# pananananas/MVD

Hardware: AMD Instinct MI355X
Metric: UNet forward-passes/sec @512x512 SD2.1+MV adapter (higher is better)
Workload: dtype bf16; 1 GPU; cfg4: configs[3]/[4]: 8 objects x 4 target views per GPU (32 pairs), camera FiLM + cross-view adapter; pairs_per_gpu=32, global_pairs=32, latent=64x64x4, image=512x512, forward=cold, hip_graph=False, q2_statistics=replica-local, parallelism=dp1 (pairs sharded by object), weights=synthetic seeded, SD2.1 shapes (865.9M UNet x2 + 99.2M adapter + 19.1M camera), encoder_weights=distinct

## Files before the change

### include/mvd_hip.h

```cpp
#ifndef MVD_HIP_H
#define MVD_HIP_H
#include <stddef.h>
#include <stdint.h>

#ifdef __cplusplus
extern "C" {
#endif

#define MVD_MAX_LEVELS 4

typedef struct {
  int in_channels;
  int out_channels;
  int num_levels;
  int block_out_channels[MVD_MAX_LEVELS];
  int num_heads[MVD_MAX_LEVELS];
  int layers_per_block;
  int cross_attention_dim;
  int norm_num_groups;
  float norm_eps;
  int cam_output_dim;
  int cam_hidden_dim;
  int simple_cam_encoder;
  float cam_modulation_strength;
} mvd_config_t;

typedef struct mvd_engine mvd_engine_t;

const char* mvd_last_error(void);

int mvd_engine_create(const mvd_config_t* cfg, mvd_engine_t** out);
int mvd_engine_destroy(mvd_engine_t* e);

int mvd_engine_set_weight(mvd_engine_t* e, int set, const char* slot, const void* ptr, int64_t numel, int dtype);
int mvd_engine_clear_weights(mvd_engine_t* e, int set);

int64_t mvd_engine_workspace_bytes(mvd_engine_t* e, int batch, int height, int width, int text_len, int ref_batch);
int64_t mvd_engine_refcache_bytes(mvd_engine_t* e, int ref_batch, int height, int width, int keep_features);
int mvd_engine_bind_workspace(mvd_engine_t* e, void* ws, int64_t ws_bytes, void* refcache, int64_t refcache_bytes);

enum {
  MVD_USE_CAMERA = 1,
  MVD_USE_IMAGE = 2,
  MVD_REUSE_REF = 4,
  MVD_KEEP_FEATURES = 8
};

typedef struct {
  int batch;
  int height, width;
  int text_len;
  const float* sample;
  const float* timesteps;
  const float* text;
  const float* source_camera;
  const float* target_camera;
  int cam_rows;
  int cam_batch;
  const float* fourier_proj;
  const float* source_latents;
  const float* encoder_text;
  int ref_batch;
  int flags;
  float* out;
} mvd_forward_args_t;

int mvd_unet_forward(mvd_engine_t* e, const mvd_forward_args_t* args, void* stream);

int64_t mvd_engine_reference_pixels(mvd_engine_t* e, int height, int width);
int mvd_engine_reference_encode(mvd_engine_t* e, const mvd_forward_args_t* args, float* local_stats, void* stream);
int mvd_engine_reference_finish(mvd_engine_t* e, const float* mean_k, void* stream);

int mvd_engine_set_graph(mvd_engine_t* e, int enable);

int mvd_engine_share_encoder_weights(mvd_engine_t* e, int enable);

int mvd_engine_set_profiling(mvd_engine_t* e, int enable);
int mvd_engine_profile_summary(mvd_engine_t* e, int cap, int* cls, int* launches, double* ms, double* flops, double* bytes);
int mvd_engine_profile_shapes(mvd_engine_t* e, char* buf_host, int cap);

int mvd_engine_num_features(mvd_engine_t* e);
int mvd_engine_feature_shape(mvd_engine_t* e, int idx, int* channels, int* height, int* width);
int mvd_engine_get_feature(mvd_engine_t* e, int idx, float* out_nchw, void* stream);
int mvd_engine_encode_cameras(mvd_engine_t* e, const float* source_camera, const float* target_camera, int cam_rows,
                              int batch, const float* fourier_proj, float* out_emb, void* stream);
int mvd_engine_apply_modulation(mvd_engine_t* e, const char* name, const float* emb, int batch, const float* x_nchw,
                                int channels, int hw, float* out_nchw, void* stream);
int mvd_engine_get_camera_embedding(mvd_engine_t* e, float* out, void* stream);

int mvd_op_linear(const void* a, const void* a2, int k1, int k2, const void* w, const float* bias, const float* rowvec,
                  int ld_rowvec, int rows_per_batch, const void* res, float alpha, int geglu, void* out, int out_f32,
                  int m, int n, int force_cfg, int splitk, float* splitk_ws ,
                  void* stream);
int mvd_op_ln_linear(const void* x, int k, const void* w_folded, const float* c1, const float* c2, float eps, int geglu,
                     void* out, int m, int n, void* stream);
int mvd_op_linear_xs(const void* x, int ldx, const void* w_packed, int m, int k, int units, int geglu, int ln, float ln_eps,
                     const void* res, int ldres, void* out, int ldo, int csplit, void* stream);
int mvd_op_conv3x3_ws(const void* x, int batch, int h, int w, int c, const void* w_packed, const float* bias, const float* rowvec,
                      int ld_rowvec, const void* res, const void* sc, const void* sc2, int sc_c1, int sc_c2, void* out, int n,
                      int variant, void* stream);
int mvd_op_conv3x3(const void* x, int batch, int in_h, int in_w, int cin, int stride, int upsample, int asym_pad, const void* w,
                   const float* bias, const float* rowvec, int ld_rowvec, const void* res, const void* sc, const void* sc2,
                   int sc_c1, int sc_c2, void* out, int cout, int force_cfg, int splitk, float* splitk_ws, void* stream);
int mvd_op_conv3x3_up4(const void* x, int batch, int in_h, int in_w, int cin, const void* w4, const float* bias, void* out, int cout,
                       int force_cfg, void* stream);
int mvd_op_attention(const void* q, const void* k, const void* v, void* o, int batch, int heads, int nq, int nk, int ldq,
                     int ldk, int ldv, int ldo, float scale, void* stream);
int64_t mvd_op_attention_split_ws_bytes(int batch, int heads, int nq, int nsplit);
int mvd_op_attention_split(const void* q, const void* k, const void* v, void* o, int batch, int heads, int nq, int nk, int ldq,
                           int ldk, int ldv, int ldo, int nsplit, void* ws, void* stream);
int mvd_op_groupnorm(const void* x0, const void* x1, int c0, int c1, int batch, int hw, int groups, float eps,
                     const float* gamma, const float* beta, int silu, void* y, float* ws, void* stream);
int mvd_op_layernorm(const void* x, int rows, int c, float eps, const float* gamma, const float* beta, void* y,
                     void* stream);
int mvd_op_refnorm(const void* x, int batch, int hw, int c, void* y, void* stream);
int mvd_op_film(const void* x, int batch, int hw, int c, const float* scale, const float* shift, void* y, void* stream);
int mvd_op_conv_in(const void* x, int batch, int h, int w, int cin, const float* wt, const float* bias, int cout, void* y,
                   void* stream);
int mvd_op_conv_out(const void* x, int batch, int h, int w, int c, const void* wt, const float* bias, int cout, float* y,
                    void* stream);
int mvd_op_nchw_to_nhwc(const float* x, int batch, int c, int hw, const float* scale, const float* shift, void* y,
                        void* stream);
int mvd_op_nhwc_to_nchw(const void* x, int batch, int hw, int c, float* y, void* stream);
int mvd_op_f32_to_bf16(const float* x, int64_t n, void* y, void* stream);
int mvd_op_skinny_linear(const float* x, int ldx, int batch, int k, const void* w, int wbf16, const float* bias, int n, int act_in,
                         float* y, int ldy, void* stream);
int mvd_gemm_num_configs(void);
int mvd_debug_last_gemm_plan(int* out);
int mvd_debug_last_attention_plan(int* out);
int mvd_debug_last_groupnorm_plan(int* out);
long mvd_debug_up4_launches(void);
int mvd_debug_last_gemm_nowait(void);
int mvd_debug_pick_splitk(int m, int n, int k, int geglu);
int mvd_debug_pick_splitk_conv(int m, int n, int k);
int mvd_gemm_sm_num_tiles(void);
int mvd_debug_set_attention_nw(int nw_log2);
typedef enum {
  MVD_DBG_NO_SM_LN_FOLD = 1,
  MVD_DBG_SM_NO_SPLITK = 2,
  MVD_DBG_NO_SM = 4,
  MVD_DBG_NO_SPLIT_KV = 8,
  MVD_DBG_ONE_STREAM = 16,
  MVD_DBG_SINGLE_STREAM_POLICY = 32,
  MVD_DBG_SIDE_DEFAULT_PRIORITY = 64,
  MVD_DBG_NO_XS = 128,
  MVD_DBG_NO_WS = 256,
  MVD_DBG_WS_SMALL_MAPS = 512,
  MVD_DBG_WS_BLOCK64 = 1024,
  MVD_DBG_WS_NO_SHORTCUT = 2048,
  MVD_DBG_WS_NOT_IN_ENCODER = 4096,
  MVD_DBG_WS_ONLY_IN_ENCODER = 8192,
  MVD_DBG_WS_THEN_TILED = 16384,
  MVD_DBG_WS_CHECK = 32768,
  MVD_DBG_GRAPH_ONE_STREAM = 65536,
  MVD_DBG_PP_ROW_MAJOR = 131072,
  MVD_DBG_NO_DEEP_CONV_SPLIT = 262144,
  MVD_DBG_LATE_FROM_UP1 = 524288,
  MVD_DBG_NO_UP4 = 1048576,
  MVD_DBG_GN_ONE_PASS = 2097152,
  MVD_DBG_FORK_LATE = 4194304,
  MVD_DBG_SKINNY_VECTOR = 8388608
} mvd_debug_flag_t;
int mvd_debug_set_flags(int flags);

int mvd_op_ddpm_step(const float* model_out, const float* sample, const float* noise, float c0, float c1, float c2,
                     float c3, float sigma, float* out, int64_t n, void* stream);
int mvd_op_cfg_combine(const float* uncond_cond, float guidance_scale, float* out, int64_t n_half, void* stream);
int mvd_op_sampler_step(const float* model_out, int guided, float guidance_scale, const float* sample, const float* x0_prev,
                        const float* noise, float a0, float a1, float p, float q, float r, float sigma, float* out,
                        float* x0_out, int64_t n, void* stream);

int mvd_op_add_noise(const float* x0, const float* noise, const int32_t* timesteps, const float* sqrt_ac, const float* sqrt_1mac,
                     int num_train_timesteps, float* noisy, float* velocity, int batch, int64_t per_sample, void* stream);
int64_t mvd_op_noise_loss_ws_bytes(int batch, int64_t per_sample);
int mvd_op_noise_loss(const float* pred, const float* noise, const float* x0, const float* noisy, const int32_t* timesteps,
                      const float* sqrt_ac, const float* sqrt_1mac, const float* snr, int num_train_timesteps, int prediction_type,
                      float snr_gamma, float* denoised, float* result, int batch, int64_t per_sample, void* ws, int64_t ws_bytes,
                      void* stream);
int64_t mvd_op_image_metrics_ws_bytes(int n, int c, int h, int w, int want_ssim);
int mvd_op_image_metrics(const float* x, const float* y, int n, int c, int h, int w, float data_range, int want_ssim, float* result,
                         float* per_image, void* ws, int64_t ws_bytes, void* stream);

typedef struct {
  int in_channels;
  int latent_channels;
  int num_levels;
  int block_out_channels[MVD_MAX_LEVELS];
  int layers_per_block;
  int norm_num_groups;
  float norm_eps;
} mvd_vae_config_t;
typedef struct mvd_vae mvd_vae_t;
int mvd_vae_create(const mvd_vae_config_t* cfg, mvd_vae_t** out);
int mvd_vae_destroy(mvd_vae_t* v);
int mvd_vae_set_weight(mvd_vae_t* v, const char* slot, const void* ptr, int64_t numel, int dtype);
int64_t mvd_vae_workspace_bytes(mvd_vae_t* v, int batch, int height, int width, int decode);
int mvd_vae_bind_workspace(mvd_vae_t* v, void* ws, int64_t ws_bytes);
int mvd_vae_encode(mvd_vae_t* v, const float* image_nchw, int batch, int height, int width, float* moments, void* stream);
int mvd_vae_decode(mvd_vae_t* v, const float* latents_nchw, int batch, int height, int width, float* image, void* stream);
int64_t mvd_vae_mid_attention_workspace_bytes(mvd_vae_t* v, int decoder, int batch, int height, int width);
int mvd_vae_mid_attention(mvd_vae_t* v, int decoder, const void* x_nhwc_bf16, int batch, int height, int width, void* out_nhwc_bf16,
                          void* stream);
int mvd_op_softmax_rows(const float* s, int rows, int n, void* p_bf16, void* stream);
int mvd_op_gaussian_sample(const float* moments, const float* noise, int batch, int channels, int hw, float scale, float* out,
                           void* stream);

typedef struct {
  int vocab_size;
  int hidden_size;
  int intermediate_size;
  int num_layers;
  int num_heads;
  int max_positions;
  float layer_norm_eps;
  int act;
} mvd_text_config_t;
typedef struct mvd_text mvd_text_t;
int mvd_text_create(const mvd_text_config_t* cfg, mvd_text_t** out);
int mvd_text_destroy(mvd_text_t* t);
int mvd_text_set_weight(mvd_text_t* t, const char* slot, const void* ptr, int64_t numel, int dtype);
int64_t mvd_text_workspace_bytes(mvd_text_t* t, int batch, int seq_len);
int mvd_text_bind_workspace(mvd_text_t* t, void* ws, int64_t bytes);
int mvd_text_encode(mvd_text_t* t, const int32_t* ids, int batch, int seq_len, float* out, void* stream);
int mvd_op_attention_causal(const void* q, const void* k, const void* v, void* o, int batch, int heads, int n, int ldq, int ldk,
                            int ldv, int ldo, float scale, void* stream);

typedef struct {
  int image_size;
  int patch_size;
  int hidden_size;
  int intermediate_size;
  int num_layers;
  int num_heads;
  int projection_dim;
  float layer_norm_eps;
  int act;
} mvd_vision_config_t;
typedef struct mvd_vision mvd_vision_t;
int mvd_vision_create(const mvd_vision_config_t* cfg, mvd_vision_t** out);
int mvd_vision_destroy(mvd_vision_t* v);
int mvd_vision_set_weight(mvd_vision_t* v, const char* slot, const void* ptr, int64_t numel, int dtype);
int64_t mvd_vision_workspace_bytes(mvd_vision_t* v, int batch, int h, int w, int resize_to);
int mvd_vision_bind_workspace(mvd_vision_t* v, void* ws, int64_t bytes);
int mvd_vision_preprocess(mvd_vision_t* v, const float* images_nchw, int batch, int h, int w, int quantize, int resize_to, int crop,
                          const float* mean, const float* std_, int want_patches, float* pixel_values, void* stream);
// ... 71 lines not shown
```

### mvd_amd/_lib.py

```python
from __future__ import annotations

import ctypes as C
import enum
import os

HERE = os.path.dirname(os.path.abspath(__file__))
LIB_PATH = os.environ.get("MVD_HIP_LIB") or os.path.join(HERE, "libmvd_hip.so")

MVD_MAX_LEVELS = 4
MVD_USE_CAMERA, MVD_USE_IMAGE, MVD_REUSE_REF, MVD_KEEP_FEATURES = 1, 2, 4, 8


class MvdError(RuntimeError):
    pass


class DebugFlag(enum.IntFlag):
    NO_SM_LN_FOLD = 1
    SM_NO_SPLITK = 2
    NO_SM = 4
    NO_SPLIT_KV = 8
    ONE_STREAM = 16
    SINGLE_STREAM_POLICY = 32
    SIDE_DEFAULT_PRIORITY = 64
# ... 24 lines not shown
        ("norm_eps", C.c_float), ("cam_output_dim", C.c_int), ("cam_hidden_dim", C.c_int),
        ("simple_cam_encoder", C.c_int), ("cam_modulation_strength", C.c_float),
    ]


class mvd_vae_config_t(C.Structure):
    _fields_ = [
        ("in_channels", C.c_int), ("latent_channels", C.c_int), ("num_levels", C.c_int),
        ("block_out_channels", C.c_int * MVD_MAX_LEVELS), ("layers_per_block", C.c_int), ("norm_num_groups", C.c_int),
        ("norm_eps", C.c_float),
    ]


class mvd_text_config_t(C.Structure):
    _fields_ = [
        ("vocab_size", C.c_int), ("hidden_size", C.c_int), ("intermediate_size", C.c_int), ("num_layers", C.c_int),
        ("num_heads", C.c_int), ("max_positions", C.c_int), ("layer_norm_eps", C.c_float), ("act", C.c_int),
    ]


class mvd_vision_config_t(C.Structure):
    _fields_ = [
        ("image_size", C.c_int), ("patch_size", C.c_int), ("hidden_size", C.c_int), ("intermediate_size", C.c_int),
        ("num_layers", C.c_int), ("num_heads", C.c_int), ("projection_dim", C.c_int), ("layer_norm_eps", C.c_float), ("act", C.c_int),
    ]


class mvd_forward_args_t(C.Structure):
    _fields_ = [
        ("batch", C.c_int), ("height", C.c_int), ("width", C.c_int), ("text_len", C.c_int),
        ("sample", C.c_void_p), ("timesteps", C.c_void_p), ("text", C.c_void_p),
        ("source_camera", C.c_void_p), ("target_camera", C.c_void_p), ("cam_rows", C.c_int), ("cam_batch", C.c_int),
        ("fourier_proj", C.c_void_p), ("source_latents", C.c_void_p), ("encoder_text", C.c_void_p),
        ("ref_batch", C.c_int), ("flags", C.c_int), ("out", C.c_void_p),
    ]


_SIGS = {
    "mvd_last_error": (C.c_char_p, []),
    "mvd_engine_create": (C.c_int, [C.POINTER(mvd_config_t), C.POINTER(C.c_void_p)]),
    "mvd_engine_destroy": (C.c_int, [C.c_void_p]),
    "mvd_engine_set_weight": (C.c_int, [C.c_void_p, C.c_int, C.c_char_p, C.c_void_p, C.c_int64, C.c_int]),
    "mvd_engine_clear_weights": (C.c_int, [C.c_void_p, C.c_int]),
    "mvd_engine_workspace_bytes": (C.c_int64, [C.c_void_p, C.c_int, C.c_int, C.c_int, C.c_int, C.c_int]),
    "mvd_engine_refcache_bytes": (C.c_int64, [C.c_void_p, C.c_int, C.c_int, C.c_int, C.c_int]),
    "mvd_engine_bind_workspace": (C.c_int, [C.c_void_p, C.c_void_p, C.c_int64, C.c_void_p, C.c_int64]),
    "mvd_unet_forward": (C.c_int, [C.c_void_p, C.POINTER(mvd_forward_args_t), C.c_void_p]),
    "mvd_engine_set_profiling": (C.c_int, [C.c_void_p, C.c_int]),
    "mvd_engine_profile_summary": (C.c_int, [C.c_void_p, C.c_int, C.POINTER(C.c_int), C.POINTER(C.c_int),
                                             C.POINTER(C.c_double), C.POINTER(C.c_double), C.POINTER(C.c_double)]),
    "mvd_engine_profile_shapes": (C.c_int, [C.c_void_p, C.c_char_p, C.c_int]),
    "mvd_engine_set_graph": (C.c_int, [C.c_void_p, C.c_int]),
    "mvd_engine_reference_pixels": (C.c_int64, [C.c_void_p, C.c_int, C.c_int]),
    "mvd_engine_reference_encode": (C.c_int, [C.c_void_p, C.POINTER(mvd_forward_args_t), C.c_void_p, C.c_void_p]),
    "mvd_engine_reference_finish": (C.c_int, [C.c_void_p, C.c_void_p, C.c_void_p]),
    "mvd_engine_share_encoder_weights": (C.c_int, [C.c_void_p, C.c_int]),
    "mvd_engine_num_features": (C.c_int, [C.c_void_p]),
    "mvd_engine_feature_shape": (C.c_int, [C.c_void_p, C.c_int, C.POINTER(C.c_int), C.POINTER(C.c_int), C.POINTER(C.c_int)]),
    "mvd_engine_get_feature": (C.c_int, [C.c_void_p, C.c_int, C.c_void_p, C.c_void_p]),
    "mvd_engine_encode_cameras": (C.c_int, [C.c_void_p, C.c_void_p, C.c_void_p, C.c_int, C.c_int, C.c_void_p, C.c_void_p, C.c_void_p]),
    "mvd_engine_apply_modulation": (C.c_int, [C.c_void_p, C.c_char_p, C.c_void_p, C.c_int, C.c_void_p, C.c_int, C.c_int, C.c_void_p, C.c_void_p]),
    "mvd_engine_get_camera_embedding": (C.c_int, [C.c_void_p, C.c_void_p, C.c_void_p]),
    "mvd_op_linear": (C.c_int, [C.c_void_p, C.c_void_p, C.c_int, C.c_int, C.c_void_p, C.c_void_p, C.c_void_p, C.c_int,
                                C.c_int, C.c_void_p, C.c_float, C.c_int, C.c_void_p, C.c_int, C.c_int, C.c_int, C.c_int,
                                C.c_int, C.c_void_p, C.c_void_p]),
    "mvd_op_ln_linear": (C.c_int, [C.c_void_p, C.c_int, C.c_void_p, C.c_void_p, C.c_void_p, C.c_float, C.c_int, C.c_void_p,
                                   C.c_int, C.c_int, C.c_void_p]),
    "mvd_op_linear_xs": (C.c_int, [C.c_void_p, C.c_int, C.c_void_p, C.c_int, C.c_int, C.c_int, C.c_int, C.c_int, C.c_float,
                                   C.c_void_p, C.c_int, C.c_void_p, C.c_int, C.c_int, C.c_void_p]),
    "mvd_op_conv3x3_ws": (C.c_int, [C.c_void_p, C.c_int, C.c_int, C.c_int, C.c_int, C.c_void_p, C.c_void_p, C.c_void_p, C.c_int,
                                    C.c_void_p, C.c_void_p, C.c_void_p, C.c_int, C.c_int, C.c_void_p, C.c_int, C.c_int, C.c_void_p]),
    "mvd_op_conv3x3": (C.c_int, [C.c_void_p, C.c_int, C.c_int, C.c_int, C.c_int, C.c_int, C.c_int, C.c_int, C.c_void_p, C.c_void_p,
                                 C.c_void_p, C.c_int, C.c_void_p, C.c_void_p, C.c_void_p, C.c_int, C.c_int, C.c_void_p,
                                 C.c_int, C.c_int, C.c_int, C.c_void_p, C.c_void_p]),
    "mvd_op_attention": (C.c_int, [C.c_void_p, C.c_void_p, C.c_void_p, C.c_void_p, C.c_int, C.c_int, C.c_int, C.c_int,
                                   C.c_int, C.c_int, C.c_int, C.c_int, C.c_float, C.c_void_p]),
    "mvd_op_attention_split_ws_bytes": (C.c_int64, [C.c_int, C.c_int, C.c_int, C.c_int]),
    "mvd_op_attention_split": (C.c_int, [C.c_void_p, C.c_void_p, C.c_void_p, C.c_void_p, C.c_int, C.c_int, C.c_int, C.c_int, C.c_int,
                                         C.c_int, C.c_int, C.c_int, C.c_int, C.c_void_p, C.c_void_p]),
    "mvd_op_groupnorm": (C.c_int, [C.c_void_p, C.c_void_p, C.c_int, C.c_int, C.c_int, C.c_int, C.c_int, C.c_float,
                                   C.c_void_p, C.c_void_p, C.c_int, C.c_void_p, C.c_void_p, C.c_void_p]),
    "mvd_op_layernorm": (C.c_int, [C.c_void_p, C.c_int, C.c_int, C.c_float, C.c_void_p, C.c_void_p, C.c_void_p, C.c_void_p]),
    "mvd_op_refnorm": (C.c_int, [C.c_void_p, C.c_int, C.c_int, C.c_int, C.c_void_p, C.c_void_p]),
    "mvd_op_film": (C.c_int, [C.c_void_p, C.c_int, C.c_int, C.c_int, C.c_void_p, C.c_void_p, C.c_void_p, C.c_void_p]),
    "mvd_op_conv_in": (C.c_int, [C.c_void_p, C.c_int, C.c_int, C.c_int, C.c_int, C.c_void_p, C.c_void_p, C.c_int, C.c_void_p, C.c_void_p]),
    "mvd_op_conv_out": (C.c_int, [C.c_void_p, C.c_int, C.c_int, C.c_int, C.c_int, C.c_void_p, C.c_void_p, C.c_int, C.c_void_p, C.c_void_p]),
    "mvd_op_nchw_to_nhwc": (C.c_int, [C.c_void_p, C.c_int, C.c_int, C.c_int, C.c_void_p, C.c_void_p, C.c_void_p, C.c_void_p]),
    "mvd_op_nhwc_to_nchw": (C.c_int, [C.c_void_p, C.c_int, C.c_int, C.c_int, C.c_void_p, C.c_void_p]),
    "mvd_op_f32_to_bf16": (C.c_int, [C.c_void_p, C.c_int64, C.c_void_p, C.c_void_p]),
    "mvd_op_skinny_linear": (C.c_int, [C.c_void_p, C.c_int, C.c_int, C.c_int, C.c_void_p, C.c_int, C.c_void_p, C.c_int, C.c_int,
                                        C.c_void_p, C.c_int, C.c_void_p]),
    "mvd_gemm_num_configs": (C.c_int, []),
    "mvd_debug_last_gemm_plan": (C.c_int, [C.POINTER(C.c_int)]),
    "mvd_debug_up4_launches": (C.c_long, []),
    "mvd_op_conv3x3_up4": (C.c_int, [C.c_void_p, C.c_int, C.c_int, C.c_int, C.c_int, C.c_void_p, C.c_void_p, C.c_void_p, C.c_int, C.c_int,
                                     C.c_void_p]),
    "mvd_debug_last_gemm_nowait": (C.c_int, []),
    "mvd_debug_last_attention_plan": (C.c_int, [C.POINTER(C.c_int)]),
    "mvd_debug_last_groupnorm_plan": (C.c_int, [C.POINTER(C.c_int)]),
    "mvd_debug_pick_splitk": (C.c_int, [C.c_int, C.c_int, C.c_int, C.c_int]),
    "mvd_debug_pick_splitk_conv": (C.c_int, [C.c_int, C.c_int, C.c_int]),
    "mvd_gemm_sm_num_tiles": (C.c_int, []),
    "mvd_debug_set_attention_nw": (C.c_int, [C.c_int]),
    "mvd_debug_set_flags": (C.c_int, [C.c_int]),
    "mvd_op_ddpm_step": (C.c_int, [C.c_void_p, C.c_void_p, C.c_void_p, C.c_float, C.c_float, C.c_float, C.c_float,
                                   C.c_float, C.c_void_p, C.c_int64, C.c_void_p]),
    "mvd_op_cfg_combine": (C.c_int, [C.c_void_p, C.c_float, C.c_void_p, C.c_int64, C.c_void_p]),
    "mvd_op_sampler_step": (C.c_int, [C.c_void_p, C.c_int, C.c_float, C.c_void_p, C.c_void_p, C.c_void_p, C.c_float, C.c_float,
                                      C.c_float, C.c_float, C.c_float, C.c_float, C.c_void_p, C.c_void_p, C.c_int64, C.c_void_p]),
    "mvd_op_add_noise": (C.c_int, [C.c_void_p, C.c_void_p, C.c_void_p, C.c_void_p, C.c_void_p, C.c_int, C.c_void_p, C.c_void_p, C.c_int,
                                   C.c_int64, C.c_void_p]),
    "mvd_op_noise_loss_ws_bytes": (C.c_int64, [C.c_int, C.c_int64]),
    "mvd_op_noise_loss": (C.c_int, [C.c_void_p, C.c_void_p, C.c_void_p, C.c_void_p, C.c_void_p, C.c_void_p, C.c_void_p, C.c_void_p,
                                    C.c_int, C.c_int, C.c_float, C.c_void_p, C.c_void_p, C.c_int, C.c_int64, C.c_void_p, C.c_int64,
                                    C.c_void_p]),
    "mvd_op_image_metrics_ws_bytes": (C.c_int64, [C.c_int, C.c_int, C.c_int, C.c_int, C.c_int]),
    "mvd_op_image_metrics": (C.c_int, [C.c_void_p, C.c_void_p, C.c_int, C.c_int, C.c_int, C.c_int, C.c_float, C.c_int, C.c_void_p,
                                       C.c_void_p, C.c_void_p, C.c_int64, C.c_void_p]),
    "mvd_vae_create": (C.c_int, [C.POINTER(mvd_vae_config_t), C.POINTER(C.c_void_p)]),
    "mvd_vae_destroy": (C.c_int, [C.c_void_p]),
    "mvd_vae_set_weight": (C.c_int, [C.c_void_p, C.c_char_p, C.c_void_p, C.c_int64, C.c_int]),
    "mvd_vae_workspace_bytes": (C.c_int64, [C.c_void_p, C.c_int, C.c_int, C.c_int, C.c_int]),
    "mvd_vae_bind_workspace": (C.c_int, [C.c_void_p, C.c_void_p, C.c_int64]),
    "mvd_vae_encode": (C.c_int, [C.c_void_p, C.c_void_p, C.c_int, C.c_int, C.c_int, C.c_void_p, C.c_void_p]),
    "mvd_vae_decode": (C.c_int, [C.c_void_p, C.c_void_p, C.c_int, C.c_int, C.c_int, C.c_void_p, C.c_void_p]),
    "mvd_vae_mid_attention_workspace_bytes": (C.c_int64, [C.c_void_p, C.c_int, C.c_int, C.c_int, C.c_int]),
    "mvd_vae_mid_attention": (C.c_int, [C.c_void_p, C.c_int, C.c_void_p, C.c_int, C.c_int, C.c_int, C.c_void_p, C.c_void_p]),
    "mvd_op_softmax_rows": (C.c_int, [C.c_void_p, C.c_int, C.c_int, C.c_void_p, C.c_void_p]),
    "mvd_op_gaussian_sample": (C.c_int, [C.c_void_p, C.c_void_p, C.c_int, C.c_int, C.c_int, C.c_float, C.c_void_p, C.c_void_p]),
    "mvd_text_create": (C.c_int, [C.POINTER(mvd_text_config_t), C.POINTER(C.c_void_p)]),
    "mvd_text_destroy": (C.c_int, [C.c_void_p]),
    "mvd_text_set_weight": (C.c_int, [C.c_void_p, C.c_char_p, C.c_void_p, C.c_int64, C.c_int]),
    "mvd_text_workspace_bytes": (C.c_int64, [C.c_void_p, C.c_int, C.c_int]),
    "mvd_text_bind_workspace": (C.c_int, [C.c_void_p, C.c_void_p, C.c_int64]),
    "mvd_text_encode": (C.c_int, [C.c_void_p, C.c_void_p, C.c_int, C.c_int, C.c_void_p, C.c_void_p]),
    "mvd_op_attention_causal": (C.c_int, [C.c_void_p, C.c_void_p, C.c_void_p, C.c_void_p, C.c_int, C.c_int, C.c_int, C.c_int,
                                          C.c_int, C.c_int, C.c_int, C.c_float, C.c_void_p]),
    "mvd_vision_create": (C.c_int, [C.POINTER(mvd_vision_config_t), C.POINTER(C.c_void_p)]),
    "mvd_vision_destroy": (C.c_int, [C.c_void_p]),
    "mvd_vision_set_weight": (C.c_int, [C.c_void_p, C.c_char_p, C.c_void_p, C.c_int64, C.c_int]),
    "mvd_vision_workspace_bytes": (C.c_int64, [C.c_void_p, C.c_int, C.c_int, C.c_int, C.c_int]),
    "mvd_vision_bind_workspace": (C.c_int, [C.c_void_p, C.c_void_p, C.c_int64]),
    "mvd_vision_preprocess": (C.c_int, [C.c_void_p, C.c_void_p, C.c_int, C.c_int, C.c_int, C.c_int, C.c_int, C.c_int,
                                        C.POINTER(C.c_float), C.POINTER(C.c_float), C.c_int, C.c_void_p, C.c_void_p]),
    "mvd_vision_patch_rows_offset": (C.c_int64, [C.c_void_p]),
    "mvd_vision_encode": (C.c_int, [C.c_void_p, C.c_void_p, C.c_int, C.c_void_p, C.c_void_p, C.c_void_p, C.c_void_p]),
    "mvd_op_clip_pool_project": (C.c_int, [C.c_void_p, C.c_void_p, C.c_void_p, C.c_int, C.c_int, C.c_int, C.c_int, C.c_void_p,
                                           C.c_void_p, C.c_float, C.c_void_p, C.c_int, C.c_void_p, C.c_void_p, C.c_void_p]),
    "mvd_op_clip_cosine": (C.c_int, [C.c_void_p, C.c_void_p, C.c_int, C.c_int, C.c_void_p, C.c_void_p, C.c_void_p]),
    "mvd_vgg_create": (C.c_int, [C.POINTER(C.c_void_p)]),
    "mvd_vgg_destroy": (C.c_int, [C.c_void_p]),
    "mvd_vgg_set_weight": (C.c_int, [C.c_void_p, C.c_char_p, C.c_void_p, C.c_int64, C.c_int]),
    "mvd_vgg_workspace_bytes": (C.c_int64, [C.c_void_p, C.c_int, C.c_int, C.c_int]),
    "mvd_vgg_bind_workspace": (C.c_int, [C.c_void_p, C.c_void_p, C.c_int64]),
    "mvd_vgg_features": (C.c_int, [C.c_void_p, C.c_void_p, C.c_int, C.c_int, C.c_int, C.c_void_p, C.POINTER(C.c_void_p), C.c_void_p]),
    "mvd_vgg_perceptual": (C.c_int, [C.c_void_p, C.c_void_p, C.c_void_p, C.c_int, C.c_int, C.c_int, C.c_void_p, C.c_void_p, C.c_void_p]),
    "mvd_op_conv3x3_relu": (C.c_int, [C.c_void_p, C.c_int, C.c_int, C.c_int, C.c_int, C.c_void_p, C.c_void_p, C.c_void_p, C.c_int, C.c_int,
                                      C.c_int, C.c_int, C.c_int, C.c_void_p, C.c_void_p]),
    "mvd_op_linear_relu": (C.c_int, [C.c_void_p, C.c_int, C.c_void_p, C.c_void_p, C.c_void_p, C.c_int, C.c_int, C.c_int, C.c_int, C.c_int,
                                     C.c_int, C.c_void_p, C.c_void_p]),
    "mvd_op_maxpool2x2": (C.c_int, [C.c_void_p, C.c_int, C.c_int, C.c_int, C.c_int, C.c_void_p, C.c_void_p]),
    "mvd_op_sqdiff_mean_ws_bytes": (C.c_int64, [C.c_int, C.c_int64]),
    "mvd_op_sqdiff_mean": (C.c_int, [C.c_void_p, C.c_void_p, C.c_int, C.c_int64, C.c_void_p, C.c_void_p, C.c_void_p, C.c_int64, C.c_void_p]),
    "mvd_lpips_create": (C.c_int, [C.POINTER(C.c_void_p)]),
    "mvd_lpips_destroy": (C.c_int, [C.c_void_p]),
    "mvd_lpips_set_weight": (C.c_int, [C.c_void_p, C.c_char_p, C.c_void_p, C.c_int64, C.c_int]),
    "mvd_lpips_workspace_bytes": (C.c_int64, [C.c_void_p, C.c_int, C.c_int, C.c_int]),
    "mvd_lpips_bind_workspace": (C.c_int, [C.c_void_p, C.c_void_p, C.c_int64]),
    "mvd_lpips_features": (C.c_int, [C.c_void_p, C.c_void_p, C.c_int, C.c_int, C.c_int, C.POINTER(C.c_void_p), C.c_void_p]),
    "mvd_lpips_distance": (C.c_int, [C.c_void_p, C.c_void_p, C.c_void_p, C.c_int, C.c_int, C.c_int, C.c_int, C.c_void_p, C.c_void_p,
                                     C.c_void_p, C.c_void_p]),
    "mvd_op_im2col_patch": (C.c_int, [C.c_void_p, C.c_int, C.c_int, C.c_int, C.c_int, C.POINTER(C.c_float), C.POINTER(C.c_float), C.c_void_p,
                                      C.c_void_p]),
    "mvd_op_maxpool3x3s2": (C.c_int, [C.c_void_p, C.c_int, C.c_int, C.c_int, C.c_int, C.c_void_p, C.c_void_p]),
    "mvd_op_lpips_head_ws_bytes": (C.c_int64, [C.c_int, C.POINTER(C.c_int), C.c_int]),
    "mvd_op_lpips_head": (C.c_int, [C.c_int, C.POINTER(C.c_void_p), C.POINTER(C.c_void_p), C.POINTER(C.c_int), C.POINTER(C.c_int),
                                    C.POINTER(C.c_int), C.POINTER(C.c_int), C.POINTER(C.c_void_p), C.c_int, C.c_void_p, C.c_void_p, C.c_void_p,
                                    C.c_void_p, C.c_int64, C.c_void_p]),
    "mvd_fid_create": (C.c_int, [C.POINTER(C.c_int), C.c_int, C.POINTER(C.c_int), C.c_int, C.POINTER(C.c_char_p), C.c_int, C.c_int, C.c_int,
                                 C.POINTER(C.c_void_p)]),
# ... 61 lines not shown
```

### mvd_amd/csrc/engine.hip

```cpp
#include <math.h>
#include <stdio.h>
#include <stdlib.h>
#include <string.h>

#include <string>
#include <unordered_map>
#include <vector>

#include "host_util.h"

int mvd_launch_silu_to_bf16(const float* x, int64_t n, bf16_t* y, hipStream_t s);

static int g_debug_flags = 0;
extern "C" int mvd_debug_set_flags(int flags) { g_debug_flags = flags; return 0; }
int mvd_debug_flags() { return g_debug_flags; }

namespace {

struct FeatureInfo { std::string name; int level; int C; int heads; std::string key;  };
constexpr int MVD_REF_ONLY_INTERNAL = 1 << 30;

}

struct mvd_engine {
  mvd_config_t cfg;
  WeightTable w[2];
  Arena tmp, act, persist;
  void* ws_ptr = nullptr; int64_t ws_bytes = 0;
  void* rc_ptr = nullptr; int64_t rc_bytes = 0;
  std::vector<FeatureInfo> feats;
  std::vector<bf16_t*> refkv;
  std::vector<bf16_t*> feat_keep;
  int rc_batch = 0, rc_h = 0, rc_w = 0; bool rc_valid = false; bool rc_keep = false;
  float* ref_stats_out = nullptr;
  bool rc_pending = false;
  int64_t ref_pixels(int h, int w) const { int64_t n = 0; for (auto& f : feats) n += (int64_t)(h >> f.level) * (w >> f.level); return n; }
  int64_t feat_pixel_off(int idx) const { int64_t n = 0; for (int i = 0; i < idx; ++i) n += (int64_t)(rc_h >> feats[i].level) * (rc_w >> feats[i].level); return n; }
  float* cam_emb = nullptr; int cam_batch = 0;
  unsigned int* cnt_base = nullptr; int cnt_used = 0, cnt_cap = 0;
  hipStream_t side = nullptr;
  std::vector<hipEvent_t> feat_ev;
  hipEvent_t fork_ev = nullptr, join_ev = nullptr;
  bool dual_now = false;
  int ensure_side_stream() {
    if (side) return 0;
    {
      int lo = 0, hi = 0;
      (void)hipDeviceGetStreamPriorityRange(&lo, &hi);
      const int pr = (g_debug_flags & MVD_DBG_SIDE_DEFAULT_PRIORITY) ? 0 : hi;
      if (hipStreamCreateWithPriority(&side, hipStreamNonBlocking, pr) != hipSuccess) { mvd_set_error("engine: hipStreamCreate failed"); return -3; }
    }
    feat_ev.resize(feats.size());
    for (auto& ev : feat_ev) if (hipEventCreateWithFlags(&ev, hipEventDisableTiming) != hipSuccess) { mvd_set_error("engine: hipEventCreate failed"); return -3; }
    if (hipEventCreateWithFlags(&fork_ev, hipEventDisableTiming) != hipSuccess || hipEventCreateWithFlags(&join_ev, hipEventDisableTiming) != hipSuccess) { mvd_set_error("engine: hipEventCreate failed"); return -3; }
    return 0;
  }
  bool share_encoder = false;
  struct HostState {
    std::vector<bf16_t*> refkv, feat_keep;
    int rc_batch, rc_h, rc_w; bool rc_valid, rc_keep;
    float* cam_emb; int cam_batch;
  };
  HostState host_state() const { return {refkv, feat_keep, rc_batch, rc_h, rc_w, rc_valid, rc_keep, cam_emb, cam_batch}; }
  void set_host_state(const HostState& h) {
    refkv = h.refkv; feat_keep = h.feat_keep; rc_batch = h.rc_batch; rc_h = h.rc_h; rc_w = h.rc_w; rc_valid = h.rc_valid;
    rc_keep = h.rc_keep; cam_emb = h.cam_emb; cam_batch = h.cam_batch;
  }
  struct GraphEntry { std::string key; hipGraph_t g; hipGraphExec_t x; HostState after; };
  bool dual_late = false;
  bool graph_on = false;
  std::vector<GraphEntry> graphs;
  std::vector<std::string> graph_seen;
  void drop_graphs() {
    for (auto& ge : graphs) { (void)hipGraphExecDestroy(ge.x); (void)hipGraphDestroy(ge.g); }
    graphs.clear(); graph_seen.clear();
  }
  ~mvd_engine() {
    drop_graphs();
    for (hipEvent_t ev : ev_pool) (void)hipEventDestroy(ev);
    for (hipEvent_t ev : feat_ev) if (ev) (void)hipEventDestroy(ev);
    if (fork_ev) (void)hipEventDestroy(fork_ev);
    if (join_ev) (void)hipEventDestroy(join_ev);
    if (side) (void)hipStreamDestroy(side);
  }
  std::vector<int> temb_off;
  int temb_total = 0;
  std::vector<int> tkv_off;
  int tkv_total = 0;
  bool prof = false;
  bool prof_overlap = false;
  struct ProfRec { int cls; double flops; double bytes; hipEvent_t e0, e1; int M, N, K, tag; };
  int prof_M = 0, prof_N = 0, prof_K = 0, prof_tag = 0;
  std::vector<ProfRec> prof_recs;
  std::vector<hipEvent_t> ev_pool; size_t ev_used = 0;
  hipEvent_t get_event() {
    if (ev_used == ev_pool.size()) { hipEvent_t ev = nullptr; (void)hipEventCreate(&ev); ev_pool.push_back(ev); }
    return ev_pool[ev_used++];
  }
// ... 69 lines not shown

struct Ctx {
  mvd_engine* e;
  hipStream_t s;
  int set;
  bool dry;
  int err = 0;
  bool nowait = false;

  const void* W(const std::string& name, int dtype, int64_t numel, int set_override = -1) {
    if (dry) return nullptr;
    const int st = set_override >= 0 ? set_override : set;
    return e->w[st].find(name, dtype, numel, &err, "", st);
  }
  const bf16_t* WB(const std::string& n, int64_t numel, int so = -1) { return (const bf16_t*)W(n, 1, numel, so); }
  const float* WF(const std::string& n, int64_t numel, int so = -1) { return (const float*)W(n, 0, numel, so); }
  bool has(const std::string& n, int so = -1) { return e->w[so >= 0 ? so : set].has(n); }

  template <class T> T* talloc(size_t n) { return e->tmp.alloc_n<T>(n); }
  template <class T> T* aalloc(size_t n) { return e->act.alloc_n<T>(n); }
  Act new_act(int B, int H, int W_, int C, bool longlived) { return arena_act(longlived ? e->act : e->tmp, B, H, W_, C); }

  template <class F> int profiled(int cls, double flops, double bytes, F&& launch) {
    if (!e->prof) return launch();
    hipEvent_t e0 = e->get_event(), e1 = e->get_event();
    (void)hipEventRecord(e0, s);
    const int r = launch();
    (void)hipEventRecord(e1, s);
    e->prof_recs.push_back({cls, flops, bytes, e0, e1, e->prof_M, e->prof_N, e->prof_K, e->prof_tag});
    return r;
  }
  static bool sm_enabled() {
    static const bool use_sm = MVD_ENV_INT("MVD_GEMM_SM", 1) != 0;
    return use_sm && !(g_debug_flags & MVD_DBG_NO_SM);
  }
  void tiled_plan(const MvdGemmArgs& g, int& S, int& fc) {
    S = mvd_gemm_pick_splitk(g);
    fc = -1;
    if (e->dual_now && !e->dual_late && !(g_debug_flags & MVD_DBG_SINGLE_STREAM_POLICY) && !g.geglu && !g.ln_c1 && !g.out_f32 && g.N % 320 == 0 && mvd_gemm_pp_applicable(g)) {
      const int cfg = mvd_gemm_pick_config(g);
      const long t7 = (long)((g.M + 255) / 256) * (g.N / 320);
      if (t7 >= 100) { S = 1; if (cfg != 7) fc = 7; }
    }
  }
  int gemm(MvdGemmArgs& g) {
    if (err) return err;
    int sm_tile = 0, sm_ns = 0, sm_S = 1;
    if (sm_enabled() && mvd_gemm_sm_plan(g, &sm_tile, &sm_ns, &sm_S)) {
      if (g_debug_flags & MVD_DBG_SM_NO_SPLITK) sm_S = 1;
      const size_t mark = e->tmp.off;
      if (sm_S > 1) {
        g.splitk = sm_S; g.splitk_nowait = nowait ? 1 : 0; g.part = talloc<float>((size_t)sm_S * g.M * g.N);
        const int tiles = ((g.M + 63) / 64) * (g.N / 64);
        g.tile_cnt = e->cnt_base + e->cnt_used;
        e->cnt_used += tiles;
        if (!dry && e->cnt_used > e->cnt_cap) { mvd_set_error("forward: split-K tile counters exhausted (%d > %d)", e->cnt_used, e->cnt_cap); return err = -15; }
      }
      int r = 0;
      if (!dry) {
        const double fl = 2.0 * g.M * (double)g.N * g.Ktot;
        e->prof_M = g.M; e->prof_N = g.N; e->prof_K = g.Ktot; e->prof_tag = g.seg[0].mode * 100 + g.geglu * 10 + (sm_S > 1 ? sm_S : 0);
        r = profiled(MVD_PC_SM_64X64 + sm_tile, fl, 0.0, [&] { return mvd_launch_gemm_sm(g, s, sm_tile, sm_ns); });
      }
      e->tmp.off = mark;
      return r;
    }
    int S = 1, fc = -1;
    tiled_plan(g, S, fc);
    const size_t mark = e->tmp.off;
    if (S > 1) { g.splitk = S; g.part = talloc<float>((size_t)S * g.M * g.N); } else g.splitk = 1;
    static const bool trace = MVD_ENV_INT("MVD_TRACE_GEMM", 0) != 0;
    if (trace && !dry) fprintf(stderr, "gemm M=%d N=%d K=%d mode=%d nseg=%d geglu=%d cfg=%d splitk=%d\n", g.M, g.N, g.Ktot, g.seg[0].mode, g.nseg, g.geglu, mvd_gemm_pick_config(g), S);
    int r = 0;
    if (!dry) {
      const double fl = 2.0 * g.M * (double)g.N * g.Ktot;
      e->prof_M = g.M; e->prof_N = g.N; e->prof_K = g.Ktot; e->prof_tag = g.seg[0].mode * 100 + g.geglu * 10 + (S > 1 ? S : 0);
      r = launch_tiled(g, s, fc, [&](auto&& launch) { return profiled(e->prof ? gemm_class(g, mvd_gemm_pick_config(g), S) : 0, fl, 0.0, launch); });
    }
    e->tmp.off = mark;
    return r;
  }

  int try_xs(const bf16_t* x, int K, int M, const std::string& slot, int64_t n_full, int N, bool geglu, bool ln,
             const bf16_t* res, int ldres, void* out, int ldo, int set_override = -1) {
    if (err) return err;
    if (dry || (g_debug_flags & MVD_DBG_NO_XS) || K != 320 || slot.empty() || !has(slot, set_override)) return 0;
    MvdXsArgs a; memset(&a, 0, sizeof(a));
    a.x = x; a.ldx = K; a.M = M; a.K = K; a.units = N / 32; a.geglu = geglu; a.ln = ln; a.ln_eps = 1e-5f;
    a.res = res; a.ldres = ldres; a.out = (bf16_t*)out; a.ldo = ldo;
    if (N % 64 || !mvd_gemm_xs_applicable(a)) return 0;
    if ((long)((M + 255) / 256) * mvd_gemm_xs_pick_csplit(a) < 448) return 0;
    a.w = WB(slot, (n_full / 32) * 21 * 512, set_override);
    if (!a.w) return err;
    e->prof_M = M; e->prof_N = N; e->prof_K = K; e->prof_tag = geglu * 10 + (ln ? 1 : 0);
    const int r = profiled(geglu ? MVD_PC_XS_GEGLU : (res ? MVD_PC_XS_RESIDUAL : (ln ? MVD_PC_XS_LN_DENSE : MVD_PC_XS_DENSE)), 2.0 * M * (double)N * K, 0.0, [&] { return mvd_launch_gemm_xs(a, s); });
    return r ? r : 1;
  }

  int linear(const bf16_t* a, const bf16_t* a2, int k1, int k2, int M, const bf16_t* w, const float* bias, int N,
             const bf16_t* res, int ldres, void* out, int ldo, bool geglu = false, bool out_f32 = false, int ldw = 0,
             const std::string& xs = std::string(), int xs_set = -1) {
    if (!xs.empty() && !a2 && !k2 && !geglu && !out_f32) {
      const int r = try_xs(a, k1, M, xs, N, N, false, false, res, ldres, out, ldo, xs_set);
      if (r) return r < 0 ? r : 0;
    }
    MvdGemmArgs g = gemm_dense(a, a2, k1, k2, M, w, ldw, bias, N, out, ldo);
    g.res = res; g.ldres = ldres; g.geglu = geglu; g.out_f32 = out_f32;
    return gemm(g);
  }

  int ln_linear(const bf16_t* x, int M, int C, const std::string& ln_key, const std::string& slot, int64_t n_full, int N,
                const float* bias, bf16_t* ln_tmp, void* out, int ldo, bool geglu) {
    MvdGemmArgs g = gemm_dense(x, nullptr, C, 0, M, nullptr, 0, nullptr, N, out, ldo);
    g.geglu = geglu;
    {
      const int r = try_xs(x, C, M, slot + ".wx", n_full, N, geglu, true, nullptr, 0, out, ldo);
      if (r) return r < 0 ? r : 0;
    }
    static const bool use_fold = MVD_ENV_INT("MVD_LN_FOLD", 1) != 0;
    auto sm_fold_ok = [&]() {
      MvdGemmArgs t = g;
      static const float dummy = 0.f;
      t.ln_c1 = &dummy; t.bias = &dummy; t.W = reinterpret_cast<const bf16_t*>(&dummy);
      int a_, b_, c_;
      return sm_enabled() && !(g_debug_flags & MVD_DBG_NO_SM_LN_FOLD) && mvd_gemm_sm_plan(t, &a_, &b_, &c_);
    };
    if (use_fold && !dry && has(slot + ".wf") && has(slot + ".cf") && (mvd_gemm_ln_fold_ok(g) || sm_fold_ok())) {
      const float* cf = WF(slot + ".cf", 2 * n_full);
      g.W = WB(slot + ".wf", n_full * C);
      g.ln_c1 = cf; g.bias = cf ? cf + n_full : nullptr; g.ln_eps = 1e-5f;
      return gemm(g);
    }
    CHECK(layernorm(x, M, C, WF(ln_key + ".g", C), WF(ln_key + ".b", C), ln_tmp));
    g.seg[0].p0 = ln_tmp; g.W = WB(slot + ".w", n_full * C); g.bias = bias;
    return gemm(g);
  }

  int try_ws(const Act& x, int ups, const std::string& slot, const float* bias, const float* rowvec, int ld_rowvec, const bf16_t* res,
             const bf16_t* sc0, const bf16_t* sc1, int scc0, int scc1, Act& out) {
    if (err) return err;
    if (dry || (g_debug_flags & MVD_DBG_NO_WS) || slot.empty() || !has(slot)) return 0;
    MvdWsArgs a; memset(&a, 0, sizeof(a));
    a.x = x.p; a.B = x.B; a.H = x.H; a.W = x.W; a.C = x.C; a.ups = ups; a.sc0 = sc0; a.sc1 = sc1; a.scc0 = scc0; a.scc1 = scc1;
    a.bias = bias; a.rowvec = rowvec; a.ld_rowvec = ld_rowvec; a.res = res; a.ldres = out.C; a.out = out.p; a.ldo = out.C;
    a.M = out.rows(); a.N = out.C;
    if ((g_debug_flags & MVD_DBG_WS_SMALL_MAPS) && a.M > 256) return 0;
    if (g_debug_flags & MVD_DBG_WS_BLOCK64) a.variant = 1;
    if ((g_debug_flags & MVD_DBG_WS_NO_SHORTCUT) && scc0) return 0;
    if ((g_debug_flags & MVD_DBG_WS_NOT_IN_ENCODER) && nowait) return 0;
    if ((g_debug_flags & MVD_DBG_WS_ONLY_IN_ENCODER) && !nowait) return 0;
    if (out.H != (ups ? 2 : 1) * x.H || out.W != (ups ? 2 : 1) * x.W || out.B != x.B || a.M > 1024) return 0;
    if ((long)(a.M / 64) * (a.N / 16) > 1000) return 0;
    a.w = reinterpret_cast<const bf16_t*>(&a);
    if (!mvd_conv_ws_applicable(a)) return 0;
    a.w = WB(slot, (int64_t)mvd_conv_ws_packed_elems(x.C, scc0 + scc1, out.C));
    if (!a.w) return err;
    e->prof_M = a.M; e->prof_N = a.N; e->prof_K = 9 * x.C + scc0 + scc1; e->prof_tag = 100 + (scc0 ? 1 : 0);
    const int r = profiled(MVD_PC_CONV_WS, 2.0 * a.M * (double)a.N * (9.0 * x.C + scc0 + scc1), 0.0, [&] { return mvd_launch_conv_ws(a, s); });
    if (!r && (g_debug_flags & MVD_DBG_WS_THEN_TILED)) return 0;
#ifdef MVD_PROBE
    if (!r && (g_debug_flags & MVD_DBG_WS_CHECK)) {
      const size_t mark = e->tmp.off;
      Act chk = new_act(out.B, out.H, out.W, out.C, false);
      const bf16_t* wold = WB(slot.substr(0, slot.size() - 1), (int64_t)out.C * (9 * x.C + scc0 + scc1));
      if (wold) {
        const int saved = g_debug_flags; g_debug_flags |= MVD_DBG_NO_WS;
        conv3(x, 1, ups, wold, bias, rowvec, ld_rowvec, res, sc0, sc1, scc0, scc1, chk);
        g_debug_flags = saved;
        g_ws_ptrs[0] = (const char*)x.p; g_ws_lens[0] = (size_t)x.rows() * x.C * 2;
        g_ws_ptrs[1] = (const char*)sc0; g_ws_lens[1] = (size_t)out.rows() * scc0 * 2;
        g_ws_ptrs[2] = (const char*)sc1; g_ws_lens[2] = (size_t)out.rows() * scc1 * 2;
        g_ws_ptrs[3] = (const char*)out.p; g_ws_lens[3] = (size_t)out.rows() * out.C * 2;
        ws_check_launch(slot, set, nowait, out.p, chk.p, (long)out.rows() * out.C, s);
      }
      e->tmp.off = mark;
    }
// ... 129 lines not shown
  int feat_idx = 0;

  int resnet(const std::string& key, const Act& x0, const Act* x1, int cout, Act& out) {
    const int cin0 = x0.C, cin1 = x1 ? x1->C : 0, cin = cin0 + cin1;
    const int B_ = x0.B, hw = x0.hw();
    const size_t mark = c.e->tmp.off;
    Act t1 = c.new_act(B_, x0.H, x0.W, cin, false);
    CHECK(c.groupnorm(x0.p, x1 ? x1->p : nullptr, cin0, cin1, B_, hw, cfg.norm_eps, c.WF(key + ".norm1.g", cin), c.WF(key + ".norm1.b", cin), 1, t1.p));
    Act h1 = c.new_act(B_, x0.H, x0.W, cout, false);
    const int toff = c.e->temb_off[resnet_idx++];
    CHECK(c.conv3(t1, 1, 0, c.WB(key + ".conv1.w", (int64_t)cout * 9 * cin), c.WF(key + ".conv1.b", cout), tproj + toff, c.e->temb_total,
                  nullptr, nullptr, nullptr, 0, 0, h1, key + ".conv1.ws"));
    Act t2 = c.new_act(B_, x0.H, x0.W, cout, false);
    CHECK(c.groupnorm(h1.p, nullptr, cout, 0, B_, hw, cfg.norm_eps, c.WF(key + ".norm2.g", cout), c.WF(key + ".norm2.b", cout), 1, t2.p));
    if (cin != cout) {
      CHECK(c.conv3(t2, 1, 0, c.WB(key + ".conv2.w", (int64_t)cout * (9 * cout + cin)), c.WF(key + ".conv2.b", cout), nullptr, 0, nullptr,
                    x0.p, x1 ? x1->p : nullptr, cin0, cin1, out, key + ".conv2.ws"));
    } else {
      CHECK(c.conv3(t2, 1, 0, c.WB(key + ".conv2.w", (int64_t)cout * 9 * cout), c.WF(key + ".conv2.b", cout), nullptr, 0, x0.p, nullptr,
                    nullptr, 0, 0, out, key + ".conv2.ws"));
    }
    c.e->tmp.off = mark;
    return c.err;
  }

  int transformer(const std::string& key, const Act& x, int heads, Act& out) {
    const int C = x.C, M = x.rows(), hw = x.hw(), B_ = x.B;
    const bool ad = o.adapter;
    const bool packed = c.set == 0 && (c.dry || c.has(key + ".ref_kv.w", 0));
    if (ad && !packed) { mvd_set_error("adapter requested but no adapter weights registered for %s", key.c_str()); return -14; }
    const int ld_out = packed ? 2 * C : C;
    const char* bias_slot = (packed && !ad) ? ".out.b0" : ".out.b";
    const size_t mark = c.e->tmp.off;
    bf16_t* n0 = c.talloc<bf16_t>((size_t)M * C);
    CHECK(c.groupnorm(x.p, nullptr, C, 0, B_, hw, 1e-6f, c.WF(key + ".norm.g", C), c.WF(key + ".norm.b", C), 0, n0));
    bf16_t* h = c.talloc<bf16_t>((size_t)M * C);
    CHECK(c.linear(n0, nullptr, C, 0, M, c.WB(key + ".proj_in.w", (int64_t)C * C), c.WF(key + ".proj_in.b", C), C, nullptr, 0, h, C, false, false, 0, key + ".proj_in.wx"));
    bf16_t* ln = n0;
    const float scale = 0.125f;
    bf16_t* o_self = c.talloc<bf16_t>((size_t)M * C);
    bf16_t* o_ref = ad ? c.talloc<bf16_t>((size_t)M * C) : nullptr;
    const bf16_t* rkv = ad ? c.e->refkv[feat_idx] : nullptr;
    const int ref_nk = ad ? (int)((int64_t)o.ref_batch * hw / B_) : 0;
    if (ad && (int64_t)ref_nk * B_ != (int64_t)o.ref_batch * hw) { mvd_set_error("adapter: ref tokens %d x %d not divisible by batch %d", o.ref_batch, hw, B_); return -12; }

    if (ad && c.e->dual_now && !c.dry && !c.err && hipStreamWaitEvent(c.s, c.e->feat_ev[feat_idx], 0) != hipSuccess) { mvd_set_error("forward: hipStreamWaitEvent failed"); return -3; }
    {
      const int nq = ad ? 4 * C : 3 * C;
      bf16_t* qkv = c.talloc<bf16_t>((size_t)M * nq);
      CHECK(c.ln_linear(h, M, C, key + ".ln1", key + ".attn1.qkv", (int64_t)(packed ? 4 : 3) * C, nq, nullptr, ln, qkv, nq, false));
      MvdAttnArgs a; memset(&a, 0, sizeof(a));
      a.batch = B_; a.heads = heads; a.scale = scale; a.prescaled = 1; a.nprob = ad ? 2 : 1;
      a.p[0] = {qkv, qkv + C, qkv + 2 * C, o_self, nq, nq, nq, C, (int64_t)hw * nq, (int64_t)hw * nq, (int64_t)hw * nq, (int64_t)hw * C, hw, hw};
      if (ad) a.p[1] = {qkv + 3 * C, rkv, rkv + C, o_ref, nq, 4 * C, 4 * C, C, (int64_t)hw * nq, (int64_t)ref_nk * 4 * C, (int64_t)ref_nk * 4 * C, (int64_t)hw * C, hw, ref_nk};
      CHECK(c.attention(a));
      CHECK(c.linear(o_self, o_ref, C, ad ? C : 0, M, c.WB(key + ".attn1.out.w", (int64_t)C * ld_out), c.WF(key + ".attn1" + bias_slot, C), C, h, C, h, C, false, false, ld_out,
                     ad ? std::string() : key + ".attn1.out.wx"));
    }
    {
      const int nq = ad ? 2 * C : C;
      bf16_t* q2 = c.talloc<bf16_t>((size_t)M * nq);
      const bf16_t* kv2 = tkv + c.e->tkv_off[feat_idx];
      const int ldkv = c.e->tkv_total;
      CHECK(c.ln_linear(h, M, C, key + ".ln2", key + ".attn2.q", (int64_t)(packed ? 2 : 1) * C, nq, nullptr, ln, q2, nq, false));
      MvdAttnArgs a; memset(&a, 0, sizeof(a));
      a.batch = B_; a.heads = heads; a.scale = scale; a.prescaled = 1; a.nprob = ad ? 2 : 1;
      a.p[0] = {q2, kv2, kv2 + C, o_self, nq, ldkv, ldkv, C, (int64_t)hw * nq, (int64_t)L * ldkv, (int64_t)L * ldkv, (int64_t)hw * C, hw, L};
      if (ad) a.p[1] = {q2 + C, rkv + 2 * C, rkv + 3 * C, o_ref, nq, 4 * C, 4 * C, C, (int64_t)hw * nq, (int64_t)ref_nk * 4 * C, (int64_t)ref_nk * 4 * C, (int64_t)hw * C, hw, ref_nk};
      CHECK(c.attention(a));
      CHECK(c.linear(o_self, o_ref, C, ad ? C : 0, M, c.WB(key + ".attn2.out.w", (int64_t)C * ld_out), c.WF(key + ".attn2" + bias_slot, C), C, h, C, h, C, false, false, ld_out,
                     ad ? std::string() : key + ".attn2.out.wx"));
    }
    {
      bf16_t* ff = c.talloc<bf16_t>((size_t)M * 4 * C);
      CHECK(c.ln_linear(h, M, C, key + ".ln3", key + ".ff1", (int64_t)8 * C, 8 * C, c.WF(key + ".ff1.b", 8 * C), ln, ff, 4 * C, true));
      CHECK(c.linear(ff, nullptr, 4 * C, 0, M, c.WB(key + ".ff2.w", (int64_t)C * 4 * C), c.WF(key + ".ff2.b", C), C, h, C, h, C));
    }
    CHECK(c.linear(h, nullptr, C, 0, M, c.WB(key + ".proj_out.w", (int64_t)C * C), c.WF(key + ".proj_out.b", C), C, x.p, C, out.p, C, false, false, 0, key + ".proj_out.wx"));
    c.e->tmp.off = mark;

    if (o.capture) {
      const size_t mk = c.e->tmp.off;
      bf16_t* rn = c.talloc<bf16_t>((size_t)M * C);
      if (o.defer_norm) {
        if (!c.dry && !c.err) CHECK(mvd_launch_refstats(out.p, B_, hw, C, o.stats + 2 * c.e->feat_pixel_off(feat_idx), c.s));
      } else {
        if (!c.dry && !c.err) CHECK(mvd_launch_refnorm(out.p, B_, hw, C, rn, c.s));
        CHECK(c.linear(rn, nullptr, C, 0, M, c.WB(key + ".ref_kv.w", (int64_t)4 * C * C, 0), nullptr, 4 * C, nullptr, 0, c.e->refkv[feat_idx], 4 * C, false, false, 0,
                       key + ".ref_kv.wx", 0));
        if (c.e->dual_now && !c.dry && !c.err && hipEventRecord(c.e->feat_ev[feat_idx], c.s) != hipSuccess) { mvd_set_error("forward: hipEventRecord failed"); return -3; }
      }
      if (c.e->rc_keep && !c.dry && !c.err)
        CHECK((int)hipMemcpyAsync(c.e->feat_keep[feat_idx], out.p, (size_t)M * C * sizeof(bf16_t), hipMemcpyDeviceToDevice, c.s));
      c.e->tmp.off = mk;
    }
    ++feat_idx;
    return c.err;
  }

  int film(const std::string& name, const Act& x, Act& out) {
    auto it = o.film_ss->find(name);
    if (it == o.film_ss->end()) { out = x; return 0; }
    if (c.dry || c.err) return c.err;
    return mvd_launch_film(x.p, x.B, x.hw(), x.C, it->second.first, it->second.second, x.C, out.p, c.s);
  }

  int run(const Act& x_in, float* out_nchw) {
    const int n = cfg.num_levels, Lb = cfg.layers_per_block;
    const int C0 = cfg.block_out_channels[0];
    std::vector<Act> skips;
    tkv = c.aalloc<bf16_t>((size_t)B * L * c.e->tkv_total);
    CHECK(c.linear(text, nullptr, cfg.cross_attention_dim, 0, B * L, c.WB("text_kv.w", (int64_t)c.e->tkv_total * cfg.cross_attention_dim), nullptr,
                   c.e->tkv_total, nullptr, 0, tkv, c.e->tkv_total));
    Act h = c.new_act(B, H0, W0, C0, true);
    CHECK(c.linear(x_in.p, nullptr, 64, 0, B * H0 * W0, c.WB("conv_in.w", (int64_t)C0 * 64), c.WF("conv_in.b", C0), C0, nullptr, 0, h.p, C0));
    skips.push_back(h);
    for (int i = 0; i < n; ++i) {
      const int co = cfg.block_out_channels[i];
      const std::string bk = "down_blocks." + std::to_string(i);
      for (int j = 0; j < Lb; ++j) {
        Act r = c.new_act(B, h.H, h.W, co, true);
        CHECK(resnet(bk + ".resnets." + std::to_string(j), h, nullptr, co, r));
        h = r;
        if (i + 1 < n) {
          Act t = c.new_act(B, h.H, h.W, co, true);
          CHECK(transformer(bk + ".attentions." + std::to_string(j), h, cfg.num_heads[i], t));
          h = t;
        }
        skips.push_back(h);
      }
      if (i + 1 < n) {
        Act d = c.new_act(B, (h.H + 1) / 2, (h.W + 1) / 2, co, true);
        CHECK(c.conv3(h, 2, 0, c.WB(bk + ".down.w", (int64_t)co * 9 * co), c.WF(bk + ".down.b", co), nullptr, 0, nullptr, nullptr, nullptr, 0, 0, d));
        h = d;
        skips.push_back(h);
      }
      if (o.film) {
        Act m = c.new_act(B, h.H, h.W, h.C, true);
        Act res = m;
        CHECK(film("down_" + std::to_string(i), h, res));
        h = res;
      }
    }
    {
      const int cm = cfg.block_out_channels[n - 1];
      Act r = c.new_act(B, h.H, h.W, cm, true);
      CHECK(resnet("mid_block.resnets.0", h, nullptr, cm, r));
      Act t = c.new_act(B, h.H, h.W, cm, true);
      CHECK(transformer("mid_block.attentions.0", r, cfg.num_heads[n - 1], t));
      Act r2 = c.new_act(B, h.H, h.W, cm, true);
      CHECK(resnet("mid_block.resnets.1", t, nullptr, cm, r2));
      h = r2;
      if (o.film) { Act res = h; CHECK(film("mid_0", h, res)); h = res; }
    }
    for (int i = 0; i < n; ++i) {
      const int co = cfg.block_out_channels[n - 1 - i];
      const std::string bk = "up_blocks." + std::to_string(i);
      if (!o.capture && i >= o.late_from) c.e->dual_late = true;
      for (int j = 0; j <= Lb; ++j) {
        Act skip = skips.back(); skips.pop_back();
        if (skip.H != h.H || skip.W != h.W) { mvd_set_error("up block %d: skip %dx%d vs hidden %dx%d (odd latent size unsupported)", i, skip.H, skip.W, h.H, h.W); return -13; }
        Act r = c.new_act(B, h.H, h.W, co, true);
        CHECK(resnet(bk + ".resnets." + std::to_string(j), h, &skip, co, r));
        h = r;
        if (i > 0) {
          Act t = c.new_act(B, h.H, h.W, co, true);
          CHECK(transformer(bk + ".attentions." + std::to_string(j), h, cfg.num_heads[n - 1 - i], t));
          h = t;
        }
      }
      if (i + 1 < n) {
        Act u = c.new_act(B, h.H * 2, h.W * 2, co, true);
// ... 652 lines not shown
  if (rows_per_batch > 0) g.rows_per_batch = g.outW = rows_per_batch;
  g.rowvec = rowvec; g.ld_rowvec = ld_rowvec; g.res = (const bf16_t*)res; g.ldres = on; g.alpha = alpha; g.geglu = geglu; g.out_f32 = out_f32;
  return op_launch(g, force_cfg, splitk, splitk_ws, (hipStream_t)stream);
}

int mvd_op_ln_linear(const void* x, int k, const void* w_folded, const float* c1, const float* c2, float eps, int geglu,
                     void* out, int m, int n, void* stream) {
  MvdGemmArgs g = gemm_dense((const bf16_t*)x, nullptr, k, 0, m, (const bf16_t*)w_folded, 0, c2, n, out, geglu ? n / 2 : n);
  g.ln_c1 = c1; g.ln_eps = eps; g.geglu = geglu; g.ldres = g.ldo;
  if (!c1 || !c2) { mvd_set_error("mvd_op_ln_linear: c1 and c2 are required"); return -1; }
  if (!mvd_gemm_ln_fold_ok(g)) {
    int tile = 0, ns = 0, S = 1;
    if (mvd_gemm_sm_plan(g, &tile, &ns, &S) && S == 1) {
      g_mvd_last_gemm.cfg = 100 + 10 * tile + ns; g_mvd_last_gemm.splitk = 1;
      return mvd_launch_gemm_sm(g, (hipStream_t)stream, tile, ns);
    }
    mvd_set_error("mvd_op_ln_linear: M=%d N=%d K=%d geglu=%d is not a shape of the fused LayerNorm GEMMs", m, n, k, geglu);
    return -1;
  }
  return mvd_launch_gemm(g, (hipStream_t)stream);
}

int mvd_op_conv3x3(const void* x, int batch, int in_h, int in_w, int cin, int stride, int upsample, int asym_pad, const void* w,
                   const float* bias, const float* rowvec, int ld_rowvec, const void* res, const void* sc, const void* sc2,
                   int sc_c1, int sc_c2, void* out, int cout, int force_cfg, int splitk, float* splitk_ws, void* stream) {
  const int oh = upsample ? in_h * 2 : (stride == 2 ? (in_h + 1) / 2 : in_h);
  const int ow = upsample ? in_w * 2 : (stride == 2 ? (in_w + 1) / 2 : in_w);
  MvdGemmArgs g = gemm_conv3((const bf16_t*)x, in_h, in_w, cin, stride, upsample, asym_pad, (const bf16_t*)sc, (const bf16_t*)sc2, sc_c1, sc_c2,
                             (const bf16_t*)w, bias, batch, oh, ow, cout, out);
  g.rowvec = rowvec; g.ld_rowvec = ld_rowvec; g.res = (const bf16_t*)res;
  return op_launch(g, force_cfg, splitk, splitk_ws, (hipStream_t)stream);
}

int mvd_op_conv3x3_up4(const void* x, int batch, int in_h, int in_w, int cin, const void* w4, const float* bias, void* out, int cout,
                       int force_cfg, void* stream) {
  if (!x || !w4 || !out || batch <= 0 || in_h <= 0 || in_w <= 0 || cin <= 0 || cout <= 0) { mvd_set_error("mvd_op_conv3x3_up4: bad argument"); return -1; }
  MvdGemmArgs g = gemm_conv3((const bf16_t*)x, in_h, in_w, cin, 1, 1, 0, nullptr, nullptr, 0, 0, (const bf16_t*)w4, bias, batch, 2 * in_h, 2 * in_w,
                             cout, out);
  gemm_conv3_to_up4(g);
  g.splitk = 1;
  return mvd_launch_gemm(g, (hipStream_t)stream, force_cfg);
}

int mvd_op_attention(const void* q, const void* k, const void* v, void* o, int batch, int heads, int nq, int nk, int ldq,
                     int ldk, int ldv, int ldo, float scale, void* stream) {
  MvdAttnArgs a; memset(&a, 0, sizeof(a));
  a.nprob = 1; a.batch = batch; a.heads = heads; a.scale = scale;
  a.prescaled = scale == 0.f;
  a.p[0] = {(const bf16_t*)q, (const bf16_t*)k, (const bf16_t*)v, (bf16_t*)o, ldq, ldk, ldv, ldo,
            (int64_t)nq * ldq, (int64_t)nk * ldk, (int64_t)nk * ldv, (int64_t)nq * ldo, nq, nk};
  return mvd_launch_attention(a, (hipStream_t)stream);
}

int64_t mvd_op_attention_split_ws_bytes(int batch, int heads, int nq, int nsplit) {
  MvdAttnArgs a; memset(&a, 0, sizeof(a));
  a.nprob = 1; a.batch = batch; a.heads = heads; a.p[0].nq = nq;
  return (int64_t)mvd_attention_split_ws_bytes(a, nsplit) + (int64_t)mvd_attention_split_counters(a) * 4 + 256;
}
int mvd_op_attention_split(const void* q, const void* k, const void* v, void* o, int batch, int heads, int nq, int nk, int ldq,
                           int ldk, int ldv, int ldo, int nsplit, void* ws, void* stream) {
  MvdAttnArgs a; memset(&a, 0, sizeof(a));
  a.nprob = 1; a.batch = batch; a.heads = heads; a.scale = 0.f; a.prescaled = 1;
  a.p[0] = {(const bf16_t*)q, (const bf16_t*)k, (const bf16_t*)v, (bf16_t*)o, ldq, ldk, ldv, ldo,
            (int64_t)nq * ldq, (int64_t)nk * ldk, (int64_t)nk * ldv, (int64_t)nq * ldo, nq, nk};
  if (nsplit > 1) {
    if (!ws) { mvd_set_error("op_attention_split: null workspace"); return -1; }
    const size_t pb = (mvd_attention_split_ws_bytes(a, nsplit) + 255) & ~size_t(255);
    a.nsplit = nsplit; a.split_ws = ws; a.split_cnt = reinterpret_cast<unsigned int*>(reinterpret_cast<char*>(ws) + pb);
    if (hipMemsetAsync(a.split_cnt, 0, (size_t)mvd_attention_split_counters(a) * 4, (hipStream_t)stream) != hipSuccess) { mvd_set_error("op_attention_split: hipMemsetAsync failed"); return -3; }
  }
  return mvd_launch_attention(a, (hipStream_t)stream);
}

int mvd_op_groupnorm(const void* x0, const void* x1, int c0, int c1, int batch, int hw, int groups, float eps,
                     const float* gamma, const float* beta, int silu, void* y, float* ws, void* stream) {
  return mvd_launch_groupnorm((const bf16_t*)x0, (const bf16_t*)x1, c0, c1, batch, hw, groups, eps, gamma, beta, silu, (bf16_t*)y, ws, (hipStream_t)stream);
}
int mvd_op_layernorm(const void* x, int rows, int c, float eps, const float* gamma, const float* beta, void* y, void* stream) {
  return mvd_launch_layernorm((const bf16_t*)x, rows, c, eps, gamma, beta, (bf16_t*)y, (hipStream_t)stream);
}
int mvd_op_refnorm(const void* x, int batch, int hw, int c, void* y, void* stream) {
  return mvd_launch_refnorm((const bf16_t*)x, batch, hw, c, (bf16_t*)y, (hipStream_t)stream);
}
int mvd_op_film(const void* x, int batch, int hw, int c, const float* scale, const float* shift, void* y, void* stream) {
  return mvd_launch_film((const bf16_t*)x, batch, hw, c, scale, shift, c, (bf16_t*)y, (hipStream_t)stream);
}
int mvd_op_conv_in(const void* x, int batch, int h, int w, int cin, const float* wt, const float* bias, int cout, void* y, void* stream) {
  return mvd_launch_conv_in((const bf16_t*)x, batch, h, w, cin, wt, bias, cout, (bf16_t*)y, (hipStream_t)stream);
}
int mvd_op_conv_out(const void* x, int batch, int h, int w, int c, const void* wt, const float* bias, int cout, float* y, void* stream) {
  return mvd_launch_conv_out((const bf16_t*)x, batch, h, w, c, (const bf16_t*)wt, bias, cout, y, (hipStream_t)stream);
}
int mvd_op_nchw_to_nhwc(const float* x, int batch, int c, int hw, const float* scale, const float* shift, void* y, void* stream) {
  return mvd_launch_nchw_to_nhwc(x, batch, c, hw, scale, shift, c, (bf16_t*)y, (hipStream_t)stream);
}
int mvd_op_nhwc_to_nchw(const void* x, int batch, int hw, int c, float* y, void* stream) {
  return mvd_launch_nhwc_to_nchw_f32((const bf16_t*)x, batch, hw, c, y, (hipStream_t)stream);
}
int mvd_op_f32_to_bf16(const float* x, int64_t n, void* y, void* stream) {
  return mvd_launch_f32_to_bf16(x, n, (bf16_t*)y, (hipStream_t)stream);
}
int mvd_op_skinny_linear(const float* x, int ldx, int batch, int k, const void* w, int wbf16, const float* bias, int n, int act_in,
                         float* y, int ldy, void* stream) {
  return mvd_launch_skinny_linear(x, ldx, batch, k, w, wbf16, bias, n, act_in, y, ldy, (hipStream_t)stream);
}

}
```

### mvd_amd/csrc/gemm.hip

```cpp
#include <stdlib.h>
#include <string.h>
#include "kernels.h"
#include "gemm_tile.h"

thread_local MvdLaunchPlan g_mvd_last_gemm = {-1, 1, 0, 0, 0, 0};

namespace {

__global__ __launch_bounds__(256) void splitk_reduce_kernel(const MvdGemmArgs a) {
  const long nvec = (long)a.M * (a.N >> 2);
  const int nv = a.N >> 2;
  for (long e = (long)blockIdx.x * blockDim.x + threadIdx.x; e < nvec; e += (long)gridDim.x * blockDim.x) {
    const int m = (int)(e / nv), n = (int)(e - (long)m * nv) * 4;
    f32x4 v = *reinterpret_cast<const f32x4*>(a.part + (size_t)m * a.N + n);
    for (int s = 1; s < a.splitk; ++s) v += *reinterpret_cast<const f32x4*>(a.part + ((size_t)s * a.M + m) * a.N + n);
    if (a.bias) v += *reinterpret_cast<const f32x4*>(a.bias + n);
    if (a.rowvec) v += *reinterpret_cast<const f32x4*>(a.rowvec + (size_t)(m / a.rows_per_batch) * a.ld_rowvec + n);
    v *= a.alpha;
    if (a.res) {
      const u32x2 r = *reinterpret_cast<const u32x2*>(a.res + (size_t)m * a.ldres + n);
      v[0] += bflo(r[0]); v[1] += bfhi(r[0]); v[2] += bflo(r[1]); v[3] += bfhi(r[1]);
    }
    if (a.out_f32) {
      *reinterpret_cast<f32x4*>(reinterpret_cast<float*>(a.out) + (size_t)m * a.ldo + n) = v;
    } else {
      u32x2 o = {pack2bf(v[0], v[1]), pack2bf(v[2], v[3])};
      *reinterpret_cast<u32x2*>(reinterpret_cast<bf16_t*>(a.out) + (size_t)m * a.ldo + n) = o;
    }
  }
}

struct CfgInfo { int bm, bn, tn_even; };

template <class C, int AMODE, bool GLDS>
int launch_mode(const MvdGemmArgs& a, hipStream_t s) {
  if constexpr (GLDS) { if (a.splitk > 1) return launch_mode2<C, AMODE, true, true>(a, s); }
  return launch_mode2<C, AMODE, GLDS, false>(a, s);
}

template <class C, bool DMA_ONLY = false>
int launch_cfg(const MvdGemmArgs& a, hipStream_t s, bool glds) {
  if (a.splitk > 1) glds = true;
  if (glds || DMA_ONLY) {
    if (a.seg[0].mode == MVD_A_DENSE) return launch_mode<C, 0, true>(a, s);
    return a.nseg == 1 ? launch_mode<C, 1, true>(a, s) : launch_mode<C, 2, true>(a, s);
  }
  if constexpr (!DMA_ONLY) {
    if (a.seg[0].mode == MVD_A_DENSE) return launch_mode<C, 0, false>(a, s);
    return a.nseg == 1 ? launch_mode<C, 1, false>(a, s) : launch_mode<C, 2, false>(a, s);
  }
  return -1;
}

using C0 = Cfg<256, 160, 4, 2>;
using C1 = Cfg<256, 128, 4, 2>;
using C2 = Cfg<128, 160, 2, 2>;
using C3 = Cfg<128, 128, 2, 2>;
using C4 = Cfg<128, 64, 2, 2>;
using C5 = Cfg<64, 64, 2, 2>;
using C7 = Cfg<256, 320, 2, 4>;
using C6 = Cfg<256, 320, 4, 2>;
using C8 = Cfg<128, 320, 2, 4>;
const CfgInfo kCfgs[] = {{256, 160, 0}, {256, 128, 1}, {128, 160, 0}, {128, 128, 1}, {128, 64, 1}, {64, 64, 1}, {256, 320, 1}, {256, 320, 0},
                         {128, 320, 0}};
constexpr int kNumCfgs = 9;

}

extern "C" int mvd_gemm_num_configs(void) { return kNumCfgs; }

extern "C" int mvd_debug_last_gemm_plan(int* out) {
  if (!out) { mvd_set_error("last_gemm_plan: null argument"); return -1; }
  out[0] = g_mvd_last_gemm.cfg; out[1] = g_mvd_last_gemm.splitk; out[2] = g_mvd_last_gemm.tiles;
  out[3] = g_mvd_last_gemm.grid; out[4] = g_mvd_last_gemm.per_cu;
  return 0;
}

std::atomic<long> g_mvd_up4_launches{0};
extern "C" long mvd_debug_up4_launches(void) { return g_mvd_up4_launches.load(); }

extern "C" int mvd_debug_last_gemm_nowait(void) { return g_mvd_last_gemm.nowait; }

static int deep_conv_split(const MvdGemmArgs& a, long t7) {
  static const int on = MVD_ENV_INT("MVD_GEMM_DEEP_CONV_SPLIT", 1);
  if (!on || (mvd_debug_flags() & MVD_DBG_NO_DEEP_CONV_SPLIT) || a.seg[0].mode == MVD_A_DENSE || a.geglu || a.out_f32 || t7 < 24 || t7 > 64 || a.Ktot < 8192 || (a.splitk > 0 && a.splitk < 4)) return 1;
  int s = (int)(256 / t7);
  while (s > 1 && a.Ktot / 64 / s < 16) --s;
  return s > 16 ? 16 : s;
}

int mvd_gemm_pick_config(const MvdGemmArgs& a) {
  static const int use7 = MVD_ENV_INT("MVD_GEMM_BIG", 1);
  static const int split_min_slabs = MVD_ENV_INT("MVD_GEMM_SPLIT_MINK", 4096) / 64;
  static const int use8 = MVD_ENV_INT("MVD_GEMM_C8", 0);
  if (use7 && !a.relu && a.N % 320 == 0 && a.M >= 1024) {
    const long t7 = (long)((a.M + 255) / 256) * (a.N / 320);
    if (a.geglu) { if (t7 >= 200) return 6; }
    else if (t7 >= 200) return 7;
    else if (use8 && t7 * 2 >= 200) return 8;
    else if (a.Ktot / 64 >= split_min_slabs && t7 * 2 >= 200) return 7;
    else if (deep_conv_split(a, t7) > 1) return 7;
  }
  static const int order[] = {2, 3, 4, 5};
  int cfg = -1, first_valid = -1;
  long best_blocks = -1;
  for (int c : order) {
    if (a.N % kCfgs[c].bn) continue;
    if (a.geglu && !kCfgs[c].tn_even) continue;
    if (a.relu && c == 2) continue;
    const long blocks = (long)((a.M + kCfgs[c].bm - 1) / kCfgs[c].bm) * (a.N / kCfgs[c].bn);
    if (first_valid < 0) {
      first_valid = c;
      if (blocks < 300 && !a.geglu && a.Ktot / 64 >= 16 && c <= 3 && a.M >= 512) return c;
    }
    if (blocks >= 300) return c;
    if (blocks > best_blocks) { best_blocks = blocks; cfg = c; }
  }
  return cfg;
}

int mvd_launch_gemm(const MvdGemmArgs& a, hipStream_t s, int force_cfg) {
  if (a.M <= 0 || a.N <= 0 || a.Ktot <= 0 || a.nseg < 1 || a.nseg > 2) { mvd_set_error("gemm: bad dims M=%d N=%d K=%d nseg=%d", a.M, a.N, a.Ktot, a.nseg); return -1; }
  int ksum = 0;
  for (int i = 0; i < a.nseg; ++i) {
    const MvdASeg& g = a.seg[i];
    if (g.mode == MVD_A_DENSE) {
      if (g.c0 % 64 || g.c1 % 64 || g.ksize != g.c0 + g.c1 || !g.p0 || (g.c1 && !g.p1)) { mvd_set_error("gemm: bad dense segment %d (c0=%d c1=%d ksize=%d)", i, g.c0, g.c1, g.ksize); return -1; }
    } else if (g.mode == MVD_A_CONV3) {
      if (g.ups != 0 && g.ups != 1 && g.ups != 2) { mvd_set_error("gemm: bad conv segment %d (ups=%d)", i, g.ups); return -1; }
      if (g.c0 % 64 || g.c1 != 0 || g.ksize != (g.ups == 2 ? 4 : 9) * g.c0 || !g.p0 || (g.stride != 1 && g.stride != 2) || (g.ups && g.stride != 1)) { mvd_set_error("gemm: bad conv segment %d", i); return -1; }
      if (g.asym && (g.asym != 1 || g.stride != 2 || (g.inH & 1) || (g.inW & 1))) { mvd_set_error("gemm: bottom/right-only padding needs stride 2 and an even input size"); return -1; }
      const int eh = g.ups ? 2 * g.inH : (g.stride == 2 ? (g.inH + 1) / 2 : g.inH);
      const int ew = g.ups ? 2 * g.inW : (g.stride == 2 ? (g.inW + 1) / 2 : g.inW);
      if (eh != a.outH || ew != a.outW || a.rows_per_batch != a.outH * a.outW || a.M % a.rows_per_batch) { mvd_set_error("gemm: conv geometry mismatch (in %dx%d out %dx%d rpb %d M %d)", g.inH, g.inW, a.outH, a.outW, a.rows_per_batch, a.M); return -1; }
    } else { mvd_set_error("gemm: bad mode"); return -1; }
    ksum += g.ksize;
  }
  if (a.nseg == 2 && !(a.seg[0].mode == MVD_A_CONV3 && a.seg[1].mode == MVD_A_DENSE)) { mvd_set_error("gemm: a second segment must be a dense segment after a conv segment"); return -1; }
  if (ksum != a.Ktot) { mvd_set_error("gemm: segment K sum %d != Ktot %d", ksum, a.Ktot); return -1; }
  if (a.ldw < a.Ktot || (a.ldw % 8) || !a.W) { mvd_set_error("gemm: bad weight stride ldw=%d (K=%d)", a.ldw, a.Ktot); return -1; }
  if (a.rows_per_batch <= 0) { mvd_set_error("gemm: rows_per_batch must be > 0"); return -1; }
  if (a.N % 64) { mvd_set_error("gemm: N=%d must be a multiple of 64", a.N); return -1; }
  if (a.splitk > 1 && (!a.part || a.geglu || a.splitk > (force_cfg >= 100 ? 64 : 16) || a.splitk > a.Ktot / 64)) { mvd_set_error("gemm: bad split-K request (splitk=%d)", a.splitk); return -1; }
  if (a.geglu && (a.out_f32 || a.res || a.rowvec)) { mvd_set_error("gemm: unsupported GEGLU epilogue combination"); return -1; }
  if (a.relu && (a.relu != 1 || a.geglu || a.ln_c1 || a.nseg != 1 || a.w_blocked || (a.seg[0].mode == MVD_A_CONV3 && a.seg[0].ups == 2))) {
    mvd_set_error("gemm: the ReLU epilogue takes one dense or one 3x3 segment (no GEGLU, LayerNorm fold, fused shortcut, sub-pixel upsampler, blocked weights)");
    return -1;
  }
  const int on = a.geglu ? a.N / 2 : a.N;
  if (a.ldo < on || (a.ldo % 4) || (a.res && (a.ldres % 4))) { mvd_set_error("gemm: bad leading dims"); return -1; }

  static const int default_glds = MVD_ENV_INT("MVD_GEMM_GLDS", 1);
  bool glds = default_glds != 0;
#ifdef MVD_PROBE
  static const int dbg = MVD_ENV_INT("MVD_GEMM_DEBUG", 0);
  if (dbg) const_cast<MvdGemmArgs&>(a).dbg = dbg;
#endif
  if (a.seg[0].mode == MVD_A_CONV3 && a.seg[0].ups == 2) {
    if ((force_cfg >= 0 && force_cfg != 7) || (a.dbg & ~32) || !mvd_gemm_pp_up4_applicable(a)) {
      mvd_set_error("gemm: the 2x2 sub-pixel upsampling convolution does not take this problem (in %dx%d C=%d N=%d cfg=%d): source width a multiple of 16 or 8 (even height), N %% 320 == 0, bias only, unsplit",
                    a.seg[0].inH, a.seg[0].inW, a.seg[0].c0, a.N, force_cfg);
      return -1;
    }
    g_mvd_last_gemm.cfg = 7; g_mvd_last_gemm.splitk = 1;
    return mvd_launch_gemm_pp(a, s);
  }
  int cfg = force_cfg;
  if (cfg >= 1000) { const_cast<MvdGemmArgs&>(a).w_blocked = 1; cfg -= 1000; }
  if (a.w_blocked && cfg < 100) { mvd_set_error("gemm: the blocked weight layout is read by the small-M kernels only"); return -1; }
  if (cfg >= 100) {
    const int tile = (cfg - 100) / 10, ns = (cfg - 100) % 10;
    if (a.splitk > 1 && !a.tile_cnt) { mvd_set_error("gemm: the small-M kernels combine split-K in the kernel and need tile counters"); return -1; }
    g_mvd_last_gemm.cfg = cfg; g_mvd_last_gemm.splitk = a.splitk > 1 ? a.splitk : 1;
    return mvd_launch_gemm_sm(a, s, tile, ns ? ns : 4);
  }
#ifdef MVD_PROBE
  static const int use_ring = MVD_ENV_INT("MVD_GEMM_RING", 0);
  if (cfg == 15) {
    if (a.N % 320 || a.geglu || a.out_f32) { mvd_set_error("gemm: the ring kernel needs N %% 320 == 0, bf16 output, no GEGLU"); return -1; }
    return mvd_launch_gemm_ring(a, s);
  }
#endif
  bool legacy = MVD_ENV_INT("MVD_GEMM_LEGACY", 0) != 0;
  if (cfg == 16 || cfg == 17) { legacy = true; cfg -= 10; }
  if (cfg == 14) { glds = true; cfg = 8; }
  else if (cfg >= 8 && cfg < 14) { glds = true; cfg -= 8; } else if (cfg >= 0 && cfg < 6) { glds = false; }
  if (cfg < 0) cfg = mvd_gemm_pick_config(a);
  if (a.ln_c1) {
    if ((cfg != 6 && cfg != 7) || legacy || a.dbg || !mvd_gemm_ln_fold_ok(a)) { mvd_set_error("gemm: LayerNorm fold not available for M=%d N=%d K=%d cfg=%d", a.M, a.N, a.Ktot, cfg); return -1; }
  }
  if (cfg < 0 || cfg >= kNumCfgs || a.N % kCfgs[cfg].bn || (a.geglu && !kCfgs[cfg].tn_even)) { mvd_set_error("gemm: no tile config for N=%d geglu=%d cfg=%d", a.N, a.geglu, cfg); return -1; }
  g_mvd_last_gemm.cfg = cfg; g_mvd_last_gemm.splitk = a.splitk > 1 ? a.splitk : 1;
#ifndef MVD_PROBE
  if (cfg == 0 || cfg == 1 || cfg == 8 || force_cfg == 16 || force_cfg == 17) { mvd_set_error("gemm: tile config %d exists in probe builds only", force_cfg >= 0 ? force_cfg : cfg); return -1; }
#endif
  if (a.relu) {
    if (cfg < 3 || cfg > 5) { mvd_set_error("gemm: the ReLU epilogue exists for tile configs 3, 4, 5 (128x128, 128x64, 64x64), not %d", force_cfg >= 0 ? force_cfg : cfg); return -1; }
    if (a.splitk <= 1) return mvd_launch_gemm_relu(a, s, cfg, glds);
  }
  switch (cfg) {
#ifdef MVD_PROBE
    case 0: return launch_cfg<C0>(a, s, glds);
    case 1: return launch_cfg<C1>(a, s, glds);
    case 8: return launch_cfg<C8>(a, s, true);
#endif
    case 2: return launch_cfg<C2>(a, s, glds);
    case 3: return launch_cfg<C3>(a, s, glds);
    case 4: return launch_cfg<C4>(a, s, glds);
    case 6:
      if (!a.geglu || a.seg[0].mode != MVD_A_DENSE || a.splitk > 1) { mvd_set_error("gemm: tile config 6 is GEGLU-only"); return -1; }
      if (!legacy && !(a.dbg & ~32) && mvd_gemm_pp_applicable(a)) return mvd_launch_gemm_pp(a, s);
      return launch_mode2<C6, 0, true, false>(a, s);
    case 7:
      if (!legacy && !(a.dbg & ~32) && !a.geglu && mvd_gemm_pp_applicable(a)) return mvd_launch_gemm_pp(a, s);
#ifdef MVD_PROBE
      if (use_ring && !a.out_f32 && !a.dbg) return mvd_launch_gemm_ring(a, s);
#endif
      return launch_cfg<C7, true>(a, s, true);
    default: return launch_cfg<C5>(a, s, glds);
  }
}

int mvd_gemm_pick_splitk(const MvdGemmArgs& a) {
  if (a.geglu) return 1;
  const int cfg = mvd_gemm_pick_config(a);
  if (cfg < 0) return 1;
  const long tiles = (long)((a.M + kCfgs[cfg].bm - 1) / kCfgs[cfg].bm) * (a.N / kCfgs[cfg].bn);
  const int nkt = a.Ktot / 64;
  if (cfg == 7 && deep_conv_split(a, tiles) > 1) return deep_conv_split(a, tiles);
  if (cfg == 7 || cfg == 8) return (tiles >= 200 || nkt < 16) ? 1 : 2;
  if (tiles >= 256 || nkt < 16) return 1;
  long s = 512 / tiles;
  if (s > nkt / 8) s = nkt / 8;
  long cap = (long)a.Ktot / (4L * a.M);
  cap = cap < 4 ? 4 : (cap > 16 ? 16 : cap);
  if (s > cap) s = cap;
  return s < 2 ? 1 : (int)s;
}

extern "C" int mvd_debug_pick_splitk(int m, int n, int k, int geglu) {
  MvdGemmArgs a; memset(&a, 0, sizeof(a));
  a.M = m; a.N = n; a.Ktot = k; a.geglu = geglu;
  return mvd_gemm_pick_splitk(a);
}
extern "C" int mvd_debug_pick_splitk_conv(int m, int n, int k) {
  MvdGemmArgs a; memset(&a, 0, sizeof(a));
  a.M = m; a.N = n; a.Ktot = k; a.seg[0].mode = MVD_A_CONV3;
  return mvd_gemm_pick_splitk(a);
}

int mvd_launch_splitk_reduce(const MvdGemmArgs& a, hipStream_t s) {
  if (a.splitk < 2 || !a.part || (a.N & 3)) { mvd_set_error("splitk_reduce: bad arguments"); return -1; }
  const long nvec = (long)a.M * (a.N >> 2);
  int grid = (int)((nvec + 255) / 256);
  if (grid > 2048) grid = 2048;
  if (a.relu) return mvd_launch_splitk_reduce_relu(a, s, grid);
  hipLaunchKernelGGL(splitk_reduce_kernel, dim3(grid), dim3(256), 0, s, a);
  hipError_t e = hipGetLastError();
  if (e != hipSuccess) { mvd_set_error("splitk_reduce launch: %s", hipGetErrorString(e)); return -3; }
  return 0;
}
```

### mvd_amd/csrc/gemm_pp.hip

```cpp
#include <stdlib.h>
#include <string.h>
#include "kernels.h"
#include "bufaddr.h"

namespace {

constexpr int BN = 320, NT = 512;
constexpr int B_BYTES = BN * 128, B_IT = BN * 8 / NT;

MVD_DEVINL int fresh_lane() {
  int l = (int)__builtin_amdgcn_mbcnt_hi(~0u, __builtin_amdgcn_mbcnt_lo(~0u, 0u));
  asm volatile("" : "+v"(l));
  return l;
}

MVD_DEVINL int swz_off(int row, int chunk) { return row * 128 + ((chunk ^ ((row >> 1) & 7)) << 4); }

constexpr int XCH_C1 = 0, XCH_C2 = 2048, XCH_STATS = 4096, XCH_BYTES = 6144;

template <int BM, int WM, int WN, int AMODE, bool SPLITK, bool LNF = false>
__global__ __launch_bounds__(NT, 2) void gemm_pp_kernel(const MvdGemmArgs a) {
  static_assert(!LNF || (AMODE == 0 && !SPLITK), "the LayerNorm fold is a dense, unsplit form");
  constexpr int A_BYTES = BM * 128, STAGE_BYTES = A_BYTES + B_BYTES;
  constexpr int A_IT = BM * 8 / NT;
// ... 469 lines not shown
  issue_consts(ld_n0);
  init_acc();
  asm volatile("s_waitcnt vmcnt(0)" ::: "memory");
  phase_end();
  if (grp == 1) phase_end();

  int cur = 0;
  bool pend = false;
  int pm0 = 0, pn0 = 0, pks = 0;
  for (;;) {
    const int tl = S == 1 ? tile : tile / S;
    const int ks = S == 1 ? 0 : tile - tl * S;
    int m0, n0;
    tile_mn(tl, m0, n0);
    const int next_tile = tile + tile_step;
    const bool have_next = next_tile < tile_end;
    int nkt0 = 0, nkt1 = 0;
    if (have_next) slab_range(next_tile, nkt0, nkt1);
    for (int kt = kt0; kt < kt1; ++kt) {
      const bool last_k = kt + 1 == kt1;
      const bool more = !last_k || have_next;
      const int nlk = last_k ? nkt0 : kt + 1;
      if (pend) {
        if (grp == 0) phase_end();
        if constexpr (LNF) { stats_publish(); phase_end(); }
        epilogue(pm0, pn0, pks);
        init_acc();
        phase_end();
        if (grp == 1) phase_end();
        pend = false;
      }
      if (LNF && kt == kt0 && tile != tile_first) issue_consts(n0);
      read_frags(cur, 0);
      if (more) {
        if (last_k) setup_loader(next_tile);
        if (grp == 0) { issue_a(cur ^ 1, nlk, 0, A_IT); issue_w(cur ^ 1, nlk, 0, W_Q_R0); }
        else issue_a(cur ^ 1, nlk, 0, A_IT / 2);
      }
      asm volatile("s_waitcnt lgkmcnt(0)" ::: "memory");
      phase_end();
      mfma_half();
      phase_end();
      read_frags(cur, 1);
      if (grp == 0) {
        if (more) issue_w(cur ^ 1, nlk, W_Q_R0, W_Q);
        asm volatile("s_waitcnt lgkmcnt(0)" ::: "memory");
      } else {
        if (more) issue_a(cur ^ 1, nlk, A_IT / 2, A_IT);
        asm volatile("s_waitcnt lgkmcnt(0)" ::: "memory");
      }
      phase_end();
      mfma_half();
      asm volatile("s_waitcnt vmcnt(0)" ::: "memory");
      phase_end();
      if (last_k) { pend = true; pm0 = m0; pn0 = n0; pks = ks; }
      cur ^= 1;
    }
    if (!have_next) break;
    tile = next_tile; kt0 = nkt0; kt1 = nkt1;
  }
  if constexpr (LNF) { stats_publish(); phase_end(); }
  epilogue(pm0, pn0, pks);
  if (grp == 0) phase_end();
}

template <int BM, int WM, int WN, int AMODE, bool SPLITK, bool LNF = false>
int launch_pp(const MvdGemmArgs& a, hipStream_t s) {
  constexpr int LDS_BYTES = 2 * (BM * 128 + B_BYTES) + (LNF ? XCH_BYTES : 0);
  static bool init[16] = {};
  int dev = 0;
  (void)hipGetDevice(&dev);
  if (!init[dev & 15]) {
    hipError_t e = hipFuncSetAttribute(reinterpret_cast<const void*>(&gemm_pp_kernel<BM, WM, WN, AMODE, SPLITK, LNF>),
                                       hipFuncAttributeMaxDynamicSharedMemorySize, LDS_BYTES);
    if (e != hipSuccess) { mvd_set_error("gemm_pp: hipFuncSetAttribute: %s", hipGetErrorString(e)); return -2; }
    init[dev & 15] = true;
  }
  const int ntm = ((AMODE == 4 ? a.M / 4 : a.M) + BM - 1) / BM, ntn = a.N / BN;
  MvdGemmArgs b = a;
  b.walk_cg = SPLITK ? 0 : mvd_gemm_pp_walk(a);
  int grid = 256;
  const int ntiles = ntm * ntn * (a.splitk > 1 ? a.splitk : 1) * (AMODE == 4 ? 4 : 1);
  if (ntiles < grid) grid = ((ntiles + 7) / 8) * 8;
  g_mvd_last_gemm.tiles = ntiles; g_mvd_last_gemm.grid = grid; g_mvd_last_gemm.per_cu = 1;
  hipLaunchKernelGGL((gemm_pp_kernel<BM, WM, WN, AMODE, SPLITK, LNF>), dim3(grid), dim3(NT), LDS_BYTES, s, b);
  hipError_t e = hipGetLastError();
  if (e != hipSuccess) { mvd_set_error("gemm_pp launch: %s", hipGetErrorString(e)); return -3; }
  return 0;
}

template <int BM, int WM, int WN>
int launch_pp_mode(const MvdGemmArgs& a, hipStream_t s) {
  const bool sk = a.splitk > 1;
  if (a.seg[0].mode == MVD_A_DENSE) return sk ? launch_pp<BM, WM, WN, 0, true>(a, s) : launch_pp<BM, WM, WN, 0, false>(a, s);
  if (a.seg[0].ups == 2) {
    if (!mvd_gemm_pp_up4_applicable(a)) { mvd_set_error("gemm_pp: not a problem of the 2x2 sub-pixel upsampling convolution"); return -1; }
    g_mvd_up4_launches.fetch_add(1);
    return launch_pp<BM, WM, WN, 4, false>(a, s);
  }
  if (a.seg[0].ups) {
    if (a.nseg != 1) { mvd_set_error("gemm_pp: an upsampling convolution takes no shortcut segment"); return -1; }
    return sk ? launch_pp<BM, WM, WN, 3, true>(a, s) : launch_pp<BM, WM, WN, 3, false>(a, s);
  }
  if (a.nseg == 1) return sk ? launch_pp<BM, WM, WN, 1, true>(a, s) : launch_pp<BM, WM, WN, 1, false>(a, s);
  return sk ? launch_pp<BM, WM, WN, 2, true>(a, s) : launch_pp<BM, WM, WN, 2, false>(a, s);
}

}

int mvd_gemm_pp_walk(const MvdGemmArgs& a) {
  static const int on = MVD_ENV_INT("MVD_GEMM_PP_WALK", 1);
  if (!on || (mvd_debug_flags() & MVD_DBG_PP_ROW_MAJOR) || a.walk_cg < 0) return 0;
  if (a.walk_cg > 0) return a.walk_cg;
  if (a.seg[0].mode != MVD_A_DENSE || a.nseg != 1 || a.splitk > 1) return 0;
  const int ntm = (a.M + 255) / 256, ntn = a.N / BN;
  if (ntm % 8 || ntm < 64 || ntn < 8) return 0;
  const size_t panel = (size_t)BN * a.Ktot * 2;
  if (panel * ntn <= (size_t)(5 << 19)) return 0;
  int c = (int)(((size_t)7 << 18) / panel);
  if (c < 2) return 0;
  while (c > 1 && (ntn % c || 32 % c)) --c;
  return c >= 2 ? c : 0;
}

bool mvd_gemm_pp_applicable(const MvdGemmArgs& a) {
  constexpr int BM = 256;
  const size_t lim = (size_t)1 << 31;
  if (a.N % BN || a.Ktot % 64 || a.out_f32) return false;
  if (a.relu) return false;
  if ((size_t)a.N * a.ldw * 2 >= lim) return false;
  if ((size_t)(a.M + BM) * a.ldo * 2 >= lim || (a.res && (size_t)(a.M + BM) * a.ldres * 2 >= lim)) return false;
  if (a.splitk > 1 && (size_t)(a.M + BM) * a.N * 4 >= lim) return false;
  for (int i = 0; i < a.nseg; ++i) {
    const MvdASeg& g = a.seg[i];
    if (g.mode == MVD_A_DENSE) {
      if ((size_t)(a.M + BM) * (g.c0 > g.c1 ? g.c0 : g.c1) * 2 >= lim) return false;
    } else {
      const size_t bytes = (size_t)(a.M / a.rows_per_batch) * g.inH * g.inW * g.c0 * 2 + (size_t)(g.inW + 1) * g.c0 * 2;
      if (bytes + (size_t)3 * g.inW * g.c0 * 2 >= lim) return false;
      if (2 * g.inH >= 32768 || 2 * g.inW >= 32768) return false;
    }
  }
  return true;
}

bool mvd_gemm_pp_up4_applicable(const MvdGemmArgs& a) {
  const MvdASeg& g = a.seg[0];
  if (a.nseg != 1 || g.mode != MVD_A_CONV3 || g.ups != 2 || g.stride != 1 || g.asym || g.c1) return false;
  if (a.res || a.rowvec || a.splitk > 1 || a.geglu || a.ln_c1 || a.out_f32) return false;
  if (g.c0 <= 0 || g.c0 % 64 || g.ksize != 4 * g.c0 || a.Ktot != 4 * g.c0 || a.ldw != a.Ktot) return false;
  if (g.inH <= 0 || g.inW <= 0 || a.outH != 2 * g.inH || a.outW != 2 * g.inW || a.rows_per_batch != a.outH * a.outW || a.M % a.rows_per_batch) return false;
  if (!(g.inW % 16 == 0 || (g.inW == 8 && g.inH % 2 == 0))) return false;
  const size_t lim = (size_t)1 << 31;
  if ((size_t)4 * a.N * a.ldw * 2 >= lim) return false;
  if ((size_t)(a.M + 2 * a.outW + 16 + 256) * a.ldo * 2 >= lim) return false;
  return mvd_gemm_pp_applicable(a);
}

int mvd_launch_gemm_pp(const MvdGemmArgs& a, hipStream_t s) {
  if (a.ln_c1) {
    const MvdASeg& g = a.seg[0];
    if (a.nseg != 1 || g.mode != MVD_A_DENSE || g.c1 || a.splitk > 1 || a.res || a.rowvec || !a.bias) {
      mvd_set_error("gemm_pp: the LayerNorm fold takes one dense source, a bias, no residual / row vector / split-K"); return -1;
    }
    return a.geglu ? launch_pp<256, 4, 2, 0, false, true>(a, s) : launch_pp<256, 2, 4, 0, false, true>(a, s);
  }
  if (a.geglu) {
    if (a.seg[0].mode != MVD_A_DENSE || a.splitk > 1) { mvd_set_error("gemm_pp: GEGLU needs a dense, unsplit problem"); return -1; }
    return launch_pp<256, 4, 2, 0, false>(a, s);
  }
  return launch_pp_mode<256, 2, 4>(a, s);
}

bool mvd_gemm_ln_fold_ok(const MvdGemmArgs& a) {
  const MvdASeg& g = a.seg[0];
  if (a.nseg != 1 || g.mode != MVD_A_DENSE || g.c1 || a.splitk > 1 || a.res || a.rowvec || a.out_f32) return false;
  if (a.Ktot != g.c0 || a.Ktot > 640) return false;
  if (a.geglu && a.Ktot > 320) return false;
  const int cfg = mvd_gemm_pick_config(a);
  return (a.geglu ? cfg == 6 : cfg == 7) && mvd_gemm_pp_applicable(a);
}
```

### mvd_amd/csrc/gemm_xs.hip

```cpp
#include <stdio.h>
#include <stdlib.h>
#include <string.h>
#include "../../include/mvd_hip.h"
#include "kernels.h"
#include "bufaddr.h"

namespace {

#define XS_WAIT_VM(n) asm volatile("s_waitcnt vmcnt(" #n ")" ::: "memory")

template <int KS, bool GEGLU, bool RES, bool LN>
__global__ __launch_bounds__(256, 2) void gemm_xs_kernel(const MvdXsArgs a) {
  constexpr int NW = 4, RT = 2, NS = GEGLU ? 2 : 3;
  constexpr int STG = GEGLU ? 8192 : 4096;
  constexpr int UNIT = (KS + 1) * 1024;
  constexpr int P = KS / NW;
  static_assert(KS % NW == 0 && !(GEGLU && RES) && !(RES && LN), "shape of the instantiations");
  constexpr int E = 2 * RT + (RES ? 2 * RT : 0);
  extern __shared__ __attribute__((aligned(16))) unsigned char smem[];
  const int lane = threadIdx.x & 63;
  const int wave = __builtin_amdgcn_readfirstlane(threadIdx.x >> 6);
  const int r = lane & 31, h = lane >> 5;
#ifdef XS_DBG
  constexpr int dbg = XS_DBG;
#else
  constexpr int dbg = 0;
#endif

  int rb, cp;
  if (a.csplit == 1) { rb = blockIdx.x; cp = 0; }
  else {
    const int per = 8 * a.csplit, g = blockIdx.x / per, rem = blockIdx.x - g * per;
    rb = g * 8 + (rem & 7); cp = rem >> 3;
  }
  if (rb * 256 >= a.M) return;
  const int upp = a.units / a.csplit;
  const int u0 = cp * upp, nit = upp;
  const int row_w = rb * 256 + wave * (RT * 32);

  const __amdgpu_buffer_rsrc_t rs_w = buf_rsrc(a.w, a.units * UNIT);
  auto issue_unit = [&](int it, int stage) {
    unsigned char* dst = smem + stage * UNIT;
    const unsigned so = (unsigned)(u0 + it) * (unsigned)UNIT;
    if (dbg & 4) return;
#pragma unroll
    for (int i = 0; i < P; ++i) dma16(rs_w, dst + (wave * P + i) * 1024, (unsigned)lane * 16u, so + (unsigned)((wave * P + i) * 1024));
    dma4(rs_w, dst + KS * 1024 + wave * 256, (unsigned)lane * 4u, so + (unsigned)(KS * 1024 + wave * 256));
  };
  issue_unit(0, 0);
  if (NS == 3 && nit > 1) issue_unit(1, 1);

  const __amdgpu_buffer_rsrc_t rs_x = buf_rsrc(a.x, (int)((size_t)a.M * a.ldx * 2));
  u32x4 x[RT][KS];
#pragma unroll
  for (int t = 0; t < RT; ++t) {
    const int vo = (row_w + t * 32 + r) * a.ldx * 2 + h * 16;
#pragma unroll
    for (int s = 0; s < KS; ++s) x[t][s] = (dbg & 8) ? u32x4{0x3f803f80u, 0x3f803f80u, 0x3f803f80u, 0x3f803f80u} : __builtin_amdgcn_raw_buffer_load_b128(rs_x, vo + s * 32, 0, 0);
  }
  if constexpr (LN) {
    const float invk = 1.f / (float)(KS * 16);
    const bf16x2 ones2 = __builtin_bit_cast(bf16x2, 0x3f803f80u);
#pragma unroll
    for (int t = 0; t < RT; ++t) {
      float sm = 0.f, sq = 0.f;
#pragma unroll
      for (int s = 0; s < KS; ++s) {
        const unsigned d[4] = {x[t][s].x, x[t][s].y, x[t][s].z, x[t][s].w};
#pragma unroll
        for (int e = 0; e < 4; ++e) {
          const bf16x2 v = __builtin_bit_cast(bf16x2, d[e]);
          sq = __builtin_amdgcn_fdot2_f32_bf16(v, v, sq, false);
          sm = __builtin_amdgcn_fdot2_f32_bf16(v, ones2, sm, false);
        }
      }
      sm += __shfl_xor(sm, 32); sq += __shfl_xor(sq, 32);
      const float mean = sm * invk;
      const float rstd = rsqrtf(fmaxf(sq * invk - mean * mean, 0.f) + a.ln_eps);
      const float nb = -mean * rstd;
#pragma unroll
      for (int s = 0; s < KS; ++s) {
        const unsigned d[4] = {x[t][s].x, x[t][s].y, x[t][s].z, x[t][s].w};
        x[t][s] = u32x4{pack2bf(fmaf(bflo(d[0]), rstd, nb), fmaf(bfhi(d[0]), rstd, nb)), pack2bf(fmaf(bflo(d[1]), rstd, nb), fmaf(bfhi(d[1]), rstd, nb)),
                        pack2bf(fmaf(bflo(d[2]), rstd, nb), fmaf(bfhi(d[2]), rstd, nb)), pack2bf(fmaf(bflo(d[3]), rstd, nb), fmaf(bfhi(d[3]), rstd, nb))};
      }
    }
  }
  const u32x4 one_frag = {h == 0 ? 0x3f803f80u : 0u, 0u, 0u, 0u};

  const __amdgpu_buffer_rsrc_t rs_o = buf_rsrc(a.out, (int)((size_t)a.M * a.ldo * 2));
  __amdgpu_buffer_rsrc_t rs_r = rs_o;
  if (RES) rs_r = buf_rsrc(a.res, (int)((size_t)a.M * a.ldres * 2));
  int vo_r[RT];
#pragma unroll
  for (int t = 0; t < RT; ++t) {
    vo_r[t] = RES ? (row_w + t * 32 + r) * a.ldres * 2 + h * 32 : 0;
  }

#ifdef XS_STAMPS
  long long st_acc[6] = {0, 0, 0, 0, 0, 0};
  const long long st_begin = (long long)__builtin_amdgcn_s_memtime();
  const long long st_rbegin = (long long)__builtin_amdgcn_s_memrealtime();
  long long st_t = st_begin;
#define XS_STAMP(i) do { const long long n_ = (long long)__builtin_amdgcn_s_memtime(); st_acc[i] += n_ - st_t; st_t = n_; } while (0)
#else
#define XS_STAMP(i) do {} while (0)
#endif
  float gs[16 * RT];

  auto top = [&](int it, int stage) {
    XS_STAMP(4);
    if (it == 0) XS_WAIT_VM(0);
    else if constexpr (GEGLU) { if ((it & 3) == 0) XS_WAIT_VM(8); else XS_WAIT_VM(0); }
    else if (it == nit - 1) { if (RES) XS_WAIT_VM(16); else XS_WAIT_VM(8); }
    else { if (RES) XS_WAIT_VM(22); else XS_WAIT_VM(14); }
    static_assert(P + 1 == 6 && 2 * E == (RES ? 16 : 8), "the counted waits above are written for these instantiations");
    __builtin_amdgcn_sched_barrier(0);
    XS_STAMP(0);
    __builtin_amdgcn_s_barrier();
    __builtin_amdgcn_sched_barrier(0);
    XS_STAMP(1);
    if (it + NS - 1 < nit) issue_unit(it + NS - 1, NS == 2 ? (stage ^ 1) : (stage >= 1 ? stage - 1 : 2));
    __builtin_amdgcn_sched_barrier(0);
    XS_STAMP(2);
  };
  auto multiply = [&](int stage, f32x16 (&acc)[RT], float (&side)[16 * RT], bool with_side) {
    const unsigned char* sp = smem + stage * UNIT + lane * 16;
    if (!with_side) {
      {
        const bf16x8 wb = *reinterpret_cast<const bf16x8*>(sp + KS * 1024);
#pragma unroll
        for (int t = 0; t < RT; ++t) {
          f32x16 z;
#pragma unroll
          for (int q = 0; q < 16; ++q) z[q] = 0.f;
          acc[t] = __builtin_amdgcn_mfma_f32_32x32x16_bf16(wb, __builtin_bit_cast(bf16x8, one_frag), z, 0, 0, 0);
        }
      }
#pragma unroll
      for (int s = 0; s < KS; ++s) {
        const bf16x8 wf = *reinterpret_cast<const bf16x8*>(sp + s * 1024);
#pragma unroll
        for (int t = 0; t < RT; ++t)
          if (!(dbg & 2)) acc[t] = __builtin_amdgcn_mfma_f32_32x32x16_bf16(wf, __builtin_bit_cast(bf16x8, x[t][s]), acc[t], 0, 0, 0);
          else acc[t][s & 15] += __builtin_bit_cast(float, __builtin_bit_cast(u32x4, wf).x);
      }
    } else {
#pragma unroll
      for (int st = 0; st <= KS; ++st) {
        const bf16x8 wc = *reinterpret_cast<const bf16x8*>(sp + (st == 0 ? KS : st - 1) * 1024);
#ifndef XS_GELU_GROUP
#define XS_GELU_GROUP 2
#endif
        if (st % (XS_GELU_GROUP / 2) == 0 && !(dbg & 16)) {
#pragma unroll
          for (int e = 0; e < XS_GELU_GROUP; ++e) {
            const int v = (st / (XS_GELU_GROUP / 2)) * XS_GELU_GROUP + e;
            if (v < 16 * RT) side[v] = gelu_erf_f(side[v]);
          }
#pragma unroll
          for (int e = 0; e < XS_GELU_GROUP; ++e) {
            const int v = (st / (XS_GELU_GROUP / 2)) * XS_GELU_GROUP + e;
            if (v < 16 * RT) asm volatile("" : "+v"(side[v]));
          }
        }
#pragma unroll
        for (int t = 0; t < RT; ++t) {
// ... 43 lines not shown
  auto add_res = [&](f32x16& o, int t, int so) {
    const u32x4 r0 = __builtin_amdgcn_raw_buffer_load_b128(rs_r, vo_r[t], so, 0);
    const u32x4 r1 = __builtin_amdgcn_raw_buffer_load_b128(rs_r, vo_r[t] + 16, so, 0);
#pragma unroll
    for (int e = 0; e < 4; ++e) {
      o[2 * e] += bflo(r0[e]); o[2 * e + 1] += bfhi(r0[e]);
      o[8 + 2 * e] += bflo(r1[e]); o[8 + 2 * e + 1] += bfhi(r1[e]);
    }
  };
  auto store_pair = [&](int g, f32x16 (&v0)[RT], f32x16 (&v1)[RT]) {
#pragma unroll
    for (int t = 0; t < RT; ++t) {
      if (RES) { add_res(v0[t], t, g * 128); add_res(v1[t], t, g * 128 + 64); }
      stage_chunk(0, 2 * h, pack8(v0[t], 0)); stage_chunk(0, 2 * h + 1, pack8(v0[t], 1));
      stage_chunk(0, 4 + 2 * h, pack8(v1[t], 0)); stage_chunk(0, 4 + 2 * h + 1, pack8(v1[t], 1));
      flush_rows(t, 0, g * 128);
    }
    __builtin_amdgcn_sched_barrier(0);
  };
  auto stage_tile = [&](int half, const f32x16 (&v)[RT]) {
#pragma unroll
    for (int t = 0; t < RT; ++t) { stage_chunk(t, 4 * half + 2 * h, pack8(v[t], 0)); stage_chunk(t, 4 * half + 2 * h + 1, pack8(v[t], 1)); }
    __builtin_amdgcn_sched_barrier(0);
  };
  auto flush_group = [&](int g) {
#pragma unroll
    for (int t = 0; t < RT; ++t) flush_rows(t, t, g * 128);
    __builtin_amdgcn_sched_barrier(0);
  };

#ifdef XS_STAMPS
  const long long st_prolog = (long long)__builtin_amdgcn_s_memtime() - st_begin;
  st_t = (long long)__builtin_amdgcn_s_memtime();
#endif
  int stage = 0;
  if constexpr (!GEGLU) {
    for (int it = 0; it < nit; it += 2) {
      f32x16 acc0[RT], acc1[RT];
      top(it, stage);
      multiply(stage, acc0, gs, false);
      stage = stage == NS - 1 ? 0 : stage + 1;
      top(it + 1, stage);
      multiply(stage, acc1, gs, false);
      stage = stage == NS - 1 ? 0 : stage + 1;
      store_pair((u0 + it) >> 1, acc0, acc1);
    }
  } else {
    for (int it = 0; it < nit; it += 2) {
      {
        top(it, stage);
        f32x16 gg[RT];
        multiply(stage, gg, gs, false);
#pragma unroll
        for (int t = 0; t < RT; ++t)
#pragma unroll
          for (int q = 0; q < 16; ++q) gs[t * 16 + q] = gg[t][q];
        stage = stage == NS - 1 ? 0 : stage + 1;
      }
      {
        top(it + 1, stage);
        f32x16 acc[RT];
        multiply(stage, acc, gs, true);
#pragma unroll
        for (int t = 0; t < RT; ++t)
#pragma unroll
          for (int q = 0; q < 16; ++q) acc[t][q] *= gs[t * 16 + q];
        stage_tile((it >> 1) & 1, acc);
        if (it & 2) flush_group((u0 + it) >> 2);
        stage = stage == NS - 1 ? 0 : stage + 1;
      }
    }
  }
#ifdef XS_STAMPS
  XS_STAMP(4);
  if (wave == 0 && lane == 0) {
    asm volatile("s_waitcnt vmcnt(0)" ::: "memory");
    long long* dst = reinterpret_cast<long long*>(a.out + (size_t)a.M * a.ldo) + (size_t)blockIdx.x * 8;
    for (int i = 0; i < 5; ++i) dst[i] = st_acc[i];
    dst[5] = (long long)__builtin_amdgcn_s_memrealtime() - st_rbegin; dst[6] = (long long)__builtin_amdgcn_s_memtime() - st_begin; dst[7] = st_rbegin; (void)st_prolog;
  }
#endif
}

template <int KS, bool GEGLU, bool RES, bool LN>
int launch_xs(const MvdXsArgs& a, hipStream_t s) {
  constexpr int LDS_BYTES = (GEGLU ? 2 : 3) * (KS + 1) * 1024 + 4 * (GEGLU ? 8192 : 4096);
  static bool init[16] = {};
  int dev = 0;
  (void)hipGetDevice(&dev);
  if (!init[dev & 15]) {
    hipError_t e = hipFuncSetAttribute(reinterpret_cast<const void*>(&gemm_xs_kernel<KS, GEGLU, RES, LN>), hipFuncAttributeMaxDynamicSharedMemorySize, LDS_BYTES);
    if (e != hipSuccess) { mvd_set_error("gemm_xs: hipFuncSetAttribute: %s", hipGetErrorString(e)); return -2; }
    init[dev & 15] = true;
    if (MVD_ENV_INT("MVD_XS_TRACE", 0)) {
      int occ = -1;
      (void)hipOccupancyMaxActiveBlocksPerMultiprocessor(&occ, reinterpret_cast<const void*>(&gemm_xs_kernel<KS, GEGLU, RES, LN>), 256, LDS_BYTES);
      fprintf(stderr, "gemm_xs<%d,%d,%d,%d>: %d workgroups per CU by the occupancy query (LDS %d B)\n", KS, (int)GEGLU, (int)RES, (int)LN, occ, LDS_BYTES);
    }
  }
  const int nrb = (a.M + 255) / 256;
  const int grid = a.csplit == 1 ? nrb : ((nrb + 7) / 8) * 8 * a.csplit;
  g_mvd_last_gemm.cfg = 9; g_mvd_last_gemm.splitk = 1; g_mvd_last_gemm.tiles = nrb * a.csplit; g_mvd_last_gemm.grid = grid; g_mvd_last_gemm.per_cu = 2;
  hipLaunchKernelGGL((gemm_xs_kernel<KS, GEGLU, RES, LN>), dim3(grid), dim3(256), LDS_BYTES, s, a);
  hipError_t e = hipGetLastError();
  if (e != hipSuccess) { mvd_set_error("gemm_xs launch: %s", hipGetErrorString(e)); return -3; }
  return 0;
}

}

bool mvd_gemm_xs_applicable(const MvdXsArgs& a) {
  const size_t lim = (size_t)1 << 31;
  if (a.K != 320 || a.units <= 0 || a.M <= 0 || a.relu) return false;
  if (a.units % (a.geglu ? 4 : 2)) return false;
  if ((a.geglu || a.ln) && a.res) return false;
  if ((size_t)(a.M + 256) * a.ldx * 2 >= lim || (size_t)(a.M + 256) * a.ldo * 2 >= lim) return false;
  if (a.res && (size_t)(a.M + 256) * a.ldres * 2 >= lim) return false;
  if ((size_t)a.units * 21 * 1024 >= lim) return false;
  if ((a.ldx & 7) || (a.ldo & 7) || (a.res && (a.ldres & 7))) return false;
  return true;
}

int mvd_gemm_xs_pick_csplit(const MvdXsArgs& a) {
  const int nrb = (a.M + 255) / 256;
  const int groups = a.units / (a.geglu ? 4 : 2);
  int cs = 1;
  while (nrb * cs < 1024 && groups % (cs * 2) == 0 && groups / (cs * 2) >= 3) cs *= 2;
  return cs;
}

int mvd_launch_gemm_xs(const MvdXsArgs& a_in, hipStream_t s) {
  MvdXsArgs a = a_in;
  if (a.csplit <= 0) a.csplit = mvd_gemm_xs_pick_csplit(a);
  const int groups = a.units / (a.geglu ? 4 : 2);
  if (!mvd_gemm_xs_applicable(a) || groups % a.csplit) {
    mvd_set_error("gemm_xs: M=%d K=%d units=%d geglu=%d csplit=%d is not a shape of the X-stationary kernels", a.M, a.K, a.units, a.geglu, a.csplit);
    return -1;
  }
  if (a.geglu) return a.ln ? launch_xs<20, true, false, true>(a, s) : launch_xs<20, true, false, false>(a, s);
  if (a.res) return launch_xs<20, false, true, false>(a, s);
  return a.ln ? launch_xs<20, false, false, true>(a, s) : launch_xs<20, false, false, false>(a, s);
}

extern "C" int mvd_op_linear_xs(const void* x, int ldx, const void* w_packed, int m, int k, int units, int geglu, int ln, float ln_eps,
                                const void* res, int ldres, void* out, int ldo, int csplit, void* stream) {
  MvdXsArgs a; memset(&a, 0, sizeof(a));
  a.x = (const bf16_t*)x; a.ldx = ldx; a.w = (const bf16_t*)w_packed; a.M = m; a.K = k; a.units = units; a.geglu = geglu;
  a.ln = ln; a.ln_eps = ln_eps; a.res = (const bf16_t*)res; a.ldres = ldres; a.out = (bf16_t*)out; a.ldo = ldo; a.csplit = csplit;
  if (!x || !w_packed || !out) { mvd_set_error("mvd_op_linear_xs: null operand"); return -1; }
  return mvd_launch_gemm_xs(a, (hipStream_t)stream);
}
```

### mvd_amd/csrc/kernels.h

```cpp
#pragma once
#include <hip/hip_runtime.h>
#include <stdint.h>
#include <atomic>
#include "common.h"
#include "../../include/mvd_hip.h"

enum { MVD_A_DENSE = 0, MVD_A_CONV3 = 1 };

struct MvdASeg {
  const bf16_t* p0;
  const bf16_t* p1;
  int c0, c1;
  int mode;
  int ksize;
  int inH, inW;
  int stride;
  int ups;
  int asym;
};

struct MvdGemmArgs {
  MvdASeg seg[2];
  int nseg;
  const bf16_t* W;
  int ldw;
  int M, N, Ktot;
  int rows_per_batch;
  int outH, outW;
  const float* bias;
  const float* rowvec;
  int ld_rowvec;
  const bf16_t* res;
  int ldres;
  float alpha;
  int geglu;
  void* out;
  int ldo;
  int out_f32;
  int splitk;
  float* part;
  int w_blocked;
  int splitk_nowait;
  unsigned int* tile_cnt;
  int dbg;
  int relu;
  const float* ln_c1;
  float ln_eps;
  int walk_cg;
};
static_assert(sizeof(MvdGemmArgs) == 280, "MvdGemmArgs is a kernel argument: a size change moves the hidden arguments of every GEMM kernel");

int mvd_launch_gemm(const MvdGemmArgs& a, hipStream_t s, int force_cfg = -1);
int mvd_gemm_pick_config(const MvdGemmArgs& a);
int mvd_launch_gemm_relu(const MvdGemmArgs& a, hipStream_t s, int cfg, bool glds);
int mvd_launch_splitk_reduce_relu(const MvdGemmArgs& a, hipStream_t s, int grid);
struct MvdLaunchPlan { int cfg, splitk, tiles, grid, per_cu, nowait; };
extern thread_local MvdLaunchPlan g_mvd_last_gemm;
extern std::atomic<long> g_mvd_up4_launches;
bool mvd_gemm_pp_applicable(const MvdGemmArgs& a);
bool mvd_gemm_pp_up4_applicable(const MvdGemmArgs& a);
int mvd_gemm_pp_walk(const MvdGemmArgs& a);
int mvd_debug_flags();
bool mvd_gemm_ln_fold_ok(const MvdGemmArgs& a);
int mvd_launch_gemm_pp(const MvdGemmArgs& a, hipStream_t s);
int mvd_launch_gemm_ring(const MvdGemmArgs& a, hipStream_t s);
bool mvd_gemm_sm_applicable(const MvdGemmArgs& a, int tile);
int mvd_launch_gemm_sm(const MvdGemmArgs& a, hipStream_t s, int tile, int nstage);
bool mvd_gemm_sm_plan(const MvdGemmArgs& a, int* tile, int* nstage, int* splitk);
struct MvdXsArgs {
  const bf16_t* x; int ldx;
  const bf16_t* w;
  int M, K, units;
  int geglu;
  int ln; float ln_eps;
  const bf16_t* res; int ldres;
  bf16_t* out; int ldo;
  int csplit;
  int relu;
};
bool mvd_gemm_xs_applicable(const MvdXsArgs& a);
int mvd_gemm_xs_pick_csplit(const MvdXsArgs& a);
int mvd_launch_gemm_xs(const MvdXsArgs& a, hipStream_t s);
struct MvdWsArgs {
  const bf16_t* x; int B, H, W, C;
  int ups;
  const bf16_t* sc0; const bf16_t* sc1; int scc0, scc1;
  const bf16_t* w;
  const float* bias;
  const float* rowvec; int ld_rowvec;
  const bf16_t* res; int ldres;
  bf16_t* out; int ldo;
  int M, N;
  int variant;
  int relu;
};
bool mvd_conv_ws_applicable(const MvdWsArgs& a);
size_t mvd_conv_ws_packed_elems(int C, int sc, int N);
int mvd_launch_conv_ws(const MvdWsArgs& a, hipStream_t s);
#define MVD_OP_SPLITK_COUNTERS 4096
int mvd_launch_splitk_reduce(const MvdGemmArgs& a, hipStream_t s);
int mvd_gemm_pick_splitk(const MvdGemmArgs& a);

struct MvdAttnProblem {
  const bf16_t* q; const bf16_t* k; const bf16_t* v; bf16_t* o;
  int ldq, ldk, ldv, ldo;
  int64_t bsq, bsk, bsv, bso;
  int nq, nk;
};
struct MvdAttnArgs {
  MvdAttnProblem p[2];
  int nprob;
  int batch, heads;
  float scale;
  int prescaled;
  int dbg;
  int nsplit;
  void* split_ws;
  unsigned int* split_cnt;
};
int mvd_attention_pick_split(const MvdAttnArgs& a);
size_t mvd_attention_split_ws_bytes(const MvdAttnArgs& a, int nsplit);
int mvd_attention_split_counters(const MvdAttnArgs& a);
int mvd_launch_attention(const MvdAttnArgs& a, hipStream_t s);

#define MVD_GN_MAXCHUNK 256
int mvd_launch_groupnorm(const bf16_t* x0, const bf16_t* x1, int c0, int c1, int batch, int hw, int groups,
                         float eps, const float* gamma, const float* beta, int silu, bf16_t* y, float* ws,
                         hipStream_t s);
int mvd_launch_layernorm(const bf16_t* x, int rows, int c, float eps, const float* gamma, const float* beta,
                         bf16_t* y, hipStream_t s);
int mvd_launch_refnorm(const bf16_t* x, int batch, int hw, int c, bf16_t* y, hipStream_t s);
int mvd_launch_refstats(const bf16_t* x, int batch, int hw, int c, float* stats , hipStream_t s);
int mvd_launch_refapply(const bf16_t* x, int batch, int hw, int c, const float* mean_k , bf16_t* y, hipStream_t s);

int mvd_launch_nchw_to_nhwc(const float* x, int batch, int c, int hw, const float* scale, const float* shift,
                            int ld_ss, bf16_t* y, hipStream_t s);
int mvd_launch_film(const bf16_t* x, int batch, int hw, int c, const float* scale, const float* shift, int ld_ss,
                    bf16_t* y, hipStream_t s);
int mvd_launch_conv_in(const bf16_t* x, int batch, int h, int w, int cin, const float* wt, const float* bias,
                       int cout, bf16_t* y, hipStream_t s);
int mvd_launch_conv_out(const bf16_t* x, int batch, int h, int w, int c, const bf16_t* wt, const float* bias,
                        int cout, float* y, hipStream_t s);
int mvd_launch_im2col_in(const float* x, int batch, int c, int h, int w, const float* scale, const float* shift, int ld_ss,
                         bf16_t* y, hipStream_t s);
int mvd_launch_f32_to_bf16(const float* x, int64_t n, bf16_t* y, hipStream_t s);
int mvd_launch_nhwc_to_nchw_f32(const bf16_t* x, int batch, int hw, int c, float* y, hipStream_t s);
int mvd_launch_maxpool2x2(const bf16_t* x, int batch, int h, int w, int c, bf16_t* y, hipStream_t s);

int mvd_launch_skinny_linear(const float* x, int ldx, int batch, int k, const void* w, int wbf16, const float* bias,
                             int n, int act_in, float* y, int ldy, hipStream_t s);
struct MvdSegTable { int n; int end[16]; };
int mvd_launch_skinny_linear_grouped(const float* x, int ldx, int xseg, int batch, int k, const float* w, const float* bias, int n,
                                     const MvdSegTable& seg, float* y, int ldy, hipStream_t s);
int mvd_launch_film_params_grouped(const float* raw, int batch, const MvdSegTable& seg, float strength, float* out, int out_rows,
                                   hipStream_t s);
int mvd_launch_layernorm_f32(const float* x, int rows, int c, float eps, const float* gamma, const float* beta,
                             int silu, float* y, hipStream_t s, int nseg = 1);
int mvd_launch_timestep_embedding(const float* t, int batch, int dim, float* y, hipStream_t s);
int mvd_launch_camera_features(const float* src, const float* tgt, int batch, int cam_rows, int nfreq,
                               float max_freq, float* rflat, float* enc, hipStream_t s);
int mvd_launch_film_params(const float* raw, int batch, int dim, float strength, float* scale, float* shift, int out_rows,
                           hipStream_t s);

int mvd_launch_film_nchw_f32(const float* x, int batch, int c, int hw, const float* scale, const float* shift, float* y,
                             hipStream_t s);

void mvd_set_error(const char* fmt, ...);

enum MvdProfClass {
  MVD_PC_GEMM_256X160 = 0, MVD_PC_GEMM_256X128 = 1, MVD_PC_GEMM_128X160 = 2, MVD_PC_GEMM_128X128 = 3, MVD_PC_GEMM_128X64 = 4,
  MVD_PC_GEMM_64X64 = 5,
  MVD_PC_PP_GEGLU = 6, MVD_PC_PP_DENSE = 7,
  MVD_PC_ATTN_1WAVE = 8, MVD_PC_ATTN_2WAVE = 9, MVD_PC_ATTN_4WAVE = 10, MVD_PC_ATTN_8WAVE = 11,
  MVD_PC_GEMM_128X320 = 12,
  MVD_PC_PP_CONV3 = 13, MVD_PC_PP_SPLITK = 14, MVD_PC_PP_LN_DENSE = 15,
  MVD_PC_GROUPNORM = 16, MVD_PC_LAYERNORM = 17,
  MVD_PC_SM_64X64 = 20, MVD_PC_SM_128X64 = 21, MVD_PC_SM_64X128 = 22, MVD_PC_SM_128X128 = 23, MVD_PC_SM_64X160 = 24,
  MVD_PC_SM_128X160 = 25, MVD_PC_SM_64X320 = 26,
  MVD_PC_XS_DENSE = 30, MVD_PC_XS_RESIDUAL = 31, MVD_PC_XS_LN_DENSE = 32, MVD_PC_XS_GEGLU = 33,
  MVD_PC_CONV_WS = 34
};
```

### mvd_amd/csrc/norm.hip

```cpp
#include <stdlib.h>
#include "kernels.h"
#include "bufaddr.h"

namespace {

MVD_DEVINL void unpack8(const u32x4 v, float* f) {
  f[0] = bflo(v[0]); f[1] = bfhi(v[0]); f[2] = bflo(v[1]); f[3] = bfhi(v[1]);
  f[4] = bflo(v[2]); f[5] = bfhi(v[2]); f[6] = bflo(v[3]); f[7] = bfhi(v[3]);
}
MVD_DEVINL u32x4 pack8(const float* f) {
  return u32x4{pack2bf(f[0], f[1]), pack2bf(f[2], f[3]), pack2bf(f[4], f[5]), pack2bf(f[6], f[7])};
}

__global__ void gn_stats_kernel(const bf16_t* __restrict__ x0, const bf16_t* __restrict__ x1, int c0, int c1, int hw,
                                int groups, int rows_per_chunk, int R, float* __restrict__ ws) {
  extern __shared__ __attribute__((aligned(16))) float sh[];
  const int C = c0 + c1, vec = C >> 3;
  const int b = blockIdx.y, chunk = blockIdx.x, nchunk = gridDim.x;
  const int v = threadIdx.x % vec, r = threadIdx.x / vec;
  const int row0 = chunk * rows_per_chunk;
  const int row1 = min(hw, row0 + rows_per_chunk);
  const int ch = v * 8;
  const bool first = ch < c0;
  const bf16_t* src = first ? x0 + (size_t)b * hw * c0 + ch : x1 + (size_t)b * hw * c1 + (ch - c0);
// ... 207 lines not shown
#pragma unroll
  for (int k = 0; k < 4; ++k) { if (2 * k < kb) q0 += pq[k]; else q1 += pq[k]; }
  reduce_groups(q0, q1, s_rstd, true);
  if (!active) return;
  float ga[8], gb[8];
  {
    const f32x4 g0 = *reinterpret_cast<const f32x4*>(gamma + ch), g1 = *reinterpret_cast<const f32x4*>(gamma + ch + 4);
    const f32x4 b0 = *reinterpret_cast<const f32x4*>(beta + ch), b1 = *reinterpret_cast<const f32x4*>(beta + ch + 4);
    const float r0 = s_rstd[glo], r1 = s_rstd[glo + 1 < gpw ? glo + 1 : glo];
#pragma unroll
    for (int j = 0; j < 8; ++j) {
      const float gm = j < 4 ? g0[j] : g1[j - 4], bt = j < 4 ? b0[j] : b1[j - 4];
      ga[j] = gm * (j < kb ? r0 : r1);
      gb[j] = bt - (j < kb ? m0 : m1) * ga[j];
    }
  }
  __amdgpu_buffer_rsrc_t rs_y = buf_rsrc(y + (size_t)b * hw * C, hw * C * 2);
  const unsigned voy = (unsigned)(pl * C + ch) * 2u;
  const int sty = npl * C * 2;
#pragma unroll
  for (int i = 0; i < NV; ++i) {
    if (i < nval) {
      const unsigned w[4] = {d[i].x, d[i].y, d[i].z, d[i].w};
      u32x4 o;
#pragma unroll
      for (int k = 0; k < 4; ++k) {
        float lo = fmaf(bflo(w[k]), ga[2 * k], gb[2 * k]), hi = fmaf(bfhi(w[k]), ga[2 * k + 1], gb[2 * k + 1]);
        if (silu) { lo = silu_f(lo); hi = silu_f(hi); }
        o[k] = pack2bf(lo, hi);
      }
      store16(o, rs_y, voy, i * sty);
    }
    __builtin_amdgcn_sched_barrier(0);
  }
}

template <int MAXV>
__global__ __launch_bounds__(256) void ln_kernel(const bf16_t* __restrict__ x, int rows, int c, float eps,
                                                  const float* __restrict__ gamma, const float* __restrict__ beta,
                                                  bf16_t* __restrict__ y) {
  const int lane = threadIdx.x & 63;
  const int row = blockIdx.x * 4 + (threadIdx.x >> 6);
  if (row >= rows) return;
  const int vec = c >> 3;
  float f[MAXV][8];
  float s = 0.f;
#pragma unroll
  for (int i = 0; i < MAXV; ++i) {
    const int v = lane + i * 64;
    if (v < vec) {
      unpack8(*reinterpret_cast<const u32x4*>(x + (size_t)row * c + v * 8), f[i]);
#pragma unroll
      for (int j = 0; j < 8; ++j) s += f[i][j];
    }
  }
  const float mean = wave_sum(s) / (float)c;
  float q = 0.f;
#pragma unroll
  for (int i = 0; i < MAXV; ++i) {
    const int v = lane + i * 64;
    if (v < vec) {
#pragma unroll
      for (int j = 0; j < 8; ++j) { const float d = f[i][j] - mean; q = fmaf(d, d, q); }
    }
  }
  const float rstd = rsqrtf(wave_sum(q) / (float)c + eps);
#pragma unroll
  for (int i = 0; i < MAXV; ++i) {
    const int v = lane + i * 64;
    if (v < vec) {
      float o[8];
      const f32x4 g0 = *reinterpret_cast<const f32x4*>(gamma + v * 8), g1 = *reinterpret_cast<const f32x4*>(gamma + v * 8 + 4);
      const f32x4 b0 = *reinterpret_cast<const f32x4*>(beta + v * 8), b1 = *reinterpret_cast<const f32x4*>(beta + v * 8 + 4);
#pragma unroll
      for (int j = 0; j < 4; ++j) {
        o[j] = (f[i][j] - mean) * rstd * g0[j] + b0[j];
        o[j + 4] = (f[i][j + 4] - mean) * rstd * g1[j] + b1[j];
      }
      *reinterpret_cast<u32x4*>(y + (size_t)row * c + v * 8) = pack8(o);
    }
  }
}

__global__ __launch_bounds__(256) void refnorm_kernel(const bf16_t* __restrict__ x, int batch, int hw, int c,
                                                      bf16_t* __restrict__ y) {
  __shared__ float red[8];
  const int p = blockIdx.x;
  const int vec = c >> 3;
  const int total = batch * vec;
  const int lane = threadIdx.x & 63, wave = threadIdx.x >> 6;
  auto block_sum = [&](float v) -> float {
    v = wave_sum(v);
    __syncthreads();
    if (lane == 0) red[wave] = v;
    __syncthreads();
    return red[0] + red[1] + red[2] + red[3];
  };
  float s = 0.f;
  for (int e = threadIdx.x; e < total; e += 256) {
    const int b = e / vec, v = e % vec;
    float f[8];
    unpack8(*reinterpret_cast<const u32x4*>(x + ((size_t)b * hw + p) * c + v * 8), f);
#pragma unroll
    for (int j = 0; j < 8; ++j) s += f[j];
  }
  const float n = (float)batch * (float)c;
  const float mean = block_sum(s) / n;
  float q = 0.f;
  for (int e = threadIdx.x; e < total; e += 256) {
    const int b = e / vec, v = e % vec;
    float f[8];
    unpack8(*reinterpret_cast<const u32x4*>(x + ((size_t)b * hw + p) * c + v * 8), f);
#pragma unroll
    for (int j = 0; j < 8; ++j) { const float d = f[j] - mean; q = fmaf(d, d, q); }
  }
  const float var = block_sum(q) / (n - 1.0f);
  const float k = 0.5f / fmaxf(sqrtf(var), 1e-6f);
  for (int e = threadIdx.x; e < total; e += 256) {
    const int b = e / vec, v = e % vec;
    float f[8];
    const size_t off = ((size_t)b * hw + p) * c + v * 8;
    unpack8(*reinterpret_cast<const u32x4*>(x + off), f);
#pragma unroll
    for (int j = 0; j < 8; ++j) f[j] = (f[j] - mean) * k;
    *reinterpret_cast<u32x4*>(y + off) = pack8(f);
  }
}

__global__ __launch_bounds__(256) void refstats_kernel(const bf16_t* __restrict__ x, int batch, int hw, int c, float* __restrict__ stats) {
  __shared__ float red[8];
  const int p = blockIdx.x;
  const int vec = c >> 3;
  const int total = batch * vec;
  const int lane = threadIdx.x & 63, wave = threadIdx.x >> 6;
  auto block_sum = [&](float v) -> float {
    v = wave_sum(v);
    __syncthreads();
    if (lane == 0) red[wave] = v;
    __syncthreads();
    return red[0] + red[1] + red[2] + red[3];
  };
  float s = 0.f;
  for (int e = threadIdx.x; e < total; e += 256) {
    const int b = e / vec, v = e % vec;
    float f[8];
    unpack8(*reinterpret_cast<const u32x4*>(x + ((size_t)b * hw + p) * c + v * 8), f);
#pragma unroll
    for (int j = 0; j < 8; ++j) s += f[j];
  }
  const float mean = block_sum(s) / ((float)batch * (float)c);
  float q = 0.f;
  for (int e = threadIdx.x; e < total; e += 256) {
    const int b = e / vec, v = e % vec;
    float f[8];
    unpack8(*reinterpret_cast<const u32x4*>(x + ((size_t)b * hw + p) * c + v * 8), f);
#pragma unroll
    for (int j = 0; j < 8; ++j) { const float d = f[j] - mean; q = fmaf(d, d, q); }
  }
  const float m2 = block_sum(q);
  if (threadIdx.x == 0) { stats[2 * p] = mean; stats[2 * p + 1] = m2; }
}

__global__ __launch_bounds__(256) void refapply_kernel(const bf16_t* __restrict__ x, int batch, int hw, int c,
                                                       const float* __restrict__ mean_k, bf16_t* __restrict__ y) {
  const int vec = c >> 3;
  const long total = (long)batch * hw * vec;
  for (long e = (long)blockIdx.x * 256 + threadIdx.x; e < total; e += (long)gridDim.x * 256) {
    const int p = (int)((e / vec) % hw);
    const float mean = mean_k[2 * p], k = mean_k[2 * p + 1];
    float f[8];
    unpack8(*reinterpret_cast<const u32x4*>(x + e * 8), f);
#pragma unroll
    for (int j = 0; j < 8; ++j) f[j] = (f[j] - mean) * k;
    *reinterpret_cast<u32x4*>(y + e * 8) = pack8(f);
  }
}

__global__ __launch_bounds__(256) void ln_f32_kernel(const float* __restrict__ x, int c, float eps,
                                                      const float* __restrict__ gamma, const float* __restrict__ beta,
                                                      int silu, float* __restrict__ y, int nseg) {
  __shared__ float red[8];
  const int row = blockIdx.x;
  gamma += (size_t)(row % nseg) * c; beta += (size_t)(row % nseg) * c;
  const int lane = threadIdx.x & 63, wave = threadIdx.x >> 6;
  auto block_sum = [&](float v) -> float {
    v = wave_sum(v);
    __syncthreads();
    if (lane == 0) red[wave] = v;
    __syncthreads();
    return red[0] + red[1] + red[2] + red[3];
  };
  const float* xr = x + (size_t)row * c;
  float s = 0.f;
  for (int i = threadIdx.x; i < c; i += 256) s += xr[i];
  const float mean = block_sum(s) / (float)c;
  float q = 0.f;
  for (int i = threadIdx.x; i < c; i += 256) { const float d = xr[i] - mean; q = fmaf(d, d, q); }
  const float rstd = rsqrtf(block_sum(q) / (float)c + eps);
  for (int i = threadIdx.x; i < c; i += 256) {
    float t = (xr[i] - mean) * rstd * gamma[i] + beta[i];
    y[(size_t)row * c + i] = silu ? silu_f(t) : t;
  }
}

}

static thread_local int g_last_gn[6] = {0, 0, 0, 0, 0, 0};

static int check_launch(const char* what) {
  hipError_t e = hipGetLastError();
  if (e != hipSuccess) { mvd_set_error("%s launch: %s", what, hipGetErrorString(e)); return -3; }
  return 0;
}

static bool launch_gn_slice(const bf16_t* x0, const bf16_t* x1, int c0, int c1, int batch, int hw, int groups, float eps,
                            const float* gamma, const float* beta, int silu, bf16_t* y, hipStream_t s) {
  static const int enable = MVD_ENV_INT("MVD_GN_SLICE", 1);
  const int C = c0 + c1, cg = C / groups;
  if (!enable || cg < 8 || (cg & 1)) return false;
  int gpw = 1;
  while (gpw <= groups && ((gpw * cg) % 8 || groups % gpw)) gpw <<= 1;
  if (gpw > groups) return false;
  const int cs = gpw * cg, nvec = cs / 8, nslice = groups / gpw;
  int threads = 1024, nv = 0;
  for (int th : {256, 512, 1024}) {
    const int npl = th / nvec;
    if (npl < 1) continue;
    threads = th; nv = (hw + npl - 1) / npl;
    if (nv <= 4) break;
  }
  if (nv < 1 || nv > 21) return false;
  const long slice_bytes = (long)hw * cs * 2, nwg = (long)batch * nslice;
  const long min_wg = (mvd_debug_flags() & MVD_DBG_GN_ONE_PASS) ? 8 : 128;
  if (slice_bytes > 96 * 1024 && nwg < min_wg) return false;
  const dim3 grid((unsigned)nwg), blk((unsigned)threads);
  g_last_gn[0] = 1; g_last_gn[2] = threads; g_last_gn[3] = gpw; g_last_gn[4] = threads / nvec; g_last_gn[5] = 0;
#define GN_SLICE(NVT) do { g_last_gn[1] = NVT; \
    hipLaunchKernelGGL(gn_slice_kernel<NVT>, grid, blk, 0, s, x0, x1, c0, c1, batch, hw, groups, gpw, eps, gamma, beta, silu, y); } while (0)
  if (nv <= 2) GN_SLICE(2); else if (nv <= 4) GN_SLICE(4); else if (nv <= 8) GN_SLICE(8); else if (nv <= 16) GN_SLICE(16); else GN_SLICE(21);
#undef GN_SLICE
  return true;
}

int mvd_launch_groupnorm(const bf16_t* x0, const bf16_t* x1, int c0, int c1, int batch, int hw, int groups, float eps,
                         const float* gamma, const float* beta, int silu, bf16_t* y, float* ws, hipStream_t s) {
  const int C = c0 + c1;
  if (!x0 || (c1 && !x1) || !y || !ws || !gamma || !beta || batch <= 0 || hw <= 0 || groups <= 0 || groups > 32 ||
      (C % groups) || (c0 % 8) || (c1 % 8) || C > 8192) {
    mvd_set_error("groupnorm: bad arguments (c0=%d c1=%d batch=%d hw=%d groups=%d)", c0, c1, batch, hw, groups);
    return -1;
  }
  if (launch_gn_slice(x0, x1, c0, c1, batch, hw, groups, eps, gamma, beta, silu, y, s)) return check_launch("gn_slice");
  const int vec = C / 8;
  if (vec > 1024) { mvd_set_error("groupnorm: C=%d too wide", C); return -1; }
  const int R = vec >= 256 ? 1 : 256 / vec;
  const int threads = ((vec * R + 63) / 64) * 64;
  static const int rows_target = MVD_ENV_INT("MVD_GN_ROWS", 128);
  int nchunk = hw / rows_target;
#ifndef MVD_GN_MINBLOCKS
#define MVD_GN_MINBLOCKS 64
#endif
  if ((long)nchunk * batch < MVD_GN_MINBLOCKS) nchunk = (MVD_GN_MINBLOCKS + batch - 1) / batch;
  if (nchunk > hw / 8) nchunk = hw / 8;
  nchunk = nchunk < 1 ? 1 : (nchunk > MVD_GN_MAXCHUNK ? MVD_GN_MAXCHUNK : nchunk);
  const int rpc = (hw + nchunk - 1) / nchunk;
  nchunk = (hw + rpc - 1) / rpc;
  const size_t sh1 = (size_t)R * C * 2 * sizeof(float);
  hipLaunchKernelGGL(gn_stats_kernel, dim3(nchunk, batch), dim3(threads), sh1, s, x0, x1, c0, c1, hw, groups, rpc, R, ws);
  if (int r = check_launch("gn_stats")) return r;
  static const long per_blk_env = MVD_ENV_INT("MVD_GN_APPLY_ELEMS", 65536);
  long per_blk = per_blk_env;
  const long total_el = (long)batch * hw * C;
  if (total_el / per_blk < 1024) per_blk = total_el / 1024 < 2048 ? 2048 : total_el / 1024;
  int rows_per_blk = (int)((per_blk + C - 1) / C);
  if (rows_per_blk < 1) rows_per_blk = 1;
  if (rows_per_blk > hw) rows_per_blk = hw;
  const int nblk = (hw + rows_per_blk - 1) / rows_per_blk;
  const size_t sh2 = (size_t)(2 * groups + 2 * C) * sizeof(float);
  g_last_gn[0] = 2; g_last_gn[1] = R; g_last_gn[2] = threads; g_last_gn[3] = nchunk; g_last_gn[4] = rpc; g_last_gn[5] = rows_per_blk;
  hipLaunchKernelGGL(gn_apply_kernel, dim3(nblk, batch), dim3(256), sh2, s, x0, x1, c0, c1, hw, groups, nchunk, rpc, eps, gamma,
                     beta, silu, ws, rows_per_blk, y);
  return check_launch("gn_apply");
}

extern "C" int mvd_debug_last_groupnorm_plan(int* out) {
  if (!out) { mvd_set_error("last_groupnorm_plan: null argument"); return -1; }
  for (int i = 0; i < 6; ++i) out[i] = g_last_gn[i];
  return 0;
}

int mvd_launch_layernorm(const bf16_t* x, int rows, int c, float eps, const float* gamma, const float* beta, bf16_t* y,
                         hipStream_t s) {
  if (!x || !y || !gamma || !beta || rows <= 0 || c <= 0 || (c % 8) || c > 64 * 8 * 4) {
    mvd_set_error("layernorm: bad arguments rows=%d c=%d", rows, c);
    return -1;
  }
  const int grid = (rows + 3) / 4;
  if (c <= 512) hipLaunchKernelGGL(ln_kernel<1>, dim3(grid), dim3(256), 0, s, x, rows, c, eps, gamma, beta, y);
  else if (c <= 1024) hipLaunchKernelGGL(ln_kernel<2>, dim3(grid), dim3(256), 0, s, x, rows, c, eps, gamma, beta, y);
  else hipLaunchKernelGGL(ln_kernel<4>, dim3(grid), dim3(256), 0, s, x, rows, c, eps, gamma, beta, y);
  return check_launch("layernorm");
}

int mvd_launch_refstats(const bf16_t* x, int batch, int hw, int c, float* stats, hipStream_t s) {
  if (!x || !stats || batch <= 0 || hw <= 0 || c <= 0 || (c % 8)) { mvd_set_error("refstats: bad arguments"); return -1; }
  hipLaunchKernelGGL(refstats_kernel, dim3(hw), dim3(256), 0, s, x, batch, hw, c, stats);
  return check_launch("refstats");
}
int mvd_launch_refapply(const bf16_t* x, int batch, int hw, int c, const float* mean_k, bf16_t* y, hipStream_t s) {
  if (!x || !y || !mean_k || batch <= 0 || hw <= 0 || c <= 0 || (c % 8)) { mvd_set_error("refapply: bad arguments"); return -1; }
  const long total = (long)batch * hw * (c >> 3);
  long grid = (total + 255) / 256; if (grid > 4096) grid = 4096;
  hipLaunchKernelGGL(refapply_kernel, dim3((unsigned)grid), dim3(256), 0, s, x, batch, hw, c, mean_k, y);
  return check_launch("refapply");
}
int mvd_launch_refnorm(const bf16_t* x, int batch, int hw, int c, bf16_t* y, hipStream_t s) {
  if (!x || !y || batch <= 0 || hw <= 0 || c <= 0 || (c % 8)) { mvd_set_error("refnorm: bad arguments"); return -1; }
  hipLaunchKernelGGL(refnorm_kernel, dim3(hw), dim3(256), 0, s, x, batch, hw, c, y);
  return check_launch("refnorm");
}

int mvd_launch_layernorm_f32(const float* x, int rows, int c, float eps, const float* gamma, const float* beta, int silu,
                             float* y, hipStream_t s, int nseg) {
  if (!x || !y || !gamma || !beta || rows <= 0 || c <= 0 || nseg < 1) { mvd_set_error("layernorm_f32: bad arguments"); return -1; }
  hipLaunchKernelGGL(ln_f32_kernel, dim3(rows), dim3(256), 0, s, x, c, eps, gamma, beta, silu, y, nseg);
  return check_launch("layernorm_f32");
}
```

### mvd_amd/ops.py

```python
from __future__ import annotations

import ctypes as C
from typing import Optional

import torch

from . import _lib as L


def _p(t: Optional[torch.Tensor]):
    if t is None:
        return None
    assert t.is_cuda and t.is_contiguous(), "ops expect contiguous CUDA tensors"
    return C.c_void_p(t.data_ptr())


def _s():
    return C.c_void_p(torch.cuda.current_stream().cuda_stream)


def _bf16(*ts):
    for t in ts:
        if t is not None:
            assert t.dtype == torch.bfloat16, "expected bf16"


def _blocked(w, blocked, k, force_cfg):
    if blocked is None:
        return w.shape[0], force_cfg
    n, kb = blocked
    assert kb == k and w.numel() == n * k and n % 32 == 0 and k % 64 == 0, (tuple(w.shape), blocked, k)
    assert force_cfg >= 100, "the blocked weight layout is read by the small-M kernels only (force_cfg = 100 + 10 * tile + depth)"
    return n, force_cfg + 1000


def linear(a, w, bias=None, a2=None, rowvec=None, rows_per_batch=0, res=None, alpha=1.0, geglu=False,
           out_f32=False, force_cfg=-1, splitk=1, blocked=None):
    _bf16(a, a2, w, res)
    m, k1 = a.shape
    k2 = a2.shape[1] if a2 is not None else 0
    assert blocked is not None or w.shape[1] == k1 + k2
    n, force_cfg = _blocked(w, blocked, k1 + k2, force_cfg)
    on = n // 2 if geglu else n
    out = torch.empty(m, on, device=a.device, dtype=torch.float32 if out_f32 else torch.bfloat16)
    ws = torch.empty(splitk * m * n + 4096, device=a.device, dtype=torch.float32) if splitk > 1 else None
    L.call("mvd_op_linear", _p(a), _p(a2), k1, k2, _p(w), _p(bias), _p(rowvec),
           rowvec.shape[1] if rowvec is not None else 0, rows_per_batch, _p(res), float(alpha), int(geglu),
           _p(out), int(out_f32), m, n, force_cfg, splitk, _p(ws), _s())
    return out


def ln_linear(x, w_folded, cf, eps=1e-5, geglu=False):
    _bf16(x, w_folded)
    m, k = x.shape
    n = w_folded.shape[0]
    assert w_folded.shape[1] == k and cf.shape == (2, n) and cf.dtype == torch.float32 and cf.is_contiguous()
    out = torch.empty(m, n // 2 if geglu else n, device=x.device, dtype=torch.bfloat16)
    L.call("mvd_op_ln_linear", _p(x), k, _p(w_folded), _p(cf[0]), _p(cf[1]), float(eps), int(geglu), _p(out), m, n, _s())
    return out


def linear_xs(x, w_packed, geglu=False, ln=False, eps=1e-5, res=None, csplit=0, k=None):
    _bf16(x, w_packed, res)
    m = x.shape[0]
    units, ks1 = w_packed.shape[0], w_packed.shape[1]
    k = (ks1 - 1) * 16 if k is None else k
    n_out = units * 16 if geglu else units * 32
    out = torch.empty(m, n_out, device=x.device, dtype=torch.bfloat16)
    assert x.stride(1) == 1 and (res is None or res.stride(1) == 1)
    L.call("mvd_op_linear_xs", C.c_void_p(x.data_ptr()), x.stride(0), _p(w_packed), m, k, units, int(geglu), int(ln), float(eps),
           C.c_void_p(res.data_ptr()) if res is not None else None, res.stride(0) if res is not None else 0, _p(out), n_out,
           csplit, _s())
    return out


def conv3x3_ws(x, w_packed, bias, n, rowvec=None, res=None, shortcut=None, shortcut2=None, variant=0, upsample=False):
    _bf16(x, w_packed, res, shortcut, shortcut2)
    b, h, w, c = x.shape
    out = torch.empty(b, 2 * h if upsample else h, 2 * w if upsample else w, n, device=x.device, dtype=torch.bfloat16)
    assert bias.dtype == torch.float32 and bias.numel() == n and x.is_contiguous()
    assert rowvec is None or (rowvec.dtype == torch.float32 and rowvec.stride(1) == 1)
    pp = lambda t: C.c_void_p(t.data_ptr()) if t is not None else None
    L.call("mvd_op_conv3x3_ws", _p(x), b, h, w, c, _p(w_packed), _p(bias), pp(rowvec), rowvec.stride(0) if rowvec is not None else 0,
           pp(res), pp(shortcut), pp(shortcut2), shortcut.shape[-1] if shortcut is not None else 0,
           shortcut2.shape[-1] if shortcut2 is not None else 0, _p(out), n, int(variant) + (16 if upsample else 0), _s())
    return out


def conv3x3(x, w_packed, bias=None, stride=1, upsample=False, rowvec=None, res=None, shortcut=None,
            shortcut2=None, force_cfg=-1, splitk=1, asym_pad=False, blocked=None):
    _bf16(x, w_packed, res, shortcut, shortcut2)
    B, H, W, Cin = x.shape
    ktot = 9 * Cin + (shortcut.shape[-1] if shortcut is not None else 0) + (shortcut2.shape[-1] if shortcut2 is not None else 0)
    cout, force_cfg = _blocked(w_packed, blocked, ktot, force_cfg)
    oh = H * 2 if upsample else (H + 1) // 2 if stride == 2 else H
    ow = W * 2 if upsample else (W + 1) // 2 if stride == 2 else W
    out = torch.empty(B, oh, ow, cout, device=x.device, dtype=torch.bfloat16)
    c1 = shortcut.shape[-1] if shortcut is not None else 0
    c2 = shortcut2.shape[-1] if shortcut2 is not None else 0
    ws = torch.empty(splitk * B * oh * ow * cout + 4096, device=x.device, dtype=torch.float32) if splitk > 1 else None
    L.call("mvd_op_conv3x3", _p(x), B, H, W, Cin, stride, int(upsample), int(asym_pad), _p(w_packed), _p(bias), _p(rowvec),
           rowvec.shape[1] if rowvec is not None else 0, _p(res), _p(shortcut), _p(shortcut2), c1, c2, _p(out), cout,
           force_cfg, splitk, _p(ws), _s())
    return out


def conv3x3_up4(x, w4, bias=None, force_cfg=-1):
    _bf16(x, w4)
    B, H, W, Cin = x.shape
    assert w4.dim() == 3 and w4.shape[0] == 4 and w4.shape[2] == 4 * Cin and w4.is_contiguous() and x.is_contiguous(), tuple(w4.shape)
    cout = w4.shape[1]
    out = torch.empty(B, 2 * H, 2 * W, cout, device=x.device, dtype=torch.bfloat16)
    L.call("mvd_op_conv3x3_up4", _p(x), B, H, W, Cin, _p(w4), _p(bias), _p(out), cout, force_cfg, _s())
    return out


def conv3x3_relu(x, w_packed, bias=None, relu=True, out_f32=False, force_cfg=-1, splitk=1):
    _bf16(x, w_packed)
    B, H, W, Cin = x.shape
    cout = w_packed.shape[0]
    assert w_packed.shape[1] == 9 * Cin, (tuple(w_packed.shape), Cin)
    out = torch.empty(B, H, W, cout, device=x.device, dtype=torch.float32 if out_f32 else torch.bfloat16)
    ws = torch.empty(splitk * B * H * W * cout, device=x.device, dtype=torch.float32) if splitk > 1 else None
    L.call("mvd_op_conv3x3_relu", _p(x), B, H, W, Cin, _p(w_packed), _p(bias), _p(out), cout, int(relu), int(out_f32), force_cfg,
           splitk, _p(ws), _s())
    return out


def linear_relu(a, w, bias=None, relu=True, out_f32=False, force_cfg=-1, splitk=1):
    _bf16(a, w)
    m, k = a.shape
    n = w.shape[0]
    assert w.shape[1] == k
    out = torch.empty(m, n, device=a.device, dtype=torch.float32 if out_f32 else torch.bfloat16)
    ws = torch.empty(splitk * m * n, device=a.device, dtype=torch.float32) if splitk > 1 else None
    L.call("mvd_op_linear_relu", _p(a), k, _p(w), _p(bias), _p(out), m, n, int(relu), int(out_f32), force_cfg, splitk, _p(ws), _s())
    return out


def maxpool2x2(x, out=None):
    _bf16(x)
    B, H, W, c = x.shape
    if out is None:
        out = torch.empty(B, H // 2, W // 2, c, device=x.device, dtype=torch.bfloat16)
    L.call("mvd_op_maxpool2x2", _p(x), B, H, W, c, _p(out), _s())
    return out


def sqdiff_mean(a, b, per_pair=False):
    _f32_same(a, b)
    pairs = a.shape[0]
    n = a.numel() // pairs
    nbytes = L.check(L.lib().mvd_op_sqdiff_mean_ws_bytes(pairs, n), "mvd_op_sqdiff_mean_ws_bytes")
    ws = torch.empty(nbytes, device=a.device, dtype=torch.uint8)
    mean = torch.empty((), device=a.device, dtype=torch.float32)
# ... 110 lines not shown
    assert f.dtype == torch.float32 and w.dtype == torch.float32 and f.dim() == 2 and w.dim() == 2 and f.shape[1] == w.shape[1]
    out = torch.empty(f.shape[0], w.shape[0], dtype=torch.float32, device=f.device)
    L.call("mvd_op_fc_logits", _p(f), f.shape[0], f.shape[1], _p(w), w.shape[0], _p(out), _s())
    return out


def inception_score_chunks(logits, perm, splits):
    assert logits.dtype == torch.float32 and logits.dim() == 2 and perm.dtype == torch.int32 and perm.shape == (logits.shape[0],)
    n, classes = logits.shape
    need = L.lib().mvd_op_inception_score_workspace_bytes(n, classes, int(splits))
    if need < 0:
        raise L.MvdError(f"mvd_op_inception_score_workspace_bytes: {L.last_error()}")
    ws = torch.empty(need, dtype=torch.uint8, device=logits.device)
    out = torch.empty(min(int(splits), n), dtype=torch.float64, device=logits.device)
    chunks = C.c_int(0)
    L.call("mvd_op_inception_score", _p(logits), n, classes, _p(perm), int(splits), _p(ws), need, _p(out), C.byref(chunks), _s())
    return out[:chunks.value]


def up4_launches() -> int:
    return int(L.lib().mvd_debug_up4_launches())


def attention(q, k, v, heads, scale=0.125):
    _bf16(q, k, v)
    B, nq, _ = q.shape
    nk = k.shape[1]
    assert q.stride(2) == 1 and k.stride(2) == 1 and v.stride(2) == 1
    assert q.stride(0) == nq * q.stride(1) and k.stride(0) == nk * k.stride(1) and v.stride(0) == nk * v.stride(1)
    out = torch.empty(B, nq, heads * 64, device=q.device, dtype=torch.bfloat16)
    L.call("mvd_op_attention", C.c_void_p(q.data_ptr()), C.c_void_p(k.data_ptr()), C.c_void_p(v.data_ptr()), _p(out),
           B, heads, nq, nk, q.stride(1), k.stride(1), v.stride(1), heads * 64, float(scale), _s())
    return out


def attention_causal(q, k, v, heads, scale=0.125):
    _bf16(q, k, v)
    B, n, _ = q.shape
    assert k.shape[1] == n and v.shape[1] == n
    assert q.stride(2) == 1 and k.stride(2) == 1 and v.stride(2) == 1
    assert q.stride(0) == n * q.stride(1) and k.stride(0) == n * k.stride(1) and v.stride(0) == n * v.stride(1)
    out = torch.empty(B, n, heads * 64, device=q.device, dtype=torch.bfloat16)
    L.call("mvd_op_attention_causal", C.c_void_p(q.data_ptr()), C.c_void_p(k.data_ptr()), C.c_void_p(v.data_ptr()), _p(out),
           B, heads, n, q.stride(1), k.stride(1), v.stride(1), heads * 64, float(scale), _s())
    return out


def attention_split(q, k, v, heads, nsplit):
    _bf16(q, k, v)
    B, nq, _ = q.shape
    nk = k.shape[1]
    out = torch.empty(B, nq, heads * 64, device=q.device, dtype=torch.bfloat16)
    ws = torch.empty(int(L.lib().mvd_op_attention_split_ws_bytes(B, heads, nq, nsplit)), device=q.device, dtype=torch.uint8)
    L.call("mvd_op_attention_split", C.c_void_p(q.data_ptr()), C.c_void_p(k.data_ptr()), C.c_void_p(v.data_ptr()), _p(out),
           B, heads, nq, nk, q.stride(1), k.stride(1), v.stride(1), heads * 64, nsplit, _p(ws), _s())
    return out


def groupnorm(x, gamma, beta, groups=32, eps=1e-5, silu=False, x2=None):
    _bf16(x, x2)
    B, hw, c0 = x.shape
    c1 = x2.shape[2] if x2 is not None else 0
    y = torch.empty(B, hw, c0 + c1, device=x.device, dtype=torch.bfloat16)
    ws = torch.empty(B * 256 * groups * 2, device=x.device, dtype=torch.float32)
    L.call("mvd_op_groupnorm", _p(x), _p(x2), c0, c1, B, hw, groups, float(eps), _p(gamma), _p(beta), int(silu), _p(y),
           _p(ws), _s())
    return y


def layernorm(x, gamma, beta, eps=1e-5):
    _bf16(x)
    rows, c = x.shape
    y = torch.empty_like(x)
    L.call("mvd_op_layernorm", _p(x), rows, c, float(eps), _p(gamma), _p(beta), _p(y), _s())
    return y


def refnorm(x):
    _bf16(x)
    B, hw, c = x.shape
    y = torch.empty_like(x)
    L.call("mvd_op_refnorm", _p(x), B, hw, c, _p(y), _s())
    return y


def film(x, scale, shift):
    _bf16(x)
    B, hw, c = x.shape
    y = torch.empty_like(x)
    L.call("mvd_op_film", _p(x), B, hw, c, _p(scale), _p(shift), _p(y), _s())
    return y


def conv_in(x, w, bias):
    B, H, W, cin = x.shape
    cout = w.shape[0]
    y = torch.empty(B, H, W, cout, device=x.device, dtype=torch.bfloat16)
    L.call("mvd_op_conv_in", _p(x), B, H, W, cin, _p(w), _p(bias), cout, _p(y), _s())
    return y


def conv_out(x, w, bias):
    B, H, W, c = x.shape
    cout = w.shape[0]
    y = torch.empty(B, cout, H, W, device=x.device, dtype=torch.float32)
    L.call("mvd_op_conv_out", _p(x), B, H, W, c, _p(w), _p(bias), cout, _p(y), _s())
    return y


def softmax_rows(s):
    assert s.dtype == torch.float32 and s.dim() == 2
    out = torch.empty(s.shape, device=s.device, dtype=torch.bfloat16)
    L.call("mvd_op_softmax_rows", _p(s), s.shape[0], s.shape[1], _p(out), _s())
    return out


def ddpm_step(model_out, sample, noise, c0, c1, c2, c3, sigma):
    assert model_out.dtype == torch.float32 and sample.dtype == torch.float32
    out = torch.empty_like(sample)
    L.call("mvd_op_ddpm_step", _p(model_out), _p(sample), _p(noise), float(c0), float(c1), float(c2), float(c3),
           float(sigma), _p(out), sample.numel(), _s())
    return out


def cfg_combine(uncond_cond, guidance_scale):
    assert uncond_cond.dtype == torch.float32 and uncond_cond.shape[0] % 2 == 0
    out = torch.empty((uncond_cond.shape[0] // 2,) + tuple(uncond_cond.shape[1:]), device=uncond_cond.device,
                      dtype=torch.float32)
    L.call("mvd_op_cfg_combine", _p(uncond_cond), float(guidance_scale), _p(out), out.numel(), _s())
    return out


def sampler_step(model_out, sample, a0, a1, p, q, r=0.0, sigma=0.0, x0_prev=None, noise=None, guidance_scale=None,
                 out=None, x0_out=None):
    guided = guidance_scale is not None
    assert model_out.dtype == torch.float32 and sample.dtype == torch.float32
    assert model_out.numel() == sample.numel() * (2 if guided else 1), (tuple(model_out.shape), tuple(sample.shape))
    for t in (x0_prev, noise, out, x0_out):
        assert t is None or (t.dtype == torch.float32 and t.numel() == sample.numel())
    if out is None:
        out = torch.empty_like(sample)
    L.call("mvd_op_sampler_step", _p(model_out), int(guided), float(guidance_scale) if guided else 0.0, _p(sample), _p(x0_prev),
           _p(noise), float(a0), float(a1), float(p), float(q), float(r), float(sigma), _p(out), _p(x0_out), sample.numel(), _s())
    return out


PREDICTION_TYPES = ("epsilon", "v_prediction", "sample")


def _f32_same(*ts):
    first = next(t for t in ts if t is not None)
    for t in ts:
        if t is not None and not (t.is_cuda and t.dtype == torch.float32 and t.is_contiguous() and t.shape == first.shape):
            raise L.MvdError(f"expected contiguous fp32 CUDA tensors of shape {tuple(first.shape)}, got "
                             f"{t.dtype} {tuple(t.shape)} on {t.device}")


def _timesteps_i32(timesteps, batch, device):
    t = torch.as_tensor(timesteps, device=device)
    if t.dim() == 0:
        t = t.expand(batch)
    if t.dim() != 1 or t.shape[0] != batch or t.is_floating_point():
        raise L.MvdError(f"timesteps: expected {batch} integers, got {t.dtype} {tuple(t.shape)}")
    return t.to(torch.int32).contiguous()


def add_noise(x0, noise, timesteps, sqrt_ac, sqrt_1mac, noisy=True, velocity=False):
    _f32_same(x0, noise)
    b = x0.shape[0]
    ts = _timesteps_i32(timesteps, b, x0.device)
    assert sqrt_ac.dtype == torch.float32 and sqrt_1mac.dtype == torch.float32 and sqrt_ac.numel() == sqrt_1mac.numel()
    yn = torch.empty_like(x0) if noisy else None
    yv = torch.empty_like(x0) if velocity else None
    L.call("mvd_op_add_noise", _p(x0), _p(noise), _p(ts), _p(sqrt_ac), _p(sqrt_1mac), sqrt_ac.numel(), _p(yn), _p(yv), b,
           x0.numel() // b, _s())
    return yn, yv


def noise_loss(pred, noise, timesteps, sqrt_ac, sqrt_1mac, snr, prediction_type="v_prediction", x0=None, noisy=None,
               snr_gamma=5.0, want_denoised=False):
    _f32_same(pred, noise, x0, noisy)
    if prediction_type not in PREDICTION_TYPES:
        raise L.MvdError(f"prediction_type={prediction_type!r}: expected one of {PREDICTION_TYPES}")
    b = pred.shape[0]
    per = pred.numel() // b
    ts = _timesteps_i32(timesteps, b, pred.device)
    for t in (sqrt_ac, sqrt_1mac, snr):
        assert t.dtype == torch.float32 and t.numel() == sqrt_ac.numel()
    nbytes = L.check(L.lib().mvd_op_noise_loss_ws_bytes(b, per), "mvd_op_noise_loss_ws_bytes")
    ws = torch.empty(nbytes, device=pred.device, dtype=torch.uint8)
    result = torch.empty(5, device=pred.device, dtype=torch.float32)
    den = torch.empty_like(pred) if want_denoised else None
    L.call("mvd_op_noise_loss", _p(pred), _p(noise), _p(x0), _p(noisy), _p(ts), _p(sqrt_ac), _p(sqrt_1mac), _p(snr), sqrt_ac.numel(),
           PREDICTION_TYPES.index(prediction_type), float(snr_gamma), _p(den), _p(result), b, per, _p(ws), nbytes, _s())
    return result, den


def image_metrics(x, y, data_range, ssim=True, per_image=False):
    _f32_same(x, y)
    if x.dim() != 4:
        raise L.MvdError(f"image_metrics: expected (N, C, H, W), got {tuple(x.shape)}")
    n, c, h, w = x.shape
    nbytes = L.check(L.lib().mvd_op_image_metrics_ws_bytes(n, c, h, w, int(ssim)), "mvd_op_image_metrics_ws_bytes")
    ws = torch.empty(nbytes, device=x.device, dtype=torch.uint8)
    result = torch.empty(3, device=x.device, dtype=torch.float32)
    pi = torch.empty(n, 2, device=x.device, dtype=torch.float32) if per_image else None
    L.call("mvd_op_image_metrics", _p(x), _p(y), n, c, h, w, float(data_range), int(ssim), _p(result), _p(pi), _p(ws), nbytes, _s())
    return result, pi


def skinny_linear(x, w, bias=None, silu_in=False):
    assert x.dtype == torch.float32 and x.is_cuda and x.dim() == 2 and w.dim() == 2 and w.shape[1] == x.shape[1]
    assert w.dtype in (torch.float32, torch.bfloat16) and x.is_contiguous() and w.is_contiguous()
    b, k = x.shape
    n = w.shape[0]
    y = torch.empty(b, n, device=x.device, dtype=torch.float32)
    L.call("mvd_op_skinny_linear", _p(x), k, b, k, _p(w), int(w.dtype == torch.bfloat16), _p(bias), n, int(silu_in), _p(y), n, _s())
    return y


def nchw_to_nhwc(x, scale=None, shift=None):
    B, c, H, W = x.shape
    y = torch.empty(B, H, W, c, device=x.device, dtype=torch.bfloat16)
    L.call("mvd_op_nchw_to_nhwc", _p(x), B, c, H * W, _p(scale), _p(shift), _p(y), _s())
    return y


def nhwc_to_nchw(x):
    _bf16(x)
    B, H, W, c = x.shape
    y = torch.empty(B, c, H, W, device=x.device, dtype=torch.float32)
    L.call("mvd_op_nhwc_to_nchw", _p(x), B, H * W, c, _p(y), _s())
    return y


def f32_to_bf16(x):
    assert x.dtype == torch.float32
    y = torch.empty(x.shape, device=x.device, dtype=torch.bfloat16)
    L.call("mvd_op_f32_to_bf16", _p(x), x.numel(), _p(y), _s())
    return y


def last_gemm_plan():
    out = (C.c_int * 5)()
    L.call("mvd_debug_last_gemm_plan", out)
    return dict(cfg=out[0], splitk=out[1], tiles=out[2], grid=out[3], per_cu=out[4], nowait=L.lib().mvd_debug_last_gemm_nowait())


def last_attention_plan():
    out = (C.c_int * 2)()
    L.call("mvd_debug_last_attention_plan", out)
    return dict(waves=out[0], workgroups=out[1])


def last_groupnorm_plan():
    out = (C.c_int * 6)()
    L.call("mvd_debug_last_groupnorm_plan", out)
    if out[0] == 1:
        return dict(form="slice", nv=out[1], threads=out[2], gpw=out[3], npl=out[4])
    if out[0] == 2:
        return dict(form="two_kernel", R=out[1], threads=out[2], nchunk=out[3], rows_per_chunk=out[4], apply_rows=out[5])
    return dict(form="none")


def engine_splitk(m, n, k, geglu=False, conv=False):
    if conv:
        return L.lib().mvd_debug_pick_splitk_conv(m, n, k)
    return L.lib().mvd_debug_pick_splitk(m, n, k, int(geglu))
```

Measured before the change: 532.0 forward-passes/s.

## Fuse reference norm into X-stationary ref_kv GEMM via per-pixel stats table

For the K=320 reference-feature path, the refnorm kernel and its materialized normalized tensor are replaced by a small stats kernel that writes per-pixel mean and scale into a table. The X-stationary GEMM then applies (x-mean)*k on load through a new LN==2 mode. This removes one full read and write of the activation plus one launch. The refnorm and refstats kernels are also templated on per-thread vector count, and the GEMM walk-order logic gains a debug override.

```diff
diff --git a/include/mvd_hip.h b/include/mvd_hip.h
--- a/include/mvd_hip.h
+++ b/include/mvd_hip.h
@@ -96,6 +96,8 @@
                      void* out, int m, int n, void* stream);
 int mvd_op_linear_xs(const void* x, int ldx, const void* w_packed, int m, int k, int units, int geglu, int ln, float ln_eps,
                      const void* res, int ldres, void* out, int ldo, int csplit, void* stream);
+int mvd_op_linear_xs_refstats(const void* x, int ldx, const void* w_packed, int m, int k, int units, const float* stats, int hw,
+                              void* out, int ldo, int csplit, void* stream);
 int mvd_op_conv3x3_ws(const void* x, int batch, int h, int w, int c, const void* w_packed, const float* bias, const float* rowvec,
                       int ld_rowvec, const void* res, const void* sc, const void* sc2, int sc_c1, int sc_c2, void* out, int n,
                       int variant, void* stream);
@@ -114,6 +116,7 @@
 int mvd_op_layernorm(const void* x, int rows, int c, float eps, const float* gamma, const float* beta, void* y,
                      void* stream);
 int mvd_op_refnorm(const void* x, int batch, int hw, int c, void* y, void* stream);
+int mvd_op_refstats(const void* x, int batch, int hw, int c, float* stats, int mean_k, void* stream);
 int mvd_op_film(const void* x, int batch, int hw, int c, const float* scale, const float* shift, void* y, void* stream);
 int mvd_op_conv_in(const void* x, int batch, int h, int w, int cin, const float* wt, const float* bias, int cout, void* y,
                    void* stream);
@@ -130,9 +133,13 @@
 int mvd_debug_last_attention_plan(int* out);
 int mvd_debug_last_groupnorm_plan(int* out);
 long mvd_debug_up4_launches(void);
+long mvd_debug_refnorm_fused_launches(void);
 int mvd_debug_last_gemm_nowait(void);
 int mvd_debug_pick_splitk(int m, int n, int k, int geglu);
 int mvd_debug_pick_splitk_conv(int m, int n, int k);
+int mvd_debug_last_gemm_walk(void);
+int mvd_debug_pp_walk(int m, int n, int k, int geglu, int splitk, int conv);
+int mvd_debug_set_pp_walk(int c);
 int mvd_gemm_sm_num_tiles(void);
 int mvd_debug_set_attention_nw(int nw_log2);
 typedef enum {
@@ -161,6 +168,8 @@
   MVD_DBG_FORK_LATE = 4194304,
   MVD_DBG_SKINNY_VECTOR = 8388608
 } mvd_debug_flag_t;
+#define MVD_DBG_ALL 16777215
+int mvd_debug_set_refnorm_two_kernels(int on);
 int mvd_debug_set_flags(int flags);
 
 int mvd_op_ddpm_step(const float* model_out, const float* sample, const float* noise, float c0, float c1, float c2,
diff --git a/mvd_amd/_lib.py b/mvd_amd/_lib.py
--- a/mvd_amd/_lib.py
+++ b/mvd_amd/_lib.py
@@ -130,6 +130,9 @@
                                    C.c_void_p, C.c_void_p, C.c_int, C.c_void_p, C.c_void_p, C.c_void_p]),
     "mvd_op_layernorm": (C.c_int, [C.c_void_p, C.c_int, C.c_int, C.c_float, C.c_void_p, C.c_void_p, C.c_void_p, C.c_void_p]),
     "mvd_op_refnorm": (C.c_int, [C.c_void_p, C.c_int, C.c_int, C.c_int, C.c_void_p, C.c_void_p]),
+    "mvd_op_refstats": (C.c_int, [C.c_void_p, C.c_int, C.c_int, C.c_int, C.c_void_p, C.c_int, C.c_void_p]),
+    "mvd_op_linear_xs_refstats": (C.c_int, [C.c_void_p, C.c_int, C.c_void_p, C.c_int, C.c_int, C.c_int, C.c_void_p, C.c_int, C.c_void_p,
+                                            C.c_int, C.c_int, C.c_void_p]),
     "mvd_op_film": (C.c_int, [C.c_void_p, C.c_int, C.c_int, C.c_int, C.c_void_p, C.c_void_p, C.c_void_p, C.c_void_p]),
     "mvd_op_conv_in": (C.c_int, [C.c_void_p, C.c_int, C.c_int, C.c_int, C.c_int, C.c_void_p, C.c_void_p, C.c_int, C.c_void_p, C.c_void_p]),
     "mvd_op_conv_out": (C.c_int, [C.c_void_p, C.c_int, C.c_int, C.c_int, C.c_int, C.c_void_p, C.c_void_p, C.c_int, C.c_void_p, C.c_void_p]),
@@ -141,9 +144,14 @@
     "mvd_gemm_num_configs": (C.c_int, []),
     "mvd_debug_last_gemm_plan": (C.c_int, [C.POINTER(C.c_int)]),
     "mvd_debug_up4_launches": (C.c_long, []),
+    "mvd_debug_refnorm_fused_launches": (C.c_long, []),
+    "mvd_debug_set_refnorm_two_kernels": (C.c_int, [C.c_int]),
     "mvd_op_conv3x3_up4": (C.c_int, [C.c_void_p, C.c_int, C.c_int, C.c_int, C.c_int, C.c_void_p, C.c_void_p, C.c_void_p, C.c_int, C.c_int,
                                      C.c_void_p]),
     "mvd_debug_last_gemm_nowait": (C.c_int, []),
+    "mvd_debug_last_gemm_walk": (C.c_int, []),
+    "mvd_debug_pp_walk": (C.c_int, [C.c_int, C.c_int, C.c_int, C.c_int, C.c_int, C.c_int]),
+    "mvd_debug_set_pp_walk": (C.c_int, [C.c_int]),
     "mvd_debug_last_attention_plan": (C.c_int, [C.POINTER(C.c_int)]),
     "mvd_debug_last_groupnorm_plan": (C.c_int, [C.POINTER(C.c_int)]),
     "mvd_debug_pick_splitk": (C.c_int, [C.c_int, C.c_int, C.c_int, C.c_int]),
diff --git a/mvd_amd/csrc/engine.hip b/mvd_amd/csrc/engine.hip
--- a/mvd_amd/csrc/engine.hip
+++ b/mvd_amd/csrc/engine.hip
@@ -12,8 +12,20 @@
 int mvd_launch_silu_to_bf16(const float* x, int64_t n, bf16_t* y, hipStream_t s);
 
 static int g_debug_flags = 0;
-extern "C" int mvd_debug_set_flags(int flags) { g_debug_flags = flags; return 0; }
+extern "C" int mvd_debug_set_flags(int flags) {
+  if (flags & ~MVD_DBG_ALL) {
+    mvd_set_error("mvd_debug_set_flags: unknown bits %d (flags %d)", flags & ~MVD_DBG_ALL, flags);
+    fprintf(stderr, "mvd_debug_set_flags: unknown bits %d in %d -- flags unchanged\n", flags & ~MVD_DBG_ALL, flags);
+    return -1;
+  }
+  g_debug_flags = flags;
+  return 0;
+}
 int mvd_debug_flags() { return g_debug_flags; }
+static std::atomic<long> g_refnorm_fused_launches{0};
+static std::atomic<int> g_refnorm_two_kernels{0};
+extern "C" int mvd_debug_set_refnorm_two_kernels(int on) { g_refnorm_two_kernels.store(on ? 1 : 0); return 0; }
+extern "C" long mvd_debug_refnorm_fused_launches(void) { return g_refnorm_fused_launches.load(); }
 
 namespace {
 
@@ -249,16 +261,21 @@
   }
 
   int try_xs(const bf16_t* x, int K, int M, const std::string& slot, int64_t n_full, int N, bool geglu, bool ln,
-             const bf16_t* res, int ldres, void* out, int ldo, int set_override = -1) {
+             const bf16_t* res, int ldres, void* out, int ldo, int set_override = -1, float* ref_table = nullptr, int ref_hw = 0) {
     if (err) return err;
     if (dry || (g_debug_flags & MVD_DBG_NO_XS) || K != 320 || slot.empty() || !has(slot, set_override)) return 0;
     MvdXsArgs a; memset(&a, 0, sizeof(a));
     a.x = x; a.ldx = K; a.M = M; a.K = K; a.units = N / 32; a.geglu = geglu; a.ln = ln; a.ln_eps = 1e-5f;
     a.res = res; a.ldres = ldres; a.out = (bf16_t*)out; a.ldo = ldo;
+    if (ref_table) {
+      if (ln || geglu || res || ref_hw <= 0 || M % ref_hw) return 0;
+      a.ln = 2; a.row_stats = ref_table; a.stats_hw = ref_hw;
+    }
     if (N % 64 || !mvd_gemm_xs_applicable(a)) return 0;
     if ((long)((M + 255) / 256) * mvd_gemm_xs_pick_csplit(a) < 448) return 0;
     a.w = WB(slot, (n_full / 32) * 21 * 512, set_override);
     if (!a.w) return err;
+    if (ref_table) { if (int r = mvd_launch_refstats(x, M / ref_hw, ref_hw, K, ref_table, s, 1)) return err = r; }
     e->prof_M = M; e->prof_N = N; e->prof_K = K; e->prof_tag = geglu * 10 + (ln ? 1 : 0);
     const int r = profiled(geglu ? MVD_PC_XS_GEGLU : (res ? MVD_PC_XS_RESIDUAL : (ln ? MVD_PC_XS_LN_DENSE : MVD_PC_XS_DENSE)), 2.0 * M * (double)N * K, 0.0, [&] { return mvd_launch_gemm_xs(a, s); });
     return r ? r : 1;
@@ -554,12 +571,21 @@
     if (o.capture) {
       const size_t mk = c.e->tmp.off;
       bf16_t* rn = c.talloc<bf16_t>((size_t)M * C);
+      float* rtab = c.talloc<float>((size_t)2 * hw);
       if (o.defer_norm) {
         if (!c.dry && !c.err) CHECK(mvd_launch_refstats(out.p, B_, hw, C, o.stats + 2 * c.e->feat_pixel_off(feat_idx), c.s));
       } else {
-        if (!c.dry && !c.err) CHECK(mvd_launch_refnorm(out.p, B_, hw, C, rn, c.s));
-        CHECK(c.linear(rn, nullptr, C, 0, M, c.WB(key + ".ref_kv.w", (int64_t)4 * C * C, 0), nullptr, 4 * C, nullptr, 0, c.e->refkv[feat_idx], 4 * C, false, false, 0,
-                       key + ".ref_kv.wx", 0));
+        int fused = 0;
+        if (!g_refnorm_two_kernels.load()) {
+          fused = c.try_xs(out.p, C, M, key + ".ref_kv.wx", 4 * C, 4 * C, false, false, nullptr, 0, c.e->refkv[feat_idx], 4 * C, 0, rtab, hw);
+          if (fused < 0) return fused;
+          if (fused) g_refnorm_fused_launches.fetch_add(1);
+        }
+        if (!fused) {
+          if (!c.dry && !c.err) CHECK(mvd_launch_refnorm(out.p, B_, hw, C, rn, c.s));
+          CHECK(c.linear(rn, nullptr, C, 0, M, c.WB(key + ".ref_kv.w", (int64_t)4 * C * C, 0), nullptr, 4 * C, nullptr, 0, c.e->refkv[feat_idx], 4 * C, false, false, 0,
+                         key + ".ref_kv.wx", 0));
+        }
         if (c.e->dual_now && !c.dry && !c.err && hipEventRecord(c.e->feat_ev[feat_idx], c.s) != hipSuccess) { mvd_set_error("forward: hipEventRecord failed"); return -3; }
       }
       if (c.e->rc_keep && !c.dry && !c.err)
@@ -1378,6 +1404,9 @@
 int mvd_op_refnorm(const void* x, int batch, int hw, int c, void* y, void* stream) {
   return mvd_launch_refnorm((const bf16_t*)x, batch, hw, c, (bf16_t*)y, (hipStream_t)stream);
 }
+int mvd_op_refstats(const void* x, int batch, int hw, int c, float* stats, int mean_k, void* stream) {
+  return mvd_launch_refstats((const bf16_t*)x, batch, hw, c, stats, (hipStream_t)stream, mean_k ? 1 : 0);
+}
 int mvd_op_film(const void* x, int batch, int hw, int c, const float* scale, const float* shift, void* y, void* stream) {
   return mvd_launch_film((const bf16_t*)x, batch, hw, c, scale, shift, c, (bf16_t*)y, (hipStream_t)stream);
 }
diff --git a/mvd_amd/csrc/gemm.hip b/mvd_amd/csrc/gemm.hip
--- a/mvd_amd/csrc/gemm.hip
+++ b/mvd_amd/csrc/gemm.hip
@@ -3,7 +3,7 @@
 #include "kernels.h"
 #include "gemm_tile.h"
 
-thread_local MvdLaunchPlan g_mvd_last_gemm = {-1, 1, 0, 0, 0, 0};
+thread_local MvdLaunchPlan g_mvd_last_gemm = {-1, 1, 0, 0, 0, 0, 0};
 
 namespace {
 
@@ -80,6 +80,7 @@
 extern "C" long mvd_debug_up4_launches(void) { return g_mvd_up4_launches.load(); }
 
 extern "C" int mvd_debug_last_gemm_nowait(void) { return g_mvd_last_gemm.nowait; }
+extern "C" int mvd_debug_last_gemm_walk(void) { return g_mvd_last_gemm.walk; }
 
 static int deep_conv_split(const MvdGemmArgs& a, long t7) {
   static const int on = MVD_ENV_INT("MVD_GEMM_DEEP_CONV_SPLIT", 1);
@@ -162,7 +163,7 @@
                     a.seg[0].inH, a.seg[0].inW, a.seg[0].c0, a.N, force_cfg);
       return -1;
     }
-    g_mvd_last_gemm.cfg = 7; g_mvd_last_gemm.splitk = 1;
+    g_mvd_last_gemm.cfg = 7; g_mvd_last_gemm.splitk = 1; g_mvd_last_gemm.walk = 0;
     return mvd_launch_gemm_pp(a, s);
   }
   int cfg = force_cfg;
@@ -190,7 +191,7 @@
     if ((cfg != 6 && cfg != 7) || legacy || a.dbg || !mvd_gemm_ln_fold_ok(a)) { mvd_set_error("gemm: LayerNorm fold not available for M=%d N=%d K=%d cfg=%d", a.M, a.N, a.Ktot, cfg); return -1; }
   }
   if (cfg < 0 || cfg >= kNumCfgs || a.N % kCfgs[cfg].bn || (a.geglu && !kCfgs[cfg].tn_even)) { mvd_set_error("gemm: no tile config for N=%d geglu=%d cfg=%d", a.N, a.geglu, cfg); return -1; }
-  g_mvd_last_gemm.cfg = cfg; g_mvd_last_gemm.splitk = a.splitk > 1 ? a.splitk : 1;
+  g_mvd_last_gemm.cfg = cfg; g_mvd_last_gemm.splitk = a.splitk > 1 ? a.splitk : 1; g_mvd_last_gemm.walk = 0;
 #ifndef MVD_PROBE
   if (cfg == 0 || cfg == 1 || cfg == 8 || force_cfg == 16 || force_cfg == 17) { mvd_set_error("gemm: tile config %d exists in probe builds only", force_cfg >= 0 ? force_cfg : cfg); return -1; }
 #endif
diff --git a/mvd_amd/csrc/gemm_pp.hip b/mvd_amd/csrc/gemm_pp.hip
--- a/mvd_amd/csrc/gemm_pp.hip
+++ b/mvd_amd/csrc/gemm_pp.hip
@@ -575,7 +575,7 @@
   int grid = 256;
   const int ntiles = ntm * ntn * (a.splitk > 1 ? a.splitk : 1) * (AMODE == 4 ? 4 : 1);
   if (ntiles < grid) grid = ((ntiles + 7) / 8) * 8;
-  g_mvd_last_gemm.tiles = ntiles; g_mvd_last_gemm.grid = grid; g_mvd_last_gemm.per_cu = 1;
+  g_mvd_last_gemm.tiles = ntiles; g_mvd_last_gemm.grid = grid; g_mvd_last_gemm.per_cu = 1; g_mvd_last_gemm.walk = b.walk_cg;
   hipLaunchKernelGGL((gemm_pp_kernel<BM, WM, WN, AMODE, SPLITK, LNF>), dim3(grid), dim3(NT), LDS_BYTES, s, b);
   hipError_t e = hipGetLastError();
   if (e != hipSuccess) { mvd_set_error("gemm_pp launch: %s", hipGetErrorString(e)); return -3; }
@@ -601,19 +601,33 @@
 
 }
 
+static std::atomic<int> g_pp_walk_request{0};
+extern "C" int mvd_debug_set_pp_walk(int c) {
+  if (c < 0 || c > 32) { mvd_set_error("set_pp_walk: c = %d (0: the rule; 1..32: column tiles per group)", c); return -1; }
+  g_pp_walk_request.store(c);
+  return 0;
+}
 int mvd_gemm_pp_walk(const MvdGemmArgs& a) {
   static const int on = MVD_ENV_INT("MVD_GEMM_PP_WALK", 1);
   if (!on || (mvd_debug_flags() & MVD_DBG_PP_ROW_MAJOR) || a.walk_cg < 0) return 0;
-  if (a.walk_cg > 0) return a.walk_cg;
   if (a.seg[0].mode != MVD_A_DENSE || a.nseg != 1 || a.splitk > 1) return 0;
   const int ntm = (a.M + 255) / 256, ntn = a.N / BN;
-  if (ntm % 8 || ntm < 64 || ntn < 8) return 0;
+  if (ntm % 8) return 0;
+  const int forced = a.walk_cg > 0 ? a.walk_cg : g_pp_walk_request.load();
+  if (forced > 0) return ntn % forced ? 0 : forced;
+  if (ntm < 64 || ntn < 8) return 0;
   const size_t panel = (size_t)BN * a.Ktot * 2;
   if (panel * ntn <= (size_t)(5 << 19)) return 0;
   int c = (int)(((size_t)7 << 18) / panel);
   if (c < 2) return 0;
   while (c > 1 && (ntn % c || 32 % c)) --c;
   return c >= 2 ? c : 0;
+}
+extern "C" int mvd_debug_pp_walk(int m, int n, int k, int geglu, int splitk, int conv) {
+  MvdGemmArgs a; memset(&a, 0, sizeof(a));
+  a.M = m; a.N = n; a.Ktot = k; a.geglu = geglu; a.splitk = splitk; a.nseg = 1; a.seg[0].mode = conv ? MVD_A_CONV3 : MVD_A_DENSE;
+  if (n <= 0 || n % BN) return 0;
+  return mvd_gemm_pp_walk(a);
 }
 
 bool mvd_gemm_pp_applicable(const MvdGemmArgs& a) {
diff --git a/mvd_amd/csrc/gemm_xs.hip b/mvd_amd/csrc/gemm_xs.hip
--- a/mvd_amd/csrc/gemm_xs.hip
+++ b/mvd_amd/csrc/gemm_xs.hip
@@ -9,13 +9,13 @@
 
 #define XS_WAIT_VM(n) asm volatile("s_waitcnt vmcnt(" #n ")" ::: "memory")
 
-template <int KS, bool GEGLU, bool RES, bool LN>
+template <int KS, bool GEGLU, bool RES, int LN>
 __global__ __launch_bounds__(256, 2) void gemm_xs_kernel(const MvdXsArgs a) {
   constexpr int NW = 4, RT = 2, NS = GEGLU ? 2 : 3;
   constexpr int STG = GEGLU ? 8192 : 4096;
   constexpr int UNIT = (KS + 1) * 1024;
   constexpr int P = KS / NW;
-  static_assert(KS % NW == 0 && !(GEGLU && RES) && !(RES && LN), "shape of the instantiations");
+  static_assert(KS % NW == 0 && !(GEGLU && RES) && !(RES && LN) && !(GEGLU && LN == 2) && LN >= 0 && LN <= 2, "shape of the instantiations");
   constexpr int E = 2 * RT + (RES ? 2 * RT : 0);
   extern __shared__ __attribute__((aligned(16))) unsigned char smem[];
   const int lane = threadIdx.x & 63;
@@ -58,7 +58,7 @@
 #pragma unroll
     for (int s = 0; s < KS; ++s) x[t][s] = (dbg & 8) ? u32x4{0x3f803f80u, 0x3f803f80u, 0x3f803f80u, 0x3f803f80u} : __builtin_amdgcn_raw_buffer_load_b128(rs_x, vo + s * 32, 0, 0);
   }
-  if constexpr (LN) {
+  if constexpr (LN == 1) {
     const float invk = 1.f / (float)(KS * 16);
     const bf16x2 ones2 = __builtin_bit_cast(bf16x2, 0x3f803f80u);
 #pragma unroll
@@ -83,6 +83,19 @@
         const unsigned d[4] = {x[t][s].x, x[t][s].y, x[t][s].z, x[t][s].w};
         x[t][s] = u32x4{pack2bf(fmaf(bflo(d[0]), rstd, nb), fmaf(bfhi(d[0]), rstd, nb)), pack2bf(fmaf(bflo(d[1]), rstd, nb), fmaf(bfhi(d[1]), rstd, nb)),
                         pack2bf(fmaf(bflo(d[2]), rstd, nb), fmaf(bfhi(d[2]), rstd, nb)), pack2bf(fmaf(bflo(d[3]), rstd, nb), fmaf(bfhi(d[3]), rstd, nb))};
+      }
+    }
+  }
+  if constexpr (LN == 2) {
+#pragma unroll
+    for (int t = 0; t < RT; ++t) {
+      const int px = (row_w + t * 32 + r) % a.stats_hw;
+      const float mean = a.row_stats[2 * px], k = a.row_stats[2 * px + 1];
+#pragma unroll
+      for (int s = 0; s < KS; ++s) {
+        const unsigned d[4] = {x[t][s].x, x[t][s].y, x[t][s].z, x[t][s].w};
+        x[t][s] = u32x4{pack2bf((bflo(d[0]) - mean) * k, (bfhi(d[0]) - mean) * k), pack2bf((bflo(d[1]) - mean) * k, (bfhi(d[1]) - mean) * k),
+                        pack2bf((bflo(d[2]) - mean) * k, (bfhi(d[2]) - mean) * k), pack2bf((bflo(d[3]) - mean) * k, (bfhi(d[3]) - mean) * k)};
       }
     }
   }
@@ -292,7 +305,7 @@
 #endif
 }
 
-template <int KS, bool GEGLU, bool RES, bool LN>
+template <int KS, bool GEGLU, bool RES, int LN>
 int launch_xs(const MvdXsArgs& a, hipStream_t s) {
   constexpr int LDS_BYTES = (GEGLU ? 2 : 3) * (KS + 1) * 1024 + 4 * (GEGLU ? 8192 : 4096);
   static bool init[16] = {};
@@ -324,6 +337,7 @@
   if (a.K != 320 || a.units <= 0 || a.M <= 0 || a.relu) return false;
   if (a.units % (a.geglu ? 4 : 2)) return false;
   if ((a.geglu || a.ln) && a.res) return false;
+  if (a.ln < 0 || a.ln > 2 || (a.ln == 2 && (a.geglu || !a.row_stats || a.stats_hw <= 0))) return false;
   if ((size_t)(a.M + 256) * a.ldx * 2 >= lim || (size_t)(a.M + 256) * a.ldo * 2 >= lim) return false;
   if (a.res && (size_t)(a.M + 256) * a.ldres * 2 >= lim) return false;
   if ((size_t)a.units * 21 * 1024 >= lim) return false;
@@ -347,9 +361,10 @@
     mvd_set_error("gemm_xs: M=%d K=%d units=%d geglu=%d csplit=%d is not a shape of the X-stationary kernels", a.M, a.K, a.units, a.geglu, a.csplit);
     return -1;
   }
-  if (a.geglu) return a.ln ? launch_xs<20, true, false, true>(a, s) : launch_xs<20, true, false, false>(a, s);
-  if (a.res) return launch_xs<20, false, true, false>(a, s);
-  return a.ln ? launch_xs<20, false, false, true>(a, s) : launch_xs<20, false, false, false>(a, s);
+  if (a.geglu) return a.ln ? launch_xs<20, true, false, 1>(a, s) : launch_xs<20, true, false, 0>(a, s);
+  if (a.res) return launch_xs<20, false, true, 0>(a, s);
+  if (a.ln == 2) return launch_xs<20, false, false, 2>(a, s);
+  return a.ln ? launch_xs<20, false, false, 1>(a, s) : launch_xs<20, false, false, 0>(a, s);
 }
 
 extern "C" int mvd_op_linear_xs(const void* x, int ldx, const void* w_packed, int m, int k, int units, int geglu, int ln, float ln_eps,
@@ -360,3 +375,12 @@
   if (!x || !w_packed || !out) { mvd_set_error("mvd_op_linear_xs: null operand"); return -1; }
   return mvd_launch_gemm_xs(a, (hipStream_t)stream);
 }
+
+extern "C" int mvd_op_linear_xs_refstats(const void* x, int ldx, const void* w_packed, int m, int k, int units, const float* stats, int hw,
+                                         void* out, int ldo, int csplit, void* stream) {
+  MvdXsArgs a; memset(&a, 0, sizeof(a));
+  a.x = (const bf16_t*)x; a.ldx = ldx; a.w = (const bf16_t*)w_packed; a.M = m; a.K = k; a.units = units; a.ln = 2;
+  a.row_stats = stats; a.stats_hw = hw; a.out = (bf16_t*)out; a.ldo = ldo; a.csplit = csplit;
+  if (!x || !w_packed || !out || !stats || hw <= 0) { mvd_set_error("mvd_op_linear_xs_refstats: bad argument"); return -1; }
+  return mvd_launch_gemm_xs(a, (hipStream_t)stream);
+}
diff --git a/mvd_amd/csrc/kernels.h b/mvd_amd/csrc/kernels.h
--- a/mvd_amd/csrc/kernels.h
+++ b/mvd_amd/csrc/kernels.h
@@ -54,7 +54,7 @@
 int mvd_gemm_pick_config(const MvdGemmArgs& a);
 int mvd_launch_gemm_relu(const MvdGemmArgs& a, hipStream_t s, int cfg, bool glds);
 int mvd_launch_splitk_reduce_relu(const MvdGemmArgs& a, hipStream_t s, int grid);
-struct MvdLaunchPlan { int cfg, splitk, tiles, grid, per_cu, nowait; };
+struct MvdLaunchPlan { int cfg, splitk, tiles, grid, per_cu, nowait, walk; };
 extern thread_local MvdLaunchPlan g_mvd_last_gemm;
 extern std::atomic<long> g_mvd_up4_launches;
 bool mvd_gemm_pp_applicable(const MvdGemmArgs& a);
@@ -77,6 +77,8 @@
   bf16_t* out; int ldo;
   int csplit;
   int relu;
+  const float* row_stats;
+  int stats_hw;
 };
 bool mvd_gemm_xs_applicable(const MvdXsArgs& a);
 int mvd_gemm_xs_pick_csplit(const MvdXsArgs& a);
@@ -130,7 +132,7 @@
 int mvd_launch_layernorm(const bf16_t* x, int rows, int c, float eps, const float* gamma, const float* beta,
                          bf16_t* y, hipStream_t s);
 int mvd_launch_refnorm(const bf16_t* x, int batch, int hw, int c, bf16_t* y, hipStream_t s);
-int mvd_launch_refstats(const bf16_t* x, int batch, int hw, int c, float* stats , hipStream_t s);
+int mvd_launch_refstats(const bf16_t* x, int batch, int hw, int c, float* stats , hipStream_t s, int mean_k = 0);
 int mvd_launch_refapply(const bf16_t* x, int batch, int hw, int c, const float* mean_k , bf16_t* y, hipStream_t s);
 
 int mvd_launch_nchw_to_nhwc(const float* x, int batch, int c, int hw, const float* scale, const float* shift,
diff --git a/mvd_amd/csrc/norm.hip b/mvd_amd/csrc/norm.hip
--- a/mvd_amd/csrc/norm.hip
+++ b/mvd_amd/csrc/norm.hip
@@ -313,83 +313,87 @@
   }
 }
 
+template <int NV>
+struct RefPixel {
+  u32x4 r[NV > 0 ? NV : 1];
+  const bf16_t* x; int hw, c, vec, total, p;
+  MVD_DEVINL size_t off(int e) const { const int b = e / vec, v = e % vec; return ((size_t)b * hw + p) * c + v * 8; }
+  MVD_DEVINL RefPixel(const bf16_t* x_, int batch, int hw_, int c_) : x(x_), hw(hw_), c(c_), vec(c_ >> 3), total(batch * (c_ >> 3)), p(blockIdx.x) {
+    if constexpr (NV > 0) {
+#pragma unroll
+      for (int i = 0; i < NV; ++i) {
+        const int e = threadIdx.x + i * 256;
+        if (e < total) r[i] = *reinterpret_cast<const u32x4*>(x + off(e));
+      }
+    }
+  }
+  template <class F> MVD_DEVINL void each(F&& f) const {
+    if constexpr (NV > 0) {
+#pragma unroll
+      for (int i = 0; i < NV; ++i) {
+        const int e = threadIdx.x + i * 256;
+        if (e < total) { float v[8]; unpack8(r[i], v); f(e, v); }
+      }
+    } else {
+      for (int e = threadIdx.x; e < total; e += 256) { float v[8]; unpack8(*reinterpret_cast<const u32x4*>(x + off(e)), v); f(e, v); }
+    }
+  }
+};
+MVD_DEVINL float ref_block_sum(float v, float* red) {
+  const int lane = threadIdx.x & 63, wave = threadIdx.x >> 6;
+  v = wave_sum(v);
+  __syncthreads();
+  if (lane == 0) red[wave] = v;
+  __syncthreads();
+  return red[0] + red[1] + red[2] + red[3];
+}
+template <int NV>
+MVD_DEVINL void ref_mean_m2(const RefPixel<NV>& px, float n, float* red, float& mean, float& m2) {
+  float s = 0.f;
+  px.each([&](int, const float* f) {
+#pragma unroll
+    for (int j = 0; j < 8; ++j) s += f[j];
+  });
+  mean = ref_block_sum(s, red) / n;
+  float q = 0.f;
+  const float mu = mean;
+  px.each([&](int, const float* f) {
+#pragma unroll
+    for (int j = 0; j < 8; ++j) { const float d = f[j] - mu; q = fmaf(d, d, q); }
+  });
+  m2 = ref_block_sum(q, red);
+}
+
+template <int NV>
 __global__ __launch_bounds__(256) void refnorm_kernel(const bf16_t* __restrict__ x, int batch, int hw, int c,
                                                       bf16_t* __restrict__ y) {
   __shared__ float red[8];
-  const int p = blockIdx.x;
-  const int vec = c >> 3;
-  const int total = batch * vec;
-  const int lane = threadIdx.x & 63, wave = threadIdx.x >> 6;
-  auto block_sum = [&](float v) -> float {
-    v = wave_sum(v);
-    __syncthreads();
-    if (lane == 0) red[wave] = v;
-    __syncthreads();
-    return red[0] + red[1] + red[2] + red[3];
-  };
-  float s = 0.f;
-  for (int e = threadIdx.x; e < total; e += 256) {
-    const int b = e / vec, v = e % vec;
-    float f[8];
-    unpack8(*reinterpret_cast<const u32x4*>(x + ((size_t)b * hw + p) * c + v * 8), f);
-#pragma unroll
-    for (int j = 0; j < 8; ++j) s += f[j];
-  }
+  const RefPixel<NV> px(x, batch, hw, c);
   const float n = (float)batch * (float)c;
-  const float mean = block_sum(s) / n;
-  float q = 0.f;
-  for (int e = threadIdx.x; e < total; e += 256) {
-    const int b = e / vec, v = e % vec;
-    float f[8];
-    unpack8(*reinterpret_cast<const u32x4*>(x + ((size_t)b * hw + p) * c + v * 8), f);
-#pragma unroll
-    for (int j = 0; j < 8; ++j) { const float d = f[j] - mean; q = fmaf(d, d, q); }
-  }
-  const float var = block_sum(q) / (n - 1.0f);
+  float mean, m2;
+  ref_mean_m2(px, n, red, mean, m2);
+  const float var = m2 / (n - 1.0f);
   const float k = 0.5f / fmaxf(sqrtf(var), 1e-6f);
-  for (int e = threadIdx.x; e < total; e += 256) {
-    const int b = e / vec, v = e % vec;
-    float f[8];
-    const size_t off = ((size_t)b * hw + p) * c + v * 8;
-    unpack8(*reinterpret_cast<const u32x4*>(x + off), f);
-#pragma unroll
-    for (int j = 0; j < 8; ++j) f[j] = (f[j] - mean) * k;
-    *reinterpret_cast<u32x4*>(y + off) = pack8(f);
-  }
-}
-
-__global__ __launch_bounds__(256) void refstats_kernel(const bf16_t* __restrict__ x, int batch, int hw, int c, float* __restrict__ stats) {
+  px.each([&](int e, const float* f) {
+    float o[8];
+#pragma unroll
+    for (int j = 0; j < 8; ++j) o[j] = (f[j] - mean) * k;
+    *reinterpret_cast<u32x4*>(y + px.off(e)) = pack8(o);
+  });
+}
+
+template <int NV>
+__global__ __launch_bounds__(256) void refstats_kernel(const bf16_t* __restrict__ x, int batch, int hw, int c, float* __restrict__ stats,
+                                                       int mean_k) {
   __shared__ float red[8];
-  const int p = blockIdx.x;
-  const int vec = c >> 3;
-  const int total = batch * vec;
-  const int lane = threadIdx.x & 63, wave = threadIdx.x >> 6;
-  auto block_sum = [&](float v) -> float {
-    v = wave_sum(v);
-    __syncthreads();
-    if (lane == 0) red[wave] = v;
-    __syncthreads();
-    return red[0] + red[1] + red[2] + red[3];
-  };
-  float s = 0.f;
-  for (int e = threadIdx.x; e < total; e += 256) {
-    const int b = e / vec, v = e % vec;
-    float f[8];
-    unpack8(*reinterpret_cast<const u32x4*>(x + ((size_t)b * hw + p) * c + v * 8), f);
-#pragma unroll
-    for (int j = 0; j < 8; ++j) s += f[j];
-  }
-  const float mean = block_sum(s) / ((float)batch * (float)c);
-  float q = 0.f;
-  for (int e = threadIdx.x; e < total; e += 256) {
-    const int b = e / vec, v = e % vec;
-    float f[8];
-    unpack8(*reinterpret_cast<const u32x4*>(x + ((size_t)b * hw + p) * c + v * 8), f);
-#pragma unroll
-    for (int j = 0; j < 8; ++j) { const float d = f[j] - mean; q = fmaf(d, d, q); }
-  }
-  const float m2 = block_sum(q);
-  if (threadIdx.x == 0) { stats[2 * p] = mean; stats[2 * p + 1] = m2; }
+  const RefPixel<NV> px(x, batch, hw, c);
+  const float n = (float)batch * (float)c;
+  float mean, m2;
+  ref_mean_m2(px, n, red, mean, m2);
+  if (threadIdx.x == 0) {
+    stats[2 * blockIdx.x] = mean;
+    stats[2 * blockIdx.x + 1] = mean_k ? 0.5f / fmaxf(sqrtf(m2 / (n - 1.0f)), 1e-6f) : m2;
+  }
 }
 
 __global__ __launch_bounds__(256) void refapply_kernel(const bf16_t* __restrict__ x, int batch, int hw, int c,
@@ -533,9 +537,16 @@
   return check_launch("layernorm");
 }
 
-int mvd_launch_refstats(const bf16_t* x, int batch, int hw, int c, float* stats, hipStream_t s) {
-  if (!x || !stats || batch <= 0 || hw <= 0 || c <= 0 || (c % 8)) { mvd_set_error("refstats: bad arguments"); return -1; }
-  hipLaunchKernelGGL(refstats_kernel, dim3(hw), dim3(256), 0, s, x, batch, hw, c, stats);
+#define REF_DISPATCH(KERNEL, ...) do { \
+    const long nv_ = ((long)batch * (c >> 3) + 255) / 256; \
+    if (nv_ <= 2) hipLaunchKernelGGL(KERNEL<2>, dim3(hw), dim3(256), 0, s, __VA_ARGS__); \
+    else if (nv_ <= 5) hipLaunchKernelGGL(KERNEL<5>, dim3(hw), dim3(256), 0, s, __VA_ARGS__); \
+    else if (nv_ <= 10) hipLaunchKernelGGL(KERNEL<10>, dim3(hw), dim3(256), 0, s, __VA_ARGS__); \
+    else if (nv_ <= 20) hipLaunchKernelGGL(KERNEL<20>, dim3(hw), dim3(256), 0, s, __VA_ARGS__); \
+    else hipLaunchKernelGGL(KERNEL<0>, dim3(hw), dim3(256), 0, s, __VA_ARGS__); } while (0)
+int mvd_launch_refstats(const bf16_t* x, int batch, int hw, int c, float* stats, hipStream_t s, int mean_k) {
+  if (!x || !stats || batch <= 0 || hw <= 0 || c <= 0 || (c % 8) || (long)batch * (c >> 3) > (1L << 30)) { mvd_set_error("refstats: bad arguments"); return -1; }
+  REF_DISPATCH(refstats_kernel, x, batch, hw, c, stats, mean_k);
   return check_launch("refstats");
 }
 int mvd_launch_refapply(const bf16_t* x, int batch, int hw, int c, const float* mean_k, bf16_t* y, hipStream_t s) {
@@ -546,8 +557,8 @@
   return check_launch("refapply");
 }
 int mvd_launch_refnorm(const bf16_t* x, int batch, int hw, int c, bf16_t* y, hipStream_t s) {
-  if (!x || !y || batch <= 0 || hw <= 0 || c <= 0 || (c % 8)) { mvd_set_error("refnorm: bad arguments"); return -1; }
-  hipLaunchKernelGGL(refnorm_kernel, dim3(hw), dim3(256), 0, s, x, batch, hw, c, y);
+  if (!x || !y || batch <= 0 || hw <= 0 || c <= 0 || (c % 8) || (long)batch * (c >> 3) > (1L << 30)) { mvd_set_error("refnorm: bad arguments"); return -1; }
+  REF_DISPATCH(refnorm_kernel, x, batch, hw, c, y);
   return check_launch("refnorm");
 }
 
diff --git a/mvd_amd/ops.py b/mvd_amd/ops.py
--- a/mvd_amd/ops.py
+++ b/mvd_amd/ops.py
@@ -71,6 +71,16 @@
     L.call("mvd_op_linear_xs", C.c_void_p(x.data_ptr()), x.stride(0), _p(w_packed), m, k, units, int(geglu), int(ln), float(eps),
            C.c_void_p(res.data_ptr()) if res is not None else None, res.stride(0) if res is not None else 0, _p(out), n_out,
            csplit, _s())
+    return out
+
+
+def linear_xs_refstats(x, w_packed, stats, csplit=0):
+    _bf16(x, w_packed)
+    assert stats.dtype == torch.float32 and stats.is_contiguous() and stats.shape[1] == 2 and x.stride(1) == 1
+    m, units = x.shape[0], w_packed.shape[0]
+    out = torch.empty(m, units * 32, device=x.device, dtype=torch.bfloat16)
+    L.call("mvd_op_linear_xs_refstats", C.c_void_p(x.data_ptr()), x.stride(0), _p(w_packed), m, (w_packed.shape[1] - 1) * 16, units,
+           _p(stats), stats.shape[0], _p(out), units * 32, csplit, _s())
     return out
 
 
@@ -347,6 +357,14 @@
     y = torch.empty_like(x)
     L.call("mvd_op_refnorm", _p(x), B, hw, c, _p(y), _s())
     return y
+
+
+def refstats(x, mean_k=True):
+    _bf16(x)
+    B, hw, c = x.shape
+    st = torch.empty(hw, 2, device=x.device, dtype=torch.float32)
+    L.call("mvd_op_refstats", _p(x), B, hw, c, _p(st), int(mean_k), _s())
+    return st
 
 
 def film(x, scale, shift):
@@ -509,7 +527,8 @@
 def last_gemm_plan():
     out = (C.c_int * 5)()
     L.call("mvd_debug_last_gemm_plan", out)
-    return dict(cfg=out[0], splitk=out[1], tiles=out[2], grid=out[3], per_cu=out[4], nowait=L.lib().mvd_debug_last_gemm_nowait())
+    return dict(cfg=out[0], splitk=out[1], tiles=out[2], grid=out[3], per_cu=out[4], nowait=L.lib().mvd_debug_last_gemm_nowait(),
+                walk=L.lib().mvd_debug_last_gemm_walk())
 
 
 def last_attention_plan():
@@ -532,3 +551,7 @@
     if conv:
         return L.lib().mvd_debug_pick_splitk_conv(m, n, k)
     return L.lib().mvd_debug_pick_splitk(m, n, k, int(geglu))
+
+
+def pp_walk(m, n, k, geglu=False, splitk=1, conv=False):
+    return L.lib().mvd_debug_pp_walk(m, n, k, int(geglu), splitk, int(conv))
```

New measurement: 533.8 forward-passes/s (median of 6 runs). Within noise of the previous version (+0.3%).
